# Asichurter/GPU-Computing-Course

Measured on AMD Instinct MI355X. Metric: triangle-pairs tested/sec (total collision time in ms_per_step), 1M-tri self-collision, higher is better.
Workload: dtype f64

## Files before the change

gpu-computing-course_amd/csrc/cd_build.h:

```cpp
#pragma once
#include "cd_bvh.h"

namespace cd {

struct B32 { float lx, ly, lz, hx, hy, hz; };

__device__ __forceinline__ float hw_min(float a, float b) { float r; asm("v_min_f32 %0, %1, %2" : "=v"(r) : "v"(a), "v"(b)); return r; }
__device__ __forceinline__ float hw_max(float a, float b) { float r; asm("v_max_f32 %0, %1, %2" : "=v"(r) : "v"(a), "v"(b)); return r; }
__device__ __forceinline__ B32 b32_identity()
{
    const float inf = __uint_as_float(0x7f800000u);
    return B32{inf, inf, inf, -inf, -inf, -inf};
}
__device__ __forceinline__ B32 b32_merge(const B32 &a, const B32 &b)
{
    return B32{hw_min(a.lx, b.lx), hw_min(a.ly, b.ly), hw_min(a.lz, b.lz), hw_max(a.hx, b.hx), hw_max(a.hy, b.hy), hw_max(a.hz, b.hz)};
}
__device__ __forceinline__ B32 b32_of(const AmbTable &amb, const Box &b)
{
    const Enc32 e = enc_box32(amb, b);
    return B32{e.lx, e.ly, e.lz, e.hx, e.hy, e.hz};
}
__device__ __forceinline__ B32 b32_load(const float *p)
{
    const float2 a = reinterpret_cast<const float2 *>(p)[0], b = reinterpret_cast<const float2 *>(p)[1], c = reinterpret_cast<const float2 *>(p)[2];
    return B32{a.x, a.y, b.x, b.y, c.x, c.y};
}
__device__ __forceinline__ void b32_store(float *p, const B32 &v)
{
    reinterpret_cast<float2 *>(p)[0] = make_float2(v.lx, v.ly); reinterpret_cast<float2 *>(p)[1] = make_float2(v.lz, v.hx);
    reinterpret_cast<float2 *>(p)[2] = make_float2(v.hy, v.hz);
}
__device__ __forceinline__ B32 b32_of_leaf(const LeafBox32 *__restrict__ qbox32, int j)
{
    const float4 a = reinterpret_cast<const float4 *>(qbox32 + j)[0];
    const float2 b = reinterpret_cast<const float2 *>(qbox32 + j)[2];
    return B32{a.x, a.y, a.z, a.w, b.x, b.y};
}

__device__ __forceinline__ B32 seg_query32(const float (*t)[6], int l, int r)
{
    B32 acc = b32_identity();
    l += REFIT_BLK; r += REFIT_BLK + 1;
    for (int lev = 0; lev <= REFIT_LOG; ++lev) {
        const bool on = l < r;
        if (!__builtin_amdgcn_ballot_w64(on)) break;
        const int il = (on & ((l & 1) != 0)) ? l : 0, ir = (on & ((r & 1) != 0)) ? r - 1 : 0;
        acc = b32_merge(acc, b32_load(t[il]));
        acc = b32_merge(acc, b32_load(t[ir]));
        l = (l + 1) >> 1; r >>= 1;
    }
    return acc;
}

constexpr int DK_SHIFT = 9;
typedef uint16_t DKey;
constexpr DKey DK_PAD = 0xffffu;
static_assert(DL_LEVELS - 1 <= DK_SHIFT && ((64 + 32 + 1) << DK_SHIFT) < 0xffff, "key layout");
__device__ __forceinline__ int nsv_dir(const DKey (*T)[DL_STRIDE], bool right, int s, int thr)
{
    const int tk = thr << DK_SHIFT;
    int p = s;
#pragma unroll
    for (int k = DL_LEVELS - 1; k >= 0; --k) {
        const int q = right ? p + (1 << k) : p - (1 << k);
        const int idx = right ? p : q + 1;
        const bool inside = right ? (q <= DL_N) : (q >= -1);
        const DKey v = T[k][(idx >= 0 && idx < DL_N) ? idx : 0];
        p = (inside & (v >= (DKey)tk)) ? q : p;
    }
    return p;
}

__device__ __forceinline__ unsigned long long f64_ordered(double d)
{
    const unsigned long long u = (unsigned long long)__double_as_longlong(d);
    return (u >> 63) ? ~u : (u | 0x8000000000000000ull);
}
__device__ __forceinline__ double f64_from_ordered(unsigned long long k)
{
    return __longlong_as_double((long long)((k >> 63) ? (k & 0x7fffffffffffffffull) : ~k));
}

struct ZeroPlan { uint32_t *w0; uint32_t nw0; uint4 *q; uint32_t nq; uint32_t *w1; uint32_t nw1;
                  uint32_t *flag; };

__global__ __launch_bounds__(REFIT_BLK) void k_build_block(const double *__restrict__ verts, const LeafTri *__restrict__ leaf, int n,
                                                           const uint64_t *__restrict__ keys, int32_t *__restrict__ split_of,
                                                           double *__restrict__ boxes, NodeRec32 *__restrict__ recs32, LeafBox32 *__restrict__ qbox32,
                                                           int32_t *__restrict__ root_name, double *__restrict__ seg, float *__restrict__ seg32, int nbp2,
                                                           int32_t *__restrict__ cross_list, uint32_t *__restrict__ cross_count, uint32_t cross_cap, ZeroPlan zp,
                                                           int seg_min ,
                                                           AmbTable amb, const uint8_t *__restrict__ vamb,
                                                           const uint32_t *__restrict__ hint_perm, const uint8_t *__restrict__ hint_tri, uint32_t *__restrict__ hint_cost ,
                                                           unsigned long long *__restrict__ leaf_side ,
                                                           int store_qbox )
{
    {
        const uint32_t G = gridDim.x * REFIT_BLK;
        for (uint32_t x = blockIdx.x * REFIT_BLK + threadIdx.x; x < zp.nq; x += G) zp.q[x] = make_uint4(0u, 0u, 0u, 0u);
        if (blockIdx.x == gridDim.x - 1) {
            for (uint32_t x = threadIdx.x; x < zp.nw0; x += REFIT_BLK) zp.w0[x] = 0u;
            for (uint32_t x = threadIdx.x; x < zp.nw1; x += REFIT_BLK) zp.w1[x] = 0u;
            if (threadIdx.x == 0 && zp.flag) *zp.flag = 0u;
        }
    }
    __shared__ float t[2 * REFIT_BLK][6];
    constexpr size_t TABLE_BYTES = sizeof(DKey) * DL_LEVELS * DL_STRIDE, NB_BYTES = sizeof(float) * 6 * REFIT_BLK;
    __shared__ __align__(16) unsigned char scratch[TABLE_BYTES > NB_BYTES ? TABLE_BYTES : NB_BYTES];
    DKey (*dt)[DL_STRIDE] = reinterpret_cast<DKey (*)[DL_STRIDE]>(scratch);
    float (*nb)[6] = reinterpret_cast<float (*)[6]>(scratch);
    __shared__ int16_t lsplit[REFIT_BLK];
    __shared__ uint8_t lcov[REFIT_BLK];
    __shared__ unsigned long long lexact[REFIT_BLK / 64], lcertain[REFIT_BLK / 64];
    __shared__ unsigned long long acc[6];
    __shared__ int32_t lcross[64];
    __shared__ uint32_t lcount, lbase;
    const int b = blockIdx.x, b0 = b * REFIT_BLK, tid = threadIdx.x;
    const int j = b0 + tid;
    if (tid == 0) { lcount = 0; b32_store(t[0], b32_identity()); }
    lcov[tid] = 0;
    if (tid < 6) acc[tid] = (tid & 1) ? 0ull : ~0ull;
    for (int x = tid; x < DL_STRIDE; x += REFIT_BLK) {
        int v = 0;
        const int p = b0 - 1 + x;
        if (x < DL_N && p >= 0 && p < n - 1) v = delta_k(keys, n, p, keys[p], p + 1) + 1;
        dt[0][x] = x < DL_N ? (DKey)(v << DK_SHIFT) : DK_PAD;
    }
    Box mine = box_identity();
    B32 m32 = b32_identity();
    bool exact = false, certain = false;
    if (j < n) {
        const LeafTri lt = leaf[j];
        const d3 A = load_vertex(verts, lt.v0), B = load_vertex(verts, lt.v1), C = load_vertex(verts, lt.v2);
        mine = box_set(A, B, C);
        const Enc32 e = enc_leaf32(amb, mine, A, B, C, vamb, lt.v0, lt.v1, lt.v2);
        m32 = B32{e.lx, e.ly, e.lz, e.hx, e.hy, e.hz};
        certain = e.certain;
        exact = certain && box_is_fp32(mine);
        if (!exact || n == 1) store_box(boxes, (n - 1) + j, mine);
        if (store_qbox) {
            float4 *qp = reinterpret_cast<float4 *>(qbox32 + j);
            qp[0] = make_float4(m32.lx, m32.ly, m32.lz, m32.hx);
            qp[1] = make_float4(m32.hy, m32.hz, __uint_as_float((exact ? LB_EXACT : 0u) | (certain ? LB_CERTAIN : 0u) | (box_overlap(mine, mine) ? LB_SELF : 0u)), 0.f);
        }
    }
    b32_store(t[REFIT_BLK + tid], m32);
    {
        const unsigned long long em = __builtin_amdgcn_ballot_w64(exact), cm = __builtin_amdgcn_ballot_w64(certain);
        if ((tid & 63) == 0) { lexact[tid >> 6] = em; lcertain[tid >> 6] = cm; }
    }
    for (int dd = REFIT_LOG - 1; dd >= 0; --dd) {
        __syncthreads();
        {
            const int k = REFIT_LOG - dd;
            for (int x = tid; x < DL_STRIDE; x += REFIT_BLK) {
                const int y = x + (1 << (k - 1));
                const DKey u = dt[k - 1][x], w = y < DL_STRIDE ? dt[k - 1][y] : DK_PAD;
                dt[k][x] = (w >> DK_SHIFT) < (u >> DK_SHIFT) ? (DKey)(w + (1 << (k - 1))) : u;
            }
        }
        const int cnt = 1 << dd;
        if (tid < cnt) {
            const int k = cnt + tid;
            const B32 m = b32_merge(b32_load(t[2 * k]), b32_load(t[2 * k + 1]));
            b32_store(t[k], m);
            if (REFIT_LOG - dd >= seg_min) b32_store(seg32 + 6 * ((((size_t)nbp2 + b) << dd) + tid), m);
        }
    }
    __syncthreads();
    if (j < n) {
        const B32 tot = b32_load(t[1]);
        if (m32.lx == tot.lx) atomicMin(&acc[0], f64_ordered(mine.x1));
        if (m32.hx == tot.hx) atomicMax(&acc[1], f64_ordered(mine.x2));
        if (m32.ly == tot.ly) atomicMin(&acc[2], f64_ordered(mine.y1));
        if (m32.hy == tot.hy) atomicMax(&acc[3], f64_ordered(mine.y2));
        if (m32.lz == tot.lz) atomicMin(&acc[4], f64_ordered(mine.z1));
        if (m32.hz == tot.hz) atomicMax(&acc[5], f64_ordered(mine.z2));
    }
    if (hint_cost) {
        uint32_t c = j < n ? (uint32_t)hint_tri[hint_perm[j]] : 0u;
#pragma unroll
        for (int o = 32; o; o >>= 1) { const uint32_t u = (uint32_t)__shfl_xor((int)c, o); c = u > c ? u : c; }
        if ((tid & 63) == 0 && j < n) hint_cost[j >> 6] = c;
    }
    const bool is_left = j < n && (dt[0][tid + 1] >> DK_SHIFT) > (dt[0][tid] >> DK_SHIFT);
    {
        const unsigned long long sm = __builtin_amdgcn_ballot_w64(is_left);
        if ((tid & 63) == 0 && j < n) leaf_side[j >> 6] = sm;
    }
    const int i = j;
    int first = 0, last = 0, split = 0; bool have = false, cross = false;
    if (i < n - 1) {
        const int x = tid;
        const int dL = (int)(dt[0][x] >> DK_SHIFT), dR = (int)(dt[0][x + 1] >> DK_SHIFT);
        const bool right = dR >= dL;
        const int thr = right ? dL : dR;
        int p = nsv_dir(dt, right, right ? x + 2 : x - 1, thr);
        if (right && thr == 0) p = (n - 1 <= b0 + REFIT_BLK - 1) ? (n - 1) - (b0 - 1) : DL_N;
        if (right) { first = i; last = b0 - 1 + p; have = p <= REFIT_BLK; }
        else { first = b0 + p; last = i; have = p >= 0; }
        cross = !have;
        if (have) {
            const int a = first - (b0 - 1), e = last - 1 - (b0 - 1);
            const int k = 31 - __clz(e - a + 1);
            const int a1 = e - (1 << k) + 1;
            const DKey m0 = dt[k][a], m1 = dt[k][a1];
            const int omask = (1 << DK_SHIFT) - 1;
            split = b0 - 1 + (((m1 >> DK_SHIFT) < (m0 >> DK_SHIFT)) ? a1 + ((int)m1 & omask) : a + ((int)m0 & omask));
            split_of[i] = split;
            if (split == first) lcov[split - b0] = 1;
            if (split + 1 == last) lcov[split + 1 - b0] = 1;
        }
        lsplit[tid] = have ? (int16_t)(split - b0) : (int16_t)-1;
        if (cross) {
            const uint32_t k = atomicAdd(&lcount, 1u);
            if (k < 64u) lcross[k] = i;
            else { const uint32_t g = atomicAdd(cross_count, 1u); if (g < cross_cap) cross_list[g] = i; }
        }
    }
    __syncthreads();
    b32_store(nb[tid], seg_query32(t, have ? first - b0 : 1, have ? last - b0 : 0));
    __syncthreads();
    if (j < n && n > 1 && !lcov[tid]) {
        float4 *h = const_cast<float4 *>(is_left ? rec_left(recs32, n, (uint32_t)j) : rec_right(recs32, n, (uint32_t)(j - 1)));
        h[0] = make_float4(m32.lx, m32.ly, m32.lz, m32.hx);
        h[1] = make_float4(m32.hy, m32.hz, __int_as_float(~j), __uint_as_float((exact ? 1u : 0u) | (certain ? 2u : 0u)));
    }
    if (have) {
        const bool leafL = split == first, leafR = split + 1 == last;
        const int sl = split - b0, sr = split + 1 - b0;
        const B32 bl = b32_load(leafL ? t[REFIT_BLK + sl] : nb[sl]);
        const B32 br = b32_load(leafR ? t[REFIT_BLK + sr] : nb[sr]);
        const int32_t la = leafL ? ~split : b0 + (int)lsplit[sl], lb = leafR ? ~(split + 1) : b0 + (int)lsplit[sr];
        const uint32_t fl = ((leafL && ((lcertain[sl >> 6] >> (sl & 63)) & 1ull)) ? REC_L_CERTAIN : 0u) |
                            ((leafR && ((lcertain[sr >> 6] >> (sr & 63)) & 1ull)) ? REC_R_CERTAIN : 0u);
        const uint32_t fx = ((leafL && ((lexact[sl >> 6] >> (sl & 63)) & 1ull)) ? REC_L_EXACT : 0u) |
                            ((leafR && ((lexact[sr >> 6] >> (sr & 63)) & 1ull)) ? REC_R_EXACT : 0u);
        float4 *pl = const_cast<float4 *>(rec_left(recs32, n, (uint32_t)split)), *pr = const_cast<float4 *>(rec_right(recs32, n, (uint32_t)split));
        pl[0] = make_float4(bl.lx, bl.ly, bl.lz, bl.hx); pl[1] = make_float4(bl.hy, bl.hz, __int_as_float(la), __uint_as_float((uint32_t)first | fx));
        pr[0] = make_float4(br.lx, br.ly, br.lz, br.hx); pr[1] = make_float4(br.hy, br.hz, __int_as_float(lb), __uint_as_float((uint32_t)last | fl));
        if (i == 0) *root_name = split;
    }
    if (tid == 0) {
        const Box tot{f64_from_ordered(acc[0]), f64_from_ordered(acc[1]), f64_from_ordered(acc[2]), f64_from_ordered(acc[3]),
                      f64_from_ordered(acc[4]), f64_from_ordered(acc[5])};
        store_box(seg, nbp2 + b, tot);
        if (nbp2 == 1) store_box(boxes, 0, tot);
    }
    const uint32_t cnt = min(lcount, 64u);
    if (cnt == 0) return;
    if (tid == 0) lbase = atomicAdd(cross_count, cnt);
    __syncthreads();
    if ((uint32_t)tid < cnt && lbase + tid < cross_cap) cross_list[lbase + tid] = lcross[tid];
}

__global__ __launch_bounds__(256) void k_fill_qbox(const double *__restrict__ verts, const LeafTri *__restrict__ leaf, int n, LeafBox32 *__restrict__ qbox32,
                                                   AmbTable amb, const uint8_t *__restrict__ vamb)
{
    const int j = blockIdx.x * 256 + threadIdx.x;
    if (j >= n) return;
    const LeafTri lt = leaf[j];
    const d3 A = load_vertex(verts, lt.v0), B = load_vertex(verts, lt.v1), C = load_vertex(verts, lt.v2);
    const Box mine = box_set(A, B, C);
    const Enc32 e = enc_leaf32(amb, mine, A, B, C, vamb, lt.v0, lt.v1, lt.v2);
    const bool exact = e.certain && box_is_fp32(mine);
    float4 *qp = reinterpret_cast<float4 *>(qbox32 + j);
    qp[0] = make_float4(e.lx, e.ly, e.lz, e.hx);
    qp[1] = make_float4(e.hy, e.hz, __uint_as_float((exact ? LB_EXACT : 0u) | (e.certain ? LB_CERTAIN : 0u) | (box_overlap(mine, mine) ? LB_SELF : 0u)), 0.f);
}

__device__ __forceinline__ B32 seg_piece32(const AmbTable &amb, const double *__restrict__ seg, const float *__restrict__ seg32, const LeafBox32 *__restrict__ qbox32,
                                           int n, long long P, long long k, int p, int seg_min = SEG_MIN_LEVEL)
{
    if (p > REFIT_LOG) return b32_of(amb, load_box(seg, (int)k));
    if (p >= seg_min) return b32_load(seg32 + 6 * (size_t)k);
    const long long j0 = (k << p) - P;
    B32 x = b32_identity();
    for (int u = 0; u < (1 << p); ++u) { const long long jj = j0 + u; if (jj < n) x = b32_merge(x, b32_of_leaf(qbox32, (int)jj)); }
    return x;
}

template <int CTRL>
__device__ __forceinline__ float dpp_row_shl32(float v, float fill)
{
    return __int_as_float(__builtin_amdgcn_update_dpp(__float_as_int(fill), __float_as_int(v), CTRL, 0xf, 0xf, false));
}
template <int CTRL>
__device__ __forceinline__ B32 dpp_step32(const B32 &x)
{
    const float inf = __uint_as_float(0x7f800000u);
    const B32 y{dpp_row_shl32<CTRL>(x.lx, inf), dpp_row_shl32<CTRL>(x.ly, inf), dpp_row_shl32<CTRL>(x.lz, inf),
                dpp_row_shl32<CTRL>(x.hx, -inf), dpp_row_shl32<CTRL>(x.hy, -inf), dpp_row_shl32<CTRL>(x.hz, -inf)};
    return b32_merge(x, y);
}
__device__ __forceinline__ B32 b32_shfl_down(const B32 &x, int s)
{
    return B32{__shfl_down(x.lx, s), __shfl_down(x.ly, s), __shfl_down(x.lz, s), __shfl_down(x.hx, s), __shfl_down(x.hy, s), __shfl_down(x.hz, s)};
}

__global__ __launch_bounds__(256) void k_cross_records(int n, const NodeMeta *__restrict__ meta, const double *__restrict__ seg, const float *__restrict__ seg32,
                                                       int nbp2, const LeafBox32 *__restrict__ qbox32, double *__restrict__ boxes, NodeRec32 *__restrict__ recs32,
                                                       const int32_t *__restrict__ split_of, int32_t *__restrict__ root_name,
                                                       const int32_t *__restrict__ dense, const uint32_t *__restrict__ dense_total, uint32_t dense_cap, AmbTable amb)
{
    const int tid = threadIdx.x, lane = tid & 63;
    const uint32_t total = min(*dense_total, dense_cap);
    const long long P = (long long)nbp2 * REFIT_BLK;
    for (uint32_t kk = blockIdx.x * 4 + (tid >> 6); kk < total; kk += gridDim.x * 4) {
        const int i = __builtin_amdgcn_readfirstlane(dense[kk]);
        const NodeMeta m = meta[i];
        const int first = min(i, m.z), last = max(i, m.z);
        const int split = (m.x >= n - 1) ? m.x - (n - 1) : m.x;
        const bool second = lane >= 32;
        B32 x = b32_identity();
        if (last - first < 65535) {
            const int hl = lane & 31;
            const bool is_left = hl < 16;
            const int l0 = second ? split + 1 : first, r0 = second ? last : split;
            const int p = is_left ? hl : 31 - hl;
            const long long lp = ((long long)l0 + P + ((1ll << p) - 1)) >> p;
            const long long rp = ((long long)r0 + P + 1) >> p;
            if (lp < rp) {
                const long long k = is_left ? lp : rp - 1;
                const bool take = is_left ? (lp & 1) : (rp & 1);
                if (take) x = seg_piece32(amb, seg, seg32, qbox32, n, P, k, p);
            }
            x = dpp_step32<0x101>(x); x = dpp_step32<0x102>(x); x = dpp_step32<0x104>(x); x = dpp_step32<0x108>(x);
            x = b32_merge(x, b32_shfl_down(x, 16));
        } else {
            B32 res[2];
            for (int h = 0; h < 2; ++h) {
                const int l0 = h ? split + 1 : first, r0 = h ? last : split;
                const bool is_left = lane < 32;
                const int p = is_left ? lane : 63 - lane;
                const long long lp = ((long long)l0 + P + ((1ll << p) - 1)) >> p;
                const long long rp = ((long long)r0 + P + 1) >> p;
                B32 y = b32_identity();
                if (lp < rp) {
                    const long long k = is_left ? lp : rp - 1;
                    const bool take = is_left ? (lp & 1) : (rp & 1);
                    if (take) y = seg_piece32(amb, seg, seg32, qbox32, n, P, k, p);
                }
                for (int s = 1; s < 64; s <<= 1) y = b32_merge(y, b32_shfl_down(y, s));
                res[h] = B32{__shfl(y.lx, 0), __shfl(y.ly, 0), __shfl(y.lz, 0), __shfl(y.hx, 0), __shfl(y.hy, 0), __shfl(y.hz, 0)};
            }
            x = second ? res[1] : res[0];
        }
        const bool leafL = split == first, leafR = split + 1 == last;
        uint32_t fl = 0, fx = 0;
        if (leafL) { const uint32_t f = qbox32[first].flags; if (f & LB_CERTAIN) fl |= REC_L_CERTAIN; if (f & LB_EXACT) fx |= REC_L_EXACT; }
        if (leafR) { const uint32_t f = qbox32[last].flags; if (f & LB_CERTAIN) fl |= REC_R_CERTAIN; if (f & LB_EXACT) fx |= REC_R_EXACT; }
        if (lane == 0) {
            const int32_t la = child_link(meta, split_of, m.x, n - 1);
            float4 *pl = const_cast<float4 *>(rec_left(recs32, n, (uint32_t)split));
            pl[0] = make_float4(x.lx, x.ly, x.lz, x.hx); pl[1] = make_float4(x.hy, x.hz, __int_as_float(la), __uint_as_float((uint32_t)first | fx));
            if (i == 0) { *root_name = split; store_box(boxes, 0, load_box(seg, 1)); }
        }
        if (lane == 32) {
            const int32_t lb = child_link(meta, split_of, m.y, n - 1);
            float4 *pr = const_cast<float4 *>(rec_right(recs32, n, (uint32_t)split));
            pr[0] = make_float4(x.lx, x.ly, x.lz, x.hx); pr[1] = make_float4(x.hy, x.hz, __int_as_float(lb), __uint_as_float((uint32_t)last | fl));
        }
    }
}

__device__ __forceinline__ B32 block_box32(const float *__restrict__ seg32, int nbp2, int nblocks, int b)
{
    const B32 v = b32_load(seg32 + 6 * ((size_t)nbp2 + (b < nblocks ? b : 0)));
    return b < nblocks ? v : b32_identity();
}
struct U3 { unsigned long long a, b, c; };
__device__ __forceinline__ U3 b32_words(const B32 &v)
{
    auto w = [](float lo, float hi) { return (unsigned long long)__float_as_uint(lo) | ((unsigned long long)__float_as_uint(hi) << 32); };
    return U3{w(v.lx, v.ly), w(v.lz, v.hx), w(v.hy, v.hz)};
}
template <class Low>
__device__ __forceinline__ void top32_to_lds(float *top, const float *__restrict__ blk, int nbp2, int nblocks, Low low)
{
    const int tid = threadIdx.x, lane = tid & 63;
    const int M = nbp2 >> 3;
    if (M >= 1) {
        const int T = M;
        B32 x = b32_identity();
        if (tid < T) {
            const int b = 8 * tid;
            const float4 *q = reinterpret_cast<const float4 *>(blk + 6 * (size_t)b);
            float4 v[12];
#pragma unroll
            for (int u = 0; u < 12; ++u) v[u] = q[u];
            const B32 id = b32_identity();
            B32 pr[4];
#pragma unroll
            for (int u = 0; u < 4; ++u) {
                const float4 q0 = v[3 * u], q1 = v[3 * u + 1], q2 = v[3 * u + 2];
                const B32 b0 = b + 2 * u < nblocks ? B32{q0.x, q0.y, q0.z, q0.w, q1.x, q1.y} : id, b1 = b + 2 * u + 1 < nblocks ? B32{q1.z, q1.w, q2.x, q2.y, q2.z, q2.w} : id;
                pr[u] = b32_merge(b0, b1);
                low((nbp2 >> 1) + 4 * tid + u, pr[u]);
            }
            const B32 q0 = b32_merge(pr[0], pr[1]), q1 = b32_merge(pr[2], pr[3]);
            low((nbp2 >> 2) + 2 * tid, q0); low((nbp2 >> 2) + 2 * tid + 1, q1);
            x = b32_merge(q0, q1);
            b32_store(top + 6 * (M + tid), x);
        }
        const int kt = M + tid;
        for (int s = 1; s < 64 && s < T; s <<= 1) {
            x = b32_merge(x, b32_shfl_down(x, s));
            if (tid < T && (lane & (2 * s - 1)) == 0) b32_store(top + 6 * (kt / (2 * s)), x);
        }
        __syncthreads();
        if (T > 64 && tid == 0) {
            const int kw = T / 64;
            if (T == 128) b32_store(top + 6, b32_merge(b32_load(top + 6 * 2), b32_load(top + 6 * 3)));
            else {
                const B32 l = b32_merge(b32_load(top + 6 * kw), b32_load(top + 6 * (kw + 1))), r = b32_merge(b32_load(top + 6 * (kw + 2)), b32_load(top + 6 * (kw + 3)));
                b32_store(top + 6 * 2, l); b32_store(top + 6 * 3, r); b32_store(top + 6, b32_merge(l, r));
            }
        }
    }
    __syncthreads();
}
template <class Low>
__device__ __forceinline__ void top32_tiny(const float *__restrict__ blk, int nbp2, int nblocks, Low low)
{
    if (threadIdx.x != 0) return;
    auto blkbox = [&](int b) { const B32 v = b32_load(blk + 6 * (size_t)(b < nblocks ? b : 0)); return b < nblocks ? v : b32_identity(); };
    const B32 l = b32_merge(blkbox(0), blkbox(1));
    if (nbp2 == 2) { low(1, l); return; }
    const B32 r = b32_merge(blkbox(2), blkbox(3));
    low(2, l); low(3, r); low(1, b32_merge(l, r));
}

__device__ __forceinline__ void root_box_fold(const double *__restrict__ seg, int nbp2, int nblocks, double *__restrict__ out)
{
    __shared__ double wbox[4][6];
    const int tid = threadIdx.x, lane = tid & 63, w = tid >> 6;
    const int T = nbp2 < 256 ? nbp2 : 256, per = nbp2 / T;
    Box x = box_identity();
    if (tid < T)
        for (int u = 0; u < per; ++u) { const int b = tid * per + u; if (b < nblocks) x = box_merge(x, load_box(seg, nbp2 + b)); }
    for (int s = 1; s < 64 && s < T; s <<= 1) x = box_merge(x, box_shfl_down(x, s));
    if (lane == 0) { double *d = wbox[w]; d[0] = x.x1; d[1] = x.x2; d[2] = x.y1; d[3] = x.y2; d[4] = x.z1; d[5] = x.z2; }
    __syncthreads();
    if (tid == 0) {
        auto wb = [&](int k) { return Box{wbox[k][0], wbox[k][1], wbox[k][2], wbox[k][3], wbox[k][4], wbox[k][5]}; };
        Box r = wb(0);
        for (int k = 1; k < (T + 63) / 64; ++k) r = box_merge(r, wb(k));
        store_box(out, 0, r);
    }
}

__global__ __launch_bounds__(256) void k_top_publish(const float *__restrict__ seg32, int nbp2, int nblocks, unsigned long long *__restrict__ top_pub)
{
    __shared__ float top[6 * (TOP_IN_BLOCK / 4)];
    const int span = blockIdx.x, nspans = nbp2 / TOP_IN_BLOCK, tid = threadIdx.x;
    const int live = nblocks - span * TOP_IN_BLOCK;
    auto heap = [&](int k) { const int d = 31 - __clz(k); return ((size_t)(nspans + span) << d) + (size_t)(k - (1 << d)); };
    top32_to_lds(top, seg32 + 6 * ((size_t)nbp2 + (size_t)span * TOP_IN_BLOCK), TOP_IN_BLOCK, live < 0 ? 0 : (live > TOP_IN_BLOCK ? TOP_IN_BLOCK : live),
                 [&](int k, const B32 &v) { const U3 w = b32_words(v); unsigned long long *d = top_pub + 3 * heap(k); d[0] = w.a; d[1] = w.b; d[2] = w.c; });
    for (int k = 1 + tid; k < TOP_IN_BLOCK / 4; k += 256) {
        const size_t g = heap(k);
        const unsigned long long *src = reinterpret_cast<const unsigned long long *>(top + 6 * k);
#pragma unroll
        for (int u = 0; u < 3; ++u) top_pub[3 * g + u] = src[u];
    }
}
constexpr int TOP_MAX_SPANS = 1024;
__global__ __launch_bounds__(256) void k_top_publish_upper(unsigned long long *__restrict__ top_pub, int nspans, uint32_t *__restrict__ top_flag, uint32_t top_seq)
{
    __shared__ float h[2 * TOP_MAX_SPANS][6];
    const int tid = threadIdx.x;
    for (int k = nspans + tid; k < 2 * nspans; k += 256) {
        unsigned long long *dst = reinterpret_cast<unsigned long long *>(h[k]);
#pragma unroll
        for (int u = 0; u < 3; ++u) dst[u] = top_pub[3 * (size_t)k + u];
    }
    for (int w = nspans >> 1; w >= 1; w >>= 1) {
        __syncthreads();
        for (int k = w + tid; k < 2 * w; k += 256) {
            const B32 m = b32_merge(b32_load(h[2 * k]), b32_load(h[2 * k + 1]));
            b32_store(h[k], m);
            const unsigned long long *src = reinterpret_cast<const unsigned long long *>(h[k]);
#pragma unroll
            for (int u = 0; u < 3; ++u) top_pub[3 * (size_t)k + u] = src[u];
        }
    }
    if (tid == 0) *top_flag = top_seq;
}

__global__ __launch_bounds__(256, 2) void k_cross_fused(const uint64_t *__restrict__ keys, int n, const double *__restrict__ seg, const float *__restrict__ seg32,
                                                     int nbp2, int nblocks, const unsigned long long *__restrict__ leaf_side , double *__restrict__ boxes,
                                                     NodeRec32 *__restrict__ recs32, const int32_t *__restrict__ split_of, int32_t *__restrict__ root_name,
                                                     const int32_t *__restrict__ dense, const uint32_t *__restrict__ dense_total, uint32_t dense_cap,
                                                     unsigned long long *top_pub , uint32_t *top_flag, uint32_t top_seq,
                                                     uint32_t nord ,
                                                     uint32_t order_groups, const uint32_t *__restrict__ hint_cost, uint32_t *__restrict__ hint_order)
{
    extern __shared__ float top[];
    if (blockIdx.x < nord) { build_half_order<256>(blockIdx.x & 7u, blockIdx.x >> 3, order_groups, hint_cost, hint_order, *reinterpret_cast<OrderLds<256> *>(top)); return; }
    const uint32_t bid = blockIdx.x - nord, nbid = gridDim.x - nord;
    const int tid = threadIdx.x, lane = tid & 63, g = lane / XG, gl = lane % XG;
    if (bid == nbid - 1) { root_box_fold(seg, nbp2, nblocks, boxes); return; }
    if (bid == 0) {
        if (nbp2 > TOP_IN_BLOCK) return;
        auto low = [&](int k, const B32 &v) {
            const U3 w = b32_words(v); unsigned long long *d = top_pub + 3 * (size_t)k;
            __hip_atomic_store(d, w.a, __ATOMIC_RELAXED, __HIP_MEMORY_SCOPE_AGENT); __hip_atomic_store(d + 1, w.b, __ATOMIC_RELAXED, __HIP_MEMORY_SCOPE_AGENT);
            __hip_atomic_store(d + 2, w.c, __ATOMIC_RELAXED, __HIP_MEMORY_SCOPE_AGENT);
        };
        if (nbp2 < 8) top32_tiny(seg32 + 6 * (size_t)nbp2, nbp2, nblocks, low);
        else top32_to_lds(top, seg32 + 6 * (size_t)nbp2, nbp2, nblocks, low);
        const int nn = nbp2 < 8 ? 1 : nbp2 >> 2;
        for (int k = 1 + tid; k < nn; k += 256) {
            const unsigned long long *src = reinterpret_cast<const unsigned long long *>(top + 6 * k);
#pragma unroll
            for (int u = 0; u < 3; ++u) __hip_atomic_store(top_pub + 3 * (size_t)k + u, src[u], __ATOMIC_RELAXED, __HIP_MEMORY_SCOPE_AGENT);
        }
        __builtin_amdgcn_s_waitcnt(0);
        __syncthreads();
        if (tid == 0) __hip_atomic_store(top_flag, top_seq, __ATOMIC_RELAXED, __HIP_MEMORY_SCOPE_AGENT);
        return;
    }
    constexpr int PER_WAVE = 64 / XG, PER_BLOCK = 256 / XG;
    const uint32_t total = min(*dense_total, dense_cap);
    const long long P = (long long)nbp2 * REFIT_BLK;
    for (uint32_t wbase = (bid - 1) * PER_BLOCK + (tid >> 6) * PER_WAVE; wbase < total; wbase += (nbid - 2) * PER_BLOCK) {
        const uint32_t kq = wbase + g;
        const bool live = kq < total;
        int first = 0, last = 0, split = 0;
        {
            auto delta_v = [](uint64_t ka, int ia, uint64_t kb, int ib) { const uint64_t x = ka ^ kb; return x ? __clzll((long long)x) : 64 + __clz((int)((uint32_t)ia ^ (uint32_t)ib)); };
            const int i = live ? dense[kq] : 0;
            const uint64_t ki = keys[i], kprev = keys[i > 0 ? i - 1 : 0], knext = keys[i + 1 < n ? i + 1 : n - 1];
            const int dnext = i + 1 < n ? delta_v(ki, i, knext, i + 1) : -1, dprev = i > 0 ? delta_v(ki, i, kprev, i - 1) : -1;
            const int d = (dnext - dprev) >= 0 ? 1 : -1;
            const int delta_min = d > 0 ? dprev : dnext;
            int mlen = 0;
            for (int r = 0; r < 2; ++r) {
                const bool todo = live && mlen == 0;
                if (!__builtin_amdgcn_ballot_w64(todo)) break;
                const int e = r * XG + gl;
                const long long o = (long long)i + (long long)d * (2ll << (e < 31 ? e : 31));
                const bool yes = todo && e < 31 && o >= 0 && o < n && delta_k(keys, n, i, ki, (int)o) > delta_min;
                const uint32_t no = ~group_ballot(yes, g) & ((1u << XG) - 1u);
                if (todo && no) mlen = 2 << (r * XG + __ffs((int)no) - 1);
            }
            const int l = group_last_true(live, mlen >> 1, mlen, g, gl, [&](int x) { return delta_k(keys, n, i, ki, i + x * d) > delta_min; });
            const int j = i + l * d;
            first = min(i, j); last = max(i, j);
            const uint64_t kj = keys[j];
            const uint64_t kbefore = first > 0 ? keys[first - 1] : 0ull, kafter = last < n - 1 ? keys[last + 1] : 0ull;
            const uint64_t kf = first == i ? ki : kj, kl = last == i ? ki : kj;
            const int common = delta_v(kf, first, kl, last);
            split = group_last_true(live, first, last, g, gl, [&](int x) { return delta_k(keys, n, first, kf, x) > common; });
            if (live && gl == 0) {
                if (first == 0 && last == n - 1) *root_name = split;
                else {
                    const int dl = first > 0 ? delta_v(kf, first, kbefore, first - 1) : -1, dr = last < n - 1 ? delta_v(kl, last, kafter, last + 1) : -1;
                    uint32_t *half = reinterpret_cast<uint32_t *>(const_cast<float4 *>(dr > dl ? rec_left(recs32, n, (uint32_t)last) : rec_right(recs32, n, (uint32_t)(first - 1))));
                    half[6] = (uint32_t)split;
                }
            }
        }
        const bool leafL = split == first, leafR = split + 1 == last;
        const bool crossL = !leafL && first / REFIT_BLK != split / REFIT_BLK, crossR = !leafR && (split + 1) / REFIT_BLK != last / REFIT_BLK;
        const bool own = live && gl == 0;
        const uint32_t pwL = reinterpret_cast<const uint32_t *>(rec_left(recs32, n, (uint32_t)(own && leafL ? split : 0)))[7];
        const uint32_t pwR = reinterpret_cast<const uint32_t *>(rec_right(recs32, n, (uint32_t)(own && leafR ? split : 0)))[7];
        const uint32_t flagL = ((pwL & 1u) ? LB_EXACT : 0u) | ((pwL & 2u) ? LB_CERTAIN : 0u), flagR = ((pwR & 1u) ? LB_EXACT : 0u) | ((pwR & 2u) ? LB_CERTAIN : 0u);
        const int32_t soL = split_of[own && !leafL && !crossL ? split : 0], soR = split_of[own && !leafR && !crossR ? split + 1 : 0];
        const int sweeps = __builtin_amdgcn_ballot_w64(live && last - first >= 65535) ? 2 : 1;
        B32 accL = b32_identity(), accR = b32_identity();
        auto piece = [&](int h, int p, int side, long long &k) {
            const int l0 = h ? split + 1 : first, r0 = h ? last : split;
            const long long lp = ((long long)l0 + P + ((1ll << p) - 1)) >> p;
            const long long rp = ((long long)r0 + P + 1) >> p;
            k = side ? rp - 1 : lp;
            return live && lp < rp && ((side ? rp : lp) & 1);
        };
        for (int sw = 0; sw < sweeps; ++sw) {
            const int p = gl + 16 * sw;
            long long kk[4]; bool tk[4]; bool any_top = false;
#pragma unroll
            for (int u = 0; u < 4; ++u) { tk[u] = p > REFIT_LOG && piece(u >> 1, p, u & 1, kk[u]); any_top |= tk[u]; }
            if (!__builtin_amdgcn_ballot_w64(any_top)) continue;
            bool ready = !any_top;
            const bool must = any_top && p > REFIT_LOG + 2;
#ifdef CROSS_FORCE_FALLBACK
            for (uint32_t spin = 0; spin < 0u; ++spin) {
#else
            for (uint32_t spin = 0; spin < (1u << 20); ++spin) {
#endif
                if (!ready) ready = __hip_atomic_load(top_flag, __ATOMIC_RELAXED, __HIP_MEMORY_SCOPE_AGENT) == top_seq;
                if (!__builtin_amdgcn_ballot_w64(must && !ready)) break;
                __builtin_amdgcn_s_sleep(2);
            }
#pragma unroll
            for (int u = 0; u < 4; ++u) if (tk[u]) {
                B32 v;
                if (ready) {
                    unsigned long long w[3];
#pragma unroll
                    for (int e = 0; e < 3; ++e) w[e] = __hip_atomic_load(top_pub + 3 * (size_t)kk[u] + e, __ATOMIC_RELAXED, __HIP_MEMORY_SCOPE_AGENT);
                    v = B32{__uint_as_float((uint32_t)w[0]), __uint_as_float((uint32_t)(w[0] >> 32)), __uint_as_float((uint32_t)w[1]),
                            __uint_as_float((uint32_t)(w[1] >> 32)), __uint_as_float((uint32_t)w[2]), __uint_as_float((uint32_t)(w[2] >> 32))};
                } else {
                    v = b32_identity();
                    const long long b_first = (kk[u] << (p - REFIT_LOG)) - nbp2;
                    for (long long bb = 0; bb < (1ll << (p - REFIT_LOG)); ++bb) v = b32_merge(v, block_box32(seg32, nbp2, nblocks, (int)(b_first + bb)));
                }
                if (u < 2) accL = b32_merge(accL, v); else accR = b32_merge(accR, v);
            }
        }
        {
            constexpr int SMIN = SEG32_MIN_LEVEL, LEAF_ITEMS = 2 * ((1 << SMIN) - 1), N_ITEMS = LEAF_ITEMS + 2 * (REFIT_LOG + 1 - SMIN);
            static_assert(XG == 16 && N_ITEMS <= 2 * XG, "a lane fetches items gl and gl + 16 of either child");
            static_assert(REFIT_BLK == (1 << REFIT_LOG) && SMIN >= 1 && SMIN <= REFIT_LOG, "item t >= LEAF_ITEMS is side (t - LEAF_ITEMS) & 1 of level SMIN + (t - LEAF_ITEMS) / 2 <= REFIT_LOG of a 2^REFIT_LOG-leaf block");
            B32 it[4]; bool tk[4];
            static_assert(LEAF_ITEMS <= XG, "the leaf items are a lane's FIRST item of either child (r = 0, 2)");
#pragma unroll
            for (int r = 0; r < 4; ++r) {
                const int h = r >> 1, t = gl + 16 * (r & 1);
                int p, side, e;
                if (t < LEAF_ITEMS) { const int lg = 31 - __clz(t + 2); p = lg - 1; const int idx = t + 2 - (1 << lg); side = idx >> p; e = idx & ((1 << p) - 1); }
                else { const int u = t - LEAF_ITEMS; p = SMIN + (u >> 1); side = u & 1; e = 0; if (p > REFIT_LOG) p = REFIT_LOG; }
                long long k;
                bool take = t < N_ITEMS && piece(h, p, side, k);
                const bool leafitem = (r & 1) == 0 && p < SMIN;
                uint32_t jl = 0u;
                if (leafitem) {
                    const long long jj = take ? ((k << p) - P + e) : 0;
                    take = take && jj < n;
                    jl = take ? (uint32_t)jj : 0u;
                }
                const float *p1 = leafitem ? reinterpret_cast<const float *>(rec_left(recs32, n, jl + 1u < (uint32_t)n ? jl : 0u)) : seg32 + 6 * (size_t)(take ? k : (P >> p));
                const B32 v1 = b32_load(p1);
                if ((r & 1) == 0) {
                    const B32 vr = b32_load(leafitem ? reinterpret_cast<const float *>(rec_right(recs32, n, jl > 0u ? jl - 1u : 0u)) : p1);
                    const unsigned long long sw = leaf_side[jl >> 6];
                    const bool rt = leafitem && ((sw >> (jl & 63u)) & 1ull) == 0ull;
                    it[r] = B32{rt ? vr.lx : v1.lx, rt ? vr.ly : v1.ly, rt ? vr.lz : v1.lz, rt ? vr.hx : v1.hx, rt ? vr.hy : v1.hy, rt ? vr.hz : v1.hz};
                } else it[r] = v1;
                tk[r] = take;
            }
#pragma unroll
            for (int r = 0; r < 4; ++r) if (tk[r]) { if (r < 2) accL = b32_merge(accL, it[r]); else accR = b32_merge(accR, it[r]); }
        }
        accL = dpp_step32<0x101>(accL); accL = dpp_step32<0x102>(accL); accL = dpp_step32<0x104>(accL); accL = dpp_step32<0x108>(accL);
        accR = dpp_step32<0x101>(accR); accR = dpp_step32<0x102>(accR); accR = dpp_step32<0x104>(accR); accR = dpp_step32<0x108>(accR);
        if (own) {
            const uint32_t fl = ((leafL && (flagL & LB_CERTAIN)) ? REC_L_CERTAIN : 0u) | ((leafR && (flagR & LB_CERTAIN)) ? REC_R_CERTAIN : 0u);
            const uint32_t fx = ((leafL && (flagL & LB_EXACT)) ? REC_L_EXACT : 0u) | ((leafR && (flagR & LB_EXACT)) ? REC_R_EXACT : 0u);
            const int32_t linkL = leafL ? ~split : soL, linkR = leafR ? ~(split + 1) : soR;
            float4 *pl = const_cast<float4 *>(rec_left(recs32, n, (uint32_t)split)), *pr = const_cast<float4 *>(rec_right(recs32, n, (uint32_t)split));
            pl[0] = make_float4(accL.lx, accL.ly, accL.lz, accL.hx);
            pr[0] = make_float4(accR.lx, accR.ly, accR.lz, accR.hx);
            if (crossL) { reinterpret_cast<float2 *>(pl + 1)[0] = make_float2(accL.hy, accL.hz); reinterpret_cast<uint32_t *>(pl + 1)[3] = (uint32_t)first | fx; }
            else pl[1] = make_float4(accL.hy, accL.hz, __int_as_float(linkL), __uint_as_float((uint32_t)first | fx));
            if (crossR) { reinterpret_cast<float2 *>(pr + 1)[0] = make_float2(accR.hy, accR.hz); reinterpret_cast<uint32_t *>(pr + 1)[3] = (uint32_t)last | fl; }
            else pr[1] = make_float4(accR.hy, accR.hz, __int_as_float(linkR), __uint_as_float((uint32_t)last | fl));
        }
    }
}

}
```

gpu-computing-course_amd/csrc/mi355cd.hip:

```cpp
#include "../../include/mi355cd.h"
#include "cd_math.h"
#include "cd_sort.h"
#include "cd_bvh.h"
#include "cd_build.h"
#include "cd_traverse.h"
#include "cd_post.h"
#include "cd_proximity.h"
#include "cd_ccd.h"
#include "cd_between.h"
#include "cd_rays.h"
#include "cd_points.h"

#include <hip/hip_runtime.h>
#include <hip/hip_ext.h>
#include <atomic>
#include <cfloat>
#include <chrono>
#include <cmath>
#include <cstdio>
#include <cstring>
#include <mutex>
#include <new>
#include <utility>
#include <vector>

using namespace cd;

namespace {

#define HIPCHK(expr)                                                   \
    do {                                                               \
        hipError_t e_ = (expr);                                        \
        if (e_ != hipSuccess) return -(int)e_;                         \
    } while (0)

enum Stage { ST_CREATED = 0, ST_SORTED = 1, ST_BUILT = 2, ST_REFIT = 3 };

enum Ev { EV_MORTON0, EV_MORTON1, EV_SORT1, EV_HIER0, EV_HIER1, EV_REFIT0, EV_REFIT1, EV_TRAV0, EV_TRAV1, EV_DESC1, EV_DEEP0, EV_DEEP1, EV_CHK0, EV_CHK1, EV_BLK0, EV_BLK1, EV_COUNT };

}

struct TravBuf {
    TravState *d_state = nullptr; bool state_owned = false;
    uint32_t *d_pairs = nullptr; uint64_t pairs_cap = 0;
    char *h_report = nullptr;
    uint32_t synced_reports = 0;
    uint64_t direct_id = 0; uint32_t synced_direct = 0;
    uint2 *d_defer = nullptr; uint32_t defer_cap = 0;
    Candidates *d_cand = nullptr; uint64_t cand_cap = 0;
    int32_t *d_deep = nullptr; uint64_t deep_items = 0;
    uint32_t *post_dst = nullptr; uint64_t post_n = 0;
    bool prepared = false; unsigned long long prep_seq = 0; uint32_t *prep_area = nullptr; bool posted = false;
};

struct cd_multi;
struct cd_ctx {
    uint32_t nv = 0, nt = 0;
    cd_multi *attached_multi = nullptr;
    int stage = ST_CREATED;
    int frame_mode = CD_FRAME_REFERENCE;
    uint32_t vbase = 0;
    int trav_variant = 3;
    uint32_t queries_per_wave = 64; 
    uint32_t dbg_no_shared_path = 0;
    uint32_t dbg_diag = 0;
    uint32_t dbg_lds_pad = 0;
    double frame_host[FRAME_WORDS] = {0.004501, -0.476622, -0.381965, 3.08, 0.76, 2.36, 0.0, 0.0};
    hipStream_t stream = nullptr;
    hipEvent_t ev[EV_COUNT] = {};
    double *d_verts = nullptr; uint32_t *d_vidx = nullptr; uint32_t *d_ids = nullptr;
    uint64_t *d_keys[2] = {nullptr, nullptr}; uint32_t *d_perm[2] = {nullptr, nullptr};
    uint32_t *d_counts = nullptr; uint32_t ntiles = 0;
    uint32_t *d_chunk_tot = nullptr;
    void *d_os = nullptr; size_t os_bytes = 0 , zero_bytes = 0 , sort_hi_bytes = 0 ;
    unsigned long long *d_os_look_lo = nullptr;
    uint32_t *d_os_hist = nullptr; uint32_t *d_os_ticket = nullptr; unsigned long long *d_os_look = nullptr;
    double *d_frame = nullptr, *d_partial = nullptr;
    unsigned long long *d_top_pub = nullptr; uint32_t top_seq = 0;
    LeafTri *d_leaf = nullptr; NodeMeta *d_meta = nullptr; int32_t *d_parent = nullptr; double *d_seg = nullptr; float *d_seg32 = nullptr; uint32_t nbp2 = 1; int32_t *d_cross = nullptr; uint32_t cross_cap = 0;
    double *d_boxes = nullptr; uint32_t *d_bounded = nullptr; NodeRec32 *d_recs32 = nullptr; LeafBox32 *d_qbox = nullptr;
    unsigned long long *d_leaf_side = nullptr;
    uint32_t dbg_big_offsets = 0;
    uint32_t dbg_store_qbox = 0;
    AmbTable amb = {nullptr, 0u, 0u};
    unsigned long long *d_amb_keys = nullptr, *d_amb_vals = nullptr; uint64_t amb_cap = 0; uint32_t *d_amb_flag = nullptr;
    bool cell_table_opt = true;
    uint8_t *d_vamb = nullptr, *vamb = nullptr;
    int32_t *d_root = nullptr;
    int32_t *d_split_of = nullptr;
    uint32_t stamp_mask = 15;
    uint32_t dbg_sort_windows = 0;
    bool left_frame = false; uint32_t steps_in_mode1 = 0;
    bool local_small_ok = true, local_small_active = false;
    uint32_t dbg_split_cross = 0;
    uint32_t dbg_no_fused_build = 0;
    uint32_t *d_small = nullptr;
    TravBuf tb[2];
    int exact_blocks = 1024;
    uint64_t *pp_keys[2] = {nullptr, nullptr}; uint32_t *pp_vals[2] = {nullptr, nullptr}; uint32_t *pp_flags = nullptr;
    void *pp_os = nullptr; size_t pp_os_bytes = 0; uint32_t pp_cap = 0;
    uint64_t last_pairs_on_device = 0;
    struct StepLeft {
        bool leaves_filled = false;
        bool leaf_records_filled = false;
        bool hierarchy_valid = false;
        bool internal_boxes_valid = false;
        bool last_tree_fused = false;
        bool events_ride = false;
        bool scratch_clean = false;
        bool qbox_valid = false;
    } left;
    cd_stats stats = {};
    uint32_t sort_flags[9] = {};
    bool stage_events = true;
    uint32_t dbg_report_copies = 0;
    bool order_hint_large = false;
    bool order_hint = true;
    bool order_ready = false;
    uint32_t *d_cost = nullptr, *d_order = nullptr;
    bool order_pending = false;
    uint8_t *d_tri_cost = nullptr;
    bool prezeroed = false;
    hipEvent_t tree_done_event = nullptr;
    bool quiet_pass = false;
    int sort_mode = 0;
    bool graph_opt = false;
    bool poll_opt = true;
    unsigned long long report_seq = 0;
    uint32_t polled_steps = 0, poll_fallbacks = 0;
    uint32_t poll_fb_busy = 0, poll_fb_late_word = 0, poll_fb_lost = 0, poll_max_wait_us = 0;
    bool dbg_poll_check = false;
    uint32_t poll_stale = 0;
    hipGraph_t graph = nullptr; hipGraphExec_t graph_exec = nullptr;
    struct GraphKey { uint64_t cap, spec_n; int sort_mode, variant, frame_mode; uint32_t nt, exact_blocks, dbg; const void *p_pairs, *p_cand, *p_defer, *p_report; uint64_t cand_cap; uint32_t defer_cap, pad; } graph_key = {};
    struct GraphPost { StepLeft left; uint32_t sort_passes; } graph_post = {};
    uint64_t graph_replays = 0, graph_captures = 0;
    bool all_verts_referenced = false;
    int wall_clock_khz = 0;
    double root_box_host[6] = {};
    bool root_box_valid = false;
    ProxState *d_px_state = nullptr; ProxState *h_px_state = nullptr;
    uint2 *d_px_cand = nullptr; uint64_t px_shard_cap = 0;
    uint32_t *d_px_pairs = nullptr; double *d_px_dists = nullptr; uint64_t px_pairs_cap = 0;
    CcdState *d_cc_state = nullptr; CcdState *h_cc_state = nullptr;
    uint2 *d_cc_cand = nullptr; uint64_t cc_shard_cap = 0;
    uint32_t *d_cc_pairs = nullptr; double *d_cc_toi = nullptr, *d_cc_dists = nullptr; uint64_t cc_pairs_cap = 0;
    double *d_cc_x1 = nullptr; NodeRec32 *d_cc_recs = nullptr; int32_t *d_cc_up = nullptr; uint32_t *d_cc_arrive = nullptr;
    CcdState *d_bw_state = nullptr; CcdState *h_bw_state = nullptr;
    uint2 *d_bw_cand = nullptr; uint64_t bw_shard_cap = 0;
    uint32_t *d_bw_pairs = nullptr; double *d_bw_toi = nullptr, *d_bw_dists = nullptr; uint64_t bw_pairs_cap = 0;
    double *d_bw_x1a = nullptr; double *d_bw_x1b = nullptr; uint64_t bw_x1b_cap = 0;
    NodeRec32 *d_bw_recs = nullptr; int32_t *d_bw_up = nullptr; uint32_t *d_bw_arrive = nullptr; uint64_t bw_rec_cap = 0;
    int device = 0;
    struct SweptSeen { bool ran = false; uint32_t n = 0, m_bits = 0; double dist = 0.0; };
    SweptSeen cc_seen;
    SweptSeen bw_seen;
    RayState *d_ry_state = nullptr; RayState *h_ry_state = nullptr;
    char *d_ry_block = nullptr; uint64_t ry_cap = 0;
    PointState *d_pt_state = nullptr; PointState *h_pt_state = nullptr;
    char *d_pt_block = nullptr; uint64_t pt_cap = 0;
};

namespace {

size_t top_pub_nodes(const cd_ctx *c) { return std::max<size_t>(TOP_IN_BLOCK, c->nbp2); }
size_t top_pub_bytes(const cd_ctx *c) { return sizeof(unsigned long long) * 3 * top_pub_nodes(c) + 64; }
uint32_t *top_flag_of(cd_ctx *c) { return reinterpret_cast<uint32_t *>(c->d_top_pub + 3 * top_pub_nodes(c)); }

void free_all(cd_ctx *c)
{
    hipFree(c->d_verts); hipFree(c->d_vidx); hipFree(c->d_ids);
    for (int i = 0; i < 2; ++i) { hipFree(c->d_keys[i]); hipFree(c->d_perm[i]); }
    hipFree(c->d_counts); hipFree(c->d_chunk_tot); hipFree(c->d_os); hipFree(c->d_frame); hipFree(c->d_partial);
    hipFree(c->d_top_pub); hipFree(c->d_leaf); hipFree(c->d_meta); hipFree(c->d_parent); hipFree(c->d_seg); hipFree(c->d_seg32); hipFree(c->d_cross); hipFree(c->d_boxes);
    hipFree(c->d_bounded); hipFree(c->d_recs32); hipFree(c->d_qbox); hipFree(c->d_leaf_side); hipFree(c->d_split_of); hipFree(c->d_cost); hipFree(c->d_order); hipFree(c->d_tri_cost);
    hipFree(c->d_amb_keys); hipFree(c->d_amb_flag); hipFree(c->d_vamb);
    for (TravBuf &tb : c->tb) {
        if (tb.d_pairs) hipFree(reinterpret_cast<char *>(tb.d_pairs) - sizeof(Report));
        if (tb.h_report) hipHostFree(tb.h_report);
        hipFree(tb.d_defer); hipFree(tb.d_deep); hipFree(tb.d_cand);
        if (tb.state_owned) hipFree(tb.d_state);
    }
    for (int i = 0; i < 2; ++i) { hipFree(c->pp_keys[i]); hipFree(c->pp_vals[i]); }
    hipFree(c->pp_flags); hipFree(c->pp_os);
    hipFree(c->d_px_state); hipFree(c->d_px_cand); hipFree(c->d_px_pairs); hipFree(c->d_px_dists);
    if (c->h_px_state) hipHostFree(c->h_px_state);
    hipFree(c->d_cc_state); hipFree(c->d_cc_cand); hipFree(c->d_cc_pairs); hipFree(c->d_cc_toi); hipFree(c->d_cc_dists);
    hipFree(c->d_cc_x1); hipFree(c->d_cc_recs); hipFree(c->d_cc_up); hipFree(c->d_cc_arrive);
    if (c->h_cc_state) hipHostFree(c->h_cc_state);
    hipFree(c->d_bw_state); hipFree(c->d_bw_cand); hipFree(c->d_bw_pairs); hipFree(c->d_bw_toi); hipFree(c->d_bw_dists);
    hipFree(c->d_bw_x1a); hipFree(c->d_bw_x1b); hipFree(c->d_bw_recs); hipFree(c->d_bw_up); hipFree(c->d_bw_arrive);
    if (c->h_bw_state) hipHostFree(c->h_bw_state);
    hipFree(c->d_ry_state); hipFree(c->d_ry_block);
    if (c->h_ry_state) hipHostFree(c->h_ry_state);
    hipFree(c->d_pt_state); hipFree(c->d_pt_block);
    if (c->h_pt_state) hipHostFree(c->h_pt_state);
    if (c->graph_exec) hipGraphExecDestroy(c->graph_exec);
    if (c->graph) hipGraphDestroy(c->graph);
    for (int i = 0; i < EV_COUNT; ++i) if (c->ev[i]) hipEventDestroy(c->ev[i]);
    if (c->stream) hipStreamDestroy(c->stream);
}

inline uint32_t cdiv(uint64_t a, uint32_t b) { return (uint32_t)((a + b - 1) / b); }

struct PinnedPairs { std::mutex mu; struct Buf { const uint32_t *p; uint64_t cap, id; }; std::vector<Buf> v; uint64_t next_id = 1; };
PinnedPairs &pinned_pairs() { static PinnedPairs p; return p; }
uint64_t pinned_pairs_id(const uint32_t *pairs, uint64_t cap)
{
    if (!pairs) return 0;
    PinnedPairs &pp = pinned_pairs();
    std::lock_guard<std::mutex> lock(pp.mu);
    for (const auto &e : pp.v) if (e.p == pairs && cap <= e.cap) return e.id;
    return 0;
}
constexpr uint64_t SPEC_PAIRS = 1u << 15;

__global__ void k_morton_points(const double *__restrict__ xyz, uint64_t n, const double *__restrict__ frame , uint64_t *__restrict__ keys)
{
    const unsigned long long layout = (unsigned long long)__double_as_longlong(frame[6]);
    const KeyLayout kl = key_layout(layout, frame, frame + 3);
    for (uint64_t i = blockIdx.x * (uint64_t)blockDim.x + threadIdx.x; i < n; i += (uint64_t)gridDim.x * blockDim.x)
        keys[i] = layout ? morton3d_layout(xyz[3 * i], xyz[3 * i + 1], xyz[3 * i + 2], kl) : morton3d(xyz[3 * i], xyz[3 * i + 1], xyz[3 * i + 2], frame, frame + 3);
}
__global__ void k_expand_values(const uint64_t *__restrict__ v, uint64_t n, uint64_t *__restrict__ out)
{
    for (uint64_t i = blockIdx.x * (uint64_t)blockDim.x + threadIdx.x; i < n; i += (uint64_t)gridDim.x * blockDim.x) out[i] = expand64(v[i]);
}

__global__ void k_box_pairs(const double *__restrict__ a, const double *__restrict__ b, uint64_t n, uint8_t *__restrict__ overlap,
                            double *__restrict__ merged)
{
    for (uint64_t i = blockIdx.x * (uint64_t)blockDim.x + threadIdx.x; i < n; i += (uint64_t)gridDim.x * blockDim.x) {
        const double *pa = a + 6 * i, *pb = b + 6 * i;
        const Box x{pa[0], pa[1], pa[2], pa[3], pa[4], pa[5]}, y{pb[0], pb[1], pb[2], pb[3], pb[4], pb[5]};
        if (overlap) overlap[i] = box_overlap(x, y) ? 1 : 0;
        if (merged) {
            const Box m = box_merge(x, y);
            double *o = merged + 6 * i;
            o[0] = m.x1; o[1] = m.x2; o[2] = m.y1; o[3] = m.y2; o[4] = m.z1; o[5] = m.z2;
        }
    }
}
__global__ void k_tri_contact_points(const double *__restrict__ t, uint64_t n, uint8_t *__restrict__ out)
{
    for (uint64_t i = blockIdx.x * (uint64_t)blockDim.x + threadIdx.x; i < n; i += (uint64_t)gridDim.x * blockDim.x) {
        const double *p = t + 18 * i;
        out[i] = tri_contact_fast(d3{p[0], p[1], p[2]}, d3{p[3], p[4], p[5]}, d3{p[6], p[7], p[8]},
                                  d3{p[9], p[10], p[11]}, d3{p[12], p[13], p[14]}, d3{p[15], p[16], p[17]}) ? 1 : 0;
    }
}

__global__ void k_amb_scan(const double *__restrict__ v, uint64_t n3, uint32_t *__restrict__ flag)
{
    bool any = false;
    for (uint64_t i = blockIdx.x * (uint64_t)blockDim.x + threadIdx.x; i < n3; i += (uint64_t)gridDim.x * blockDim.x) { const double x = v[i]; any |= (double)(float)x != x; }
    if (__builtin_amdgcn_ballot_w64(any) != 0ull && (threadIdx.x & 63) == 0) atomicOr(flag, 1u);
}
__global__ void k_amb_insert(const double *__restrict__ v, uint64_t n3, unsigned long long *keys, unsigned long long *vals, uint32_t shift, uint32_t mask)
{
    for (uint64_t i = blockIdx.x * (uint64_t)blockDim.x + threadIdx.x; i < n3; i += (uint64_t)gridDim.x * blockDim.x) {
        double x = v[i];
        if (x == 0.0) x = 0.0;
        const unsigned long long key = amb_key((int)(i % 3), amb_cell(x));
        uint32_t h = amb_hash(key, shift);
        for (uint32_t probe = 0; probe <= mask; ++probe) {
            unsigned long long old = __hip_atomic_load(&keys[h], __ATOMIC_RELAXED, __HIP_MEMORY_SCOPE_AGENT) & ~AMB_BIT;
            if (old == 0ull) old = atomicCAS(&keys[h], 0ull, key) & ~AMB_BIT;
            if (old == 0ull || old == key) break;
            h = (h + 1u) & mask;
        }
        const unsigned long long o = f64_ordered(x);
        unsigned long long w = __hip_atomic_load(&vals[h], __ATOMIC_RELAXED, __HIP_MEMORY_SCOPE_AGENT);
        if (w == 0ull) w = atomicCAS(&vals[h], 0ull, o);
        if (w != 0ull && w != o && !(__hip_atomic_load(&keys[h], __ATOMIC_RELAXED, __HIP_MEMORY_SCOPE_AGENT) & AMB_BIT)) atomicOr(&keys[h], AMB_BIT);
    }
}
__global__ void k_amb_vertex(const double *__restrict__ verts, uint32_t nv, AmbTable t, uint8_t *__restrict__ vamb)
{
    for (uint32_t v = blockIdx.x * blockDim.x + threadIdx.x; v < nv; v += gridDim.x * blockDim.x) {
        const double x = verts[3 * (size_t)v], y = verts[3 * (size_t)v + 1], z = verts[3 * (size_t)v + 2];
        vamb[v] = (uint8_t)((amb_lookup(t, 0, x) ? 1u : 0u) | (amb_lookup(t, 1, y) ? 2u : 0u) | (amb_lookup(t, 2, z) ? 4u : 0u));
    }
}

constexpr int BOUNDS_BLOCKS = 1024;
constexpr uint32_t SORT_RETRY_STEPS = 64;
void graph_drop(cd_ctx *c);

int ensure_pairs(cd_ctx *c, TravBuf &tb, uint64_t cap)
{
    if (cap <= tb.pairs_cap) return 0;
    if (tb.d_pairs) hipFree(reinterpret_cast<char *>(tb.d_pairs) - sizeof(Report));
    tb.d_pairs = nullptr; tb.pairs_cap = 0;
    if (&tb == &c->tb[0]) c->last_pairs_on_device = 0;
    char *block = nullptr;
    HIPCHK(hipMalloc(&block, sizeof(Report) + sizeof(uint32_t) * 2 * cap + 16));
    tb.d_pairs = reinterpret_cast<uint32_t *>(block + sizeof(Report));
    tb.pairs_cap = cap;
    return 0;
}

float elapsed(cd_ctx *c, int a, int b)
{
    float ms = 0.f;
    if (hipEventElapsedTime(&ms, c->ev[a], c->ev[b]) != hipSuccess) { (void)hipGetLastError(); return 0.f; }
    return ms;
}

inline hipError_t evrec(cd_ctx *c, int idx)
{
    if (!c->stage_events && !(idx == EV_MORTON0 || idx == EV_TRAV0 || idx == EV_DESC1 || idx == EV_TRAV1 || idx == EV_DEEP0 || idx == EV_DEEP1)) return hipSuccess;
    if (!c->stage_events && idx == EV_MORTON0 && !(c->stamp_mask & 8u)) return hipSuccess;
    return hipEventRecord(c->ev[idx], c->stream);
}

struct Prezeroed {
    cd_ctx *c;
    explicit Prezeroed(cd_ctx *c_) : c(c_) { c->prezeroed = true; }
    ~Prezeroed() { c->prezeroed = false; }
};

static bool fused_build_next(const cd_ctx *c);
int enqueue_morton_sort(cd_ctx *c, bool links_too = true, bool frame_ready = false)
{
    const uint32_t n = c->nt;
    hipStream_t s = c->stream;
    c->order_ready = false;
    HIPCHK(evrec(c, EV_MORTON0));
    const bool auto_frame = c->frame_mode == CD_FRAME_AUTO;
    if (auto_frame && !frame_ready) k_centroid_bounds<false><<<BOUNDS_BLOCKS, 256, 0, s>>>(c->d_verts, c->d_vidx, n, c->d_partial);
    const bool self_cleaning = c->prezeroed && c->sort_mode <= 1 && fused_build_next(c);
    const bool skip_memset = self_cleaning && c->left.scratch_clean;
    c->left.scratch_clean = false;
    if (!skip_memset) HIPCHK(hipMemsetAsync(c->d_os, 0, c->sort_mode <= 1 ? (c->prezeroed ? c->zero_bytes : c->sort_hi_bytes) : c->os_bytes, s));
    const int mode = c->sort_mode;
    const bool hybrid = mode <= 1;
    const int down = mode == 0 ? 4 : 0;
    const int first_digit = hybrid ? 6 : (mode == 2 ? 4 : 0);
    int cur = mode == 3 ? 0 : 1;
    const uint32_t mblocks = c->ntiles < 2048u ? c->ntiles : 2048u;
    unsigned long long host_layout = 0ull; std::memcpy(&host_layout, &c->frame_host[6], sizeof host_layout);
    const double *mframe = auto_frame ? nullptr : c->d_frame;
    const double *mpart = auto_frame ? c->d_partial : nullptr;
    if (auto_frame || host_layout != 0ull)
        k_morton<true><<<mblocks, MORTON_THREADS, 0, s>>>(c->d_verts, c->d_vidx, n, mframe, c->d_keys[cur], c->d_os_hist, first_digit, down, c->d_os_ticket + 16,
                                                          mpart, (uint32_t)BOUNDS_BLOCKS, c->d_frame, nullptr, c->d_counts);
    else
        k_morton<false><<<mblocks, MORTON_THREADS, 0, s>>>(c->d_verts, c->d_vidx, n, mframe, c->d_keys[cur], c->d_os_hist, first_digit, down, c->d_os_ticket + 16,
                                                           mpart, (uint32_t)BOUNDS_BLOCKS, c->d_frame, nullptr, c->d_counts);
    HIPCHK(evrec(c, EV_MORTON1));
    const bool chunked = c->ntiles > (uint32_t)OS_CHUNK_MIN_TILES;
    if (chunked) k_tile_chunks<<<cdiv(c->ntiles, (uint32_t)OS_CHUNK), RADIX, 0, s>>>(c->d_counts, c->ntiles, c->d_chunk_tot);
    for (int pass = first_digit; pass < 8; ++pass) {
        k_os_pass<<<c->ntiles, OS_THREADS, 0, s>>>(c->d_keys[cur], c->d_perm[cur], c->d_keys[cur ^ 1], c->d_perm[cur ^ 1], n, pass * RADIX_BITS - down,
                                                    c->d_os_hist + pass * RADIX,
                                                    (pass >= 6 ? c->d_os_look + (size_t)(pass - 6) * c->ntiles * RADIX : c->d_os_look_lo + (size_t)pass * c->ntiles * RADIX),
                                                    c->d_os_ticket + pass, pass == first_digit, HIST_COPIES, pass == first_digit ? c->d_counts : nullptr,
                                                    pass == first_digit && chunked ? c->d_chunk_tot : nullptr);
        cur ^= 1;
    }
    c->left.leaves_filled = false; c->left.leaf_records_filled = false;
    if (hybrid) {
        const LeafFill fill{c->d_vidx, c->d_ids, n, c->d_leaf, links_too ? c->d_parent : nullptr, links_too ? c->d_bounded : nullptr};
        const bool small = c->dbg_sort_windows == 2 || (c->dbg_sort_windows == 0 && c->local_small_ok);
        c->local_small_active = small;
        if (small) {
            const uint32_t per_half_cu = cdiv(n, 512u), win = per_half_cu >= (uint32_t)LocalSmall::W ? (uint32_t)LocalSmall::W : (per_half_cu < 512u ? 512u : per_half_cu);
            k_local_sort<LeafFill, LocalSmall><<<cdiv(n, win), LocalSmall::THREADS, 0, s>>>(c->d_keys[1], c->d_perm[1], c->d_keys[0], c->d_perm[0], n, 48 - down, c->d_os_ticket + 16, fill,
                                                                                            self_cleaning ? c->d_small : nullptr, self_cleaning ? 128u : 0u, win);
        } else {
            const uint32_t per_cu = cdiv(n, 256u), win = per_cu >= (uint32_t)LOCAL_W ? (uint32_t)LOCAL_W : (per_cu < 1024u ? 1024u : per_cu);
            k_local_sort<LeafFill, LocalLarge><<<cdiv(n, win), LocalLarge::THREADS, 0, s>>>(c->d_keys[1], c->d_perm[1], c->d_keys[0], c->d_perm[0], n, 48 - down, c->d_os_ticket + 16, fill,
                                                                                            self_cleaning ? c->d_small : nullptr, self_cleaning ? 128u : 0u, win);
        }
        c->left.leaves_filled = links_too;
        c->left.leaf_records_filled = true;
    } else if (mode != 3) {
        k_sort_fixup_fill<<<cdiv(n, 256), 256, 0, s>>>(c->d_keys[1], c->d_perm[1], c->d_keys[0], c->d_perm[0], n, c->d_os_ticket + 16,
                                                       c->d_vidx, c->d_ids, c->d_leaf, links_too ? c->d_parent : nullptr, links_too ? c->d_bounded : nullptr);
        c->left.leaves_filled = links_too;
        c->left.leaf_records_filled = true;
    }
    c->stats.sort_passes = hybrid ? 2 : (mode == 2 ? 4 : 8);
    HIPCHK(evrec(c, EV_SORT1));
    HIPCHK(hipGetLastError());
    return 0;
}

int enqueue_hierarchy(cd_ctx *c, bool poison_boxes)
{
    const uint32_t n = c->nt;
    hipStream_t s = c->stream;
    HIPCHK(evrec(c, EV_HIER0));
    if (!c->prezeroed) HIPCHK(hipMemsetAsync(c->d_small, 0, 16 * sizeof(uint32_t), s));
    if (!c->left.leaves_filled || poison_boxes)
        k_fill_leaves<<<cdiv(n, 256), 256, 0, s>>>(c->d_perm[0], c->d_vidx, c->d_ids, n, c->d_leaf, c->d_parent, c->d_bounded, poison_boxes ? c->d_boxes : nullptr);
    c->left.leaves_filled = false;
    if (n > 1)
        k_hierarchy<<<cdiv(n - 1, 256), 256, 0, s>>>(c->d_keys[0], (int)n, c->d_meta, c->d_parent, c->d_small);
    c->left.hierarchy_valid = true;
    HIPCHK(evrec(c, EV_HIER1));
    HIPCHK(hipGetLastError());
    return 0;
}

static bool qbox_wanted(const cd_ctx *c)
{
    return c->trav_variant != 3 || c->dbg_split_cross || c->dbg_store_qbox || c->amb.keys != nullptr || c->amb.mask != 0u || c->attached_multi != nullptr;
}
int ensure_qbox(cd_ctx *c)
{
    if (c->left.qbox_valid) return 0;
    k_fill_qbox<<<cdiv(c->nt, 256), 256, 0, c->stream>>>(c->d_verts, c->d_leaf, (int)c->nt, c->d_qbox, c->amb, (const uint8_t *)c->vamb);
    HIPCHK(hipGetLastError());
    c->left.qbox_valid = true;
    return 0;
}
int enqueue_refit(cd_ctx *c, bool write_internal, bool fused = false)
{
    const uint32_t n = c->nt;
    hipStream_t s = c->stream;
    HIPCHK(evrec(c, EV_REFIT0));
    const int nblocks = (int)cdiv(n, REFIT_BLK);
    int32_t *cross_list = c->d_cross;
    uint32_t *cross_count = c->d_small + 16;
    if (!c->prezeroed) HIPCHK(hipMemsetAsync(cross_count, 0, 64 * sizeof(uint32_t), s));
    if (fused) {
        if (!c->left.leaf_records_filled)
            k_fill_leaves<<<cdiv(n, 256), 256, 0, s>>>(c->d_perm[0], c->d_vidx, c->d_ids, n, c->d_leaf, c->d_parent, c->d_bounded, nullptr);
        c->left.leaves_filled = false; c->left.leaf_records_filled = true;
        c->left.hierarchy_valid = false;
        const bool stamp = (c->stamp_mask & 1u) != 0;
        const bool self_cleaning = c->prezeroed && c->sort_mode <= 1;
        ZeroPlan zp{nullptr, 0u, nullptr, 0u, nullptr, 0u, top_flag_of(c)};
        if (self_cleaning) {
            const size_t gran = sizeof(unsigned long long) * (size_t)c->ntiles * RADIX;
            zp = ZeroPlan{c->d_os_hist, (uint32_t)HIST_COPIES * 8u * RADIX + 8u ,
                          reinterpret_cast<uint4 *>(c->d_os_look), (uint32_t)(2 * gran / sizeof(uint4)),
                          reinterpret_cast<uint32_t *>(c->tb[0].d_state), (uint32_t)(sizeof(TravState) / sizeof(uint32_t)), top_flag_of(c)};
        }
        const int seg_min = (c->nbp2 > 1 && !c->dbg_split_cross) ? SEG32_MIN_LEVEL : SEG_MIN_LEVEL;
        const bool hint = c->order_hint && c->trav_variant >= 3 && n > 64u && c->nbp2 > 1 && !c->dbg_split_cross && (c->nbp2 <= (uint32_t)TOP_IN_BLOCK || c->order_hint_large);
        const uint32_t *hp = hint ? c->d_perm[0] : nullptr; const uint8_t *ht = hint ? c->d_tri_cost : nullptr; uint32_t *hc = hint ? c->d_cost : nullptr;
        const int store_q = qbox_wanted(c) ? 1 : 0;
        c->left.qbox_valid = store_q != 0;
        if (stamp)
            hipExtLaunchKernelGGL(k_build_block, dim3(nblocks), dim3(REFIT_BLK), 0u, s, c->ev[EV_BLK0], c->ev[EV_BLK1], 0u,
                                  (const double *)c->d_verts, (const LeafTri *)c->d_leaf, (int)n, (const uint64_t *)c->d_keys[0], c->d_split_of,
                                  c->d_boxes, c->d_recs32, c->d_qbox, c->d_root, c->d_seg, c->d_seg32, (int)c->nbp2,
                                  cross_list, cross_count, c->cross_cap, zp, seg_min, c->amb, (const uint8_t *)c->vamb, hp, ht, hc, c->d_leaf_side, store_q);
        else
            k_build_block<<<nblocks, REFIT_BLK, 0, s>>>(c->d_verts, c->d_leaf, (int)n, c->d_keys[0], c->d_split_of, c->d_boxes, c->d_recs32, c->d_qbox, c->d_root,
                                                        c->d_seg, c->d_seg32, (int)c->nbp2, cross_list, cross_count, c->cross_cap, zp, seg_min, c->amb, (const uint8_t *)c->vamb,
                                                        hp, ht, hc, c->d_leaf_side, store_q);
        c->order_pending = hint;
        c->left.scratch_clean = self_cleaning;
    } else {
        c->left.qbox_valid = true;
        k_refit_seg_local<<<nblocks, REFIT_BLK, 0, s>>>(c->d_verts, c->d_leaf, (int)n, c->d_meta, c->d_boxes, c->d_bounded,
                                                       c->d_recs32, c->d_qbox, c->d_root, write_internal ? 1 : 0, c->d_seg, (int)c->nbp2,
                                                       cross_list, cross_count, c->cross_cap, c->amb, (const uint8_t *)c->vamb);
    }
    if (fused && n > 1 && c->nbp2 > 1 && !c->dbg_split_cross) {
        const uint32_t xb = (uint32_t)nblocks < 8u ? 8u : ((uint32_t)nblocks > 1790u ? 1790u : (uint32_t)nblocks);
        hipEvent_t done = c->tree_done_event; c->tree_done_event = nullptr;
        const uint32_t ogroups = (n + 63u) / 64u;
        const uint32_t nord = c->order_pending ? 8u * (((ogroups + 7u) / 8u + (uint32_t)ORDER_MAX_ITEMS - 1u) / (uint32_t)ORDER_MAX_ITEMS) : 0u;
        c->order_pending = false;
        const bool large = c->nbp2 > (uint32_t)TOP_IN_BLOCK;
        const uint32_t xlds = std::max((uint32_t)(large ? 64u : sizeof(float) * 6 * (c->nbp2 >= 4 ? c->nbp2 / 4 : 1)) ,
                                       nord ? (uint32_t)sizeof(OrderLds<256>) : 0u );
        uint32_t *top_flag = top_flag_of(c);
        if (++c->top_seq == 0u) ++c->top_seq;
        if (large) {
            const int nspans = (int)(c->nbp2 / (uint32_t)TOP_IN_BLOCK);
            k_top_publish<<<nspans, 256, 0, s>>>(c->d_seg32, (int)c->nbp2, nblocks, c->d_top_pub);
            k_top_publish_upper<<<1, 256, 0, s>>>(c->d_top_pub, nspans, top_flag, c->top_seq);
        }
        if (done)
            hipExtLaunchKernelGGL(k_cross_fused, dim3(nord + xb + 2u ), dim3(256), xlds, s, nullptr, done, 0u,
                                  (const uint64_t *)c->d_keys[0], (int)n, (const double *)c->d_seg, (const float *)c->d_seg32, (int)c->nbp2, nblocks, (const unsigned long long *)c->d_leaf_side, c->d_boxes,
                                  c->d_recs32, (const int32_t *)c->d_split_of, c->d_root, (const int32_t *)c->d_cross, (const uint32_t *)cross_count, c->cross_cap,
                                  c->d_top_pub, top_flag, c->top_seq, nord, ogroups, (const uint32_t *)c->d_cost, c->d_order);
        else
            k_cross_fused<<<nord + xb + 2u, 256, xlds, s>>>(c->d_keys[0], (int)n, c->d_seg, c->d_seg32, (int)c->nbp2, nblocks, c->d_leaf_side, c->d_boxes,
                                                            c->d_recs32, c->d_split_of, c->d_root, c->d_cross, cross_count, c->cross_cap, c->d_top_pub, top_flag, c->top_seq,
                                                            nord, ogroups, c->d_cost, c->d_order);
        if (nord) c->order_ready = true;
        c->left.internal_boxes_valid = write_internal;
        HIPCHK(evrec(c, EV_REFIT1));
        HIPCHK(hipGetLastError());
        return 0;
    }
    const bool top_in_meta = fused && n > 1 && c->nbp2 <= (uint32_t)TOP_IN_BLOCK;
    if (!top_in_meta) {
        if (fused && n > 1) {
            int nb = (int)c->nbp2, live = nblocks;
            while (nb > 1) {
                const int span = nb < TOP_IN_BLOCK ? nb : TOP_IN_BLOCK;
                k_top_levels<<<nb / span, 256, 0, s>>>(c->d_seg, nb, live);
                nb /= span; live = (live + span - 1) / span;
            }
        } else k_refit_seg_top<<<1, 1024, 0, s>>>(c->d_seg, (int)c->nbp2, nblocks);
    }
    const uint32_t xblocks = 2u * nblocks < 256u ? 256u : (2u * nblocks > 16384u ? 16384u : 2u * (uint32_t)nblocks);
    if (fused && n > 1) {
        k_cross_meta<<<xblocks, 256, 0, s>>>(c->d_keys[0], (int)n, c->d_meta, c->d_split_of, c->d_cross, cross_count, c->cross_cap,
                                             top_in_meta ? c->d_seg : nullptr, (int)c->nbp2, nblocks);
        k_cross_records<<<xblocks, 256, 0, s>>>((int)n, c->d_meta, c->d_seg, c->d_seg32, (int)c->nbp2, c->d_qbox, c->d_boxes, c->d_recs32,
                                                c->d_split_of, c->d_root, c->d_cross, cross_count, c->cross_cap, c->amb);
    } else if (n > 1)
        k_refit_seg_cross<<<xblocks, 256, 0, s>>>((int)n, c->d_meta, c->d_seg, (int)c->nbp2, c->d_boxes, c->d_bounded, c->d_recs32,
                                                  c->d_root, write_internal ? 1 : 0, c->d_cross, cross_count, c->cross_cap, c->amb);
    c->left.internal_boxes_valid = write_internal;
    HIPCHK(evrec(c, EV_REFIT1));
    HIPCHK(hipGetLastError());
    return 0;
}

static bool fused_build_next(const cd_ctx *c) { return !(c->trav_variant == 0 || c->dbg_no_fused_build); }
int enqueue_tree(cd_ctx *c)
{
    c->left.last_tree_fused = false;
    if (!fused_build_next(c)) {
        int rc = enqueue_hierarchy(c, false);
        if (!rc) rc = enqueue_refit(c, c->trav_variant == 0, false);
        return rc;
    }
    c->left.last_tree_fused = true;
    return enqueue_refit(c, false, true);
}

template <bool EXTERNAL, bool DEEP>
void launch_pass(cd_ctx *c, TravBuf &tb, const QuerySrc &src, uint32_t items, uint64_t cap_pairs)
{
    const int n = (int)c->nt;
    hipStream_t s = c->stream;
    const uint32_t vb = EXTERNAL ? c->vbase : 0u;
    if (c->trav_variant == 0) {
        k_traverse<EXTERNAL, DEEP><<<cdiv(items, TRAV_THREADS), TRAV_THREADS, 0, s>>>(src, items, n, c->d_meta, c->d_boxes, c->d_leaf, c->d_verts, tb.d_pairs, cap_pairs, tb.d_state,
                                                                                       DEEP ? nullptr : tb.d_defer, DEEP ? 0u : tb.defer_cap, DEEP ? tb.d_deep : nullptr, vb);
    } else {
        const bool half_mode = c->trav_variant >= 3 && !EXTERNAL && (DEEP || items == (uint32_t)n);
        const uint32_t qpw = (DEEP || c->trav_variant >= 3) ? 64u : c->queries_per_wave;
        const uint64_t shard_cap = tb.cand_cap / NSHARD;
        const dim3 grid(cdiv(items, qpw * DESC_WAVES));
        const size_t pad = DEEP ? 0 : c->dbg_lds_pad;
        const bool ride = !DEEP && !c->stage_events && !c->quiet_pass;
        hipEvent_t e0 = (ride && (c->stamp_mask & 2u)) ? c->ev[EV_TRAV0] : nullptr, e1 = (ride && (c->stamp_mask & 2u)) ? c->ev[EV_DESC1] : nullptr;
        hipEvent_t e2 = (ride && (c->stamp_mask & 4u)) ? c->ev[EV_TRAV1] : nullptr;
        const uint32_t qarg = qpw | (c->dbg_no_shared_path ? 0x40000000u : 0u);
        uint2 *dl = DEEP ? nullptr : tb.d_defer; const uint32_t dcap = DEEP ? 0u : tb.defer_cap; int32_t *deep = DEEP ? tb.d_deep : nullptr;
        const uint32_t half = half_mode ? 1u : 0u;
        const bool plain = !e0 && !e1 && !e2;
        if (half_mode && !DEEP) {
            const dim3 hgrid(cdiv(items, 64u)), hblock(HALF_THREADS);
            const uint32_t *h_order = (c->order_hint && c->order_ready) ? c->d_order : nullptr;
            const bool h_rec = c->order_hint && (c->nbp2 <= (uint32_t)TOP_IN_BLOCK || c->order_hint_large);
            const uint32_t *h_perm = h_rec ? c->d_perm[0] : nullptr; uint8_t *h_tri = h_rec ? c->d_tri_cost : nullptr;
#define LAUNCH_HALF_(DIAG, TIES, BIG)                                                                                                           \
            do { if (plain) k_descend_half<DIAG, TIES, BIG><<<hgrid, hblock, pad, s>>>(src, n, c->d_recs32, tb.d_state, tb.d_cand, (unsigned long long)shard_cap, dl, dcap, h_order, h_perm, h_tri); \
                 else hipExtLaunchKernelGGL((k_descend_half<DIAG, TIES, BIG>), hgrid, hblock, (uint32_t)pad, s, e0, e1, 0u, src, n, (const NodeRec32 *)c->d_recs32, \
                                            tb.d_state, tb.d_cand, (unsigned long long)shard_cap, dl, dcap, h_order, h_perm, h_tri); } while (0)
            const bool ties = c->amb.keys != nullptr || c->amb.mask != 0u;
            const bool big = n > HALF_SMALL_N || c->dbg_big_offsets;
#define LAUNCH_HALF(DIAG, TIES) do { if (big) LAUNCH_HALF_(DIAG, TIES, true); else LAUNCH_HALF_(DIAG, TIES, false); } while (0)
            if (c->dbg_diag) { if (ties) LAUNCH_HALF(true, true); else LAUNCH_HALF(true, false); }
            else { if (ties) LAUNCH_HALF(false, true); else LAUNCH_HALF(false, false); }
#undef LAUNCH_HALF
#undef LAUNCH_HALF_
        }
        else if (qpw == 64)
            hipExtLaunchKernelGGL((k_descend<EXTERNAL, DEEP, false>), grid, dim3(DESC_THREADS), (uint32_t)pad, s, e0, e1, 0u,
                                  src, items, n, qarg, (const NodeRec32 *)c->d_recs32, (const double *)c->d_boxes, tb.d_state, tb.d_cand, (unsigned long long)shard_cap, dl, dcap, deep, vb, half);
        else
            hipExtLaunchKernelGGL((k_descend<EXTERNAL, DEEP, true>), grid, dim3(DESC_THREADS), (uint32_t)pad, s, e0, e1, 0u,
                                  src, items, n, qarg, (const NodeRec32 *)c->d_recs32, (const double *)c->d_boxes, tb.d_state, tb.d_cand, (unsigned long long)shard_cap, dl, dcap, deep, vb, half);
        if (!DEEP && !ride && !c->quiet_pass) evrec(c, EV_DESC1);
        uint32_t *post = DEEP ? nullptr : tb.post_dst; const unsigned long long post_n = DEEP ? 0ull : (unsigned long long)tb.post_n;
        if (!DEEP) { tb.posted = post != nullptr; tb.post_dst = nullptr; tb.post_n = 0; }
        if (plain)
            k_exact<EXTERNAL><<<c->exact_blocks, EXACT_THREADS, 0, s>>>(src, n, c->d_leaf, c->d_boxes, c->d_verts, vb, tb.d_cand, (unsigned long long)shard_cap, tb.d_pairs,
                                                                        (unsigned long long)cap_pairs, tb.d_state, half, post, post_n);
        else
            hipExtLaunchKernelGGL((k_exact<EXTERNAL>), dim3(c->exact_blocks), dim3(EXACT_THREADS), 0u, s, nullptr, e2, 0u,
                                  src, n, (const LeafTri *)c->d_leaf, (const double *)c->d_boxes, (const double *)c->d_verts, vb, (const Candidates *)tb.d_cand,
                                  (unsigned long long)shard_cap, tb.d_pairs, (unsigned long long)cap_pairs, tb.d_state, half, post, post_n);
        c->left.events_ride = ride;
    }
}

struct HostCounters { uint64_t n_pairs, pairs_tested, node_visits, max_shard_candidates; uint32_t n_deferred; uint64_t wave_steps, candidates, clk_start_inv, clk_end; };

int ensure_report(TravBuf &tb)
{
    if (!tb.h_report) {
        HIPCHK(hipHostMalloc(&tb.h_report, sizeof(Report) + sizeof(uint32_t) * 2 * SPEC_PAIRS, hipHostMallocCoherent));
        std::memset(tb.h_report, 0, sizeof(Report));
    }
    return 0;
}
int enqueue_report(cd_ctx *c, TravBuf &tb, bool want_pairs, uint64_t &spec_n, uint32_t *direct = nullptr, unsigned long long seq = 0)
{
    { const int rc = ensure_report(tb); if (rc) return rc; }
    if (!want_pairs) spec_n = 0; else if (spec_n > SPEC_PAIRS) spec_n = SPEC_PAIRS;
    constexpr int REPORT_BLOCKS = 32;
    const uint64_t copy_n = tb.posted ? 0 : spec_n;
    tb.posted = false;
    k_report<<<copy_n ? REPORT_BLOCKS : 1, REPORT_THREADS, 0, c->stream>>>(tb.d_state, c->d_os_ticket + 8, c->d_boxes, reinterpret_cast<Report *>(tb.h_report),
                                                              tb.d_pairs, direct ? direct : reinterpret_cast<uint32_t *>(tb.h_report + sizeof(Report)), (unsigned long long)copy_n, seq);
    return 0;
}
constexpr uint32_t POLL_WARM = 2;
bool poll_this_report(const cd_ctx *c, TravBuf &tb, uint64_t direct_id)
{
    if (direct_id && direct_id != tb.direct_id) { tb.direct_id = direct_id; tb.synced_direct = 0; }
    return c->poll_opt && !c->stage_events && c->stamp_mask == 0 && tb.synced_reports >= POLL_WARM && (!direct_id || tb.synced_direct >= POLL_WARM);
}
int wait_report(cd_ctx *c, TravBuf &tb, unsigned long long seq)
{
    if (seq != 0ull) {
        const volatile unsigned long long *p = &reinterpret_cast<const volatile Report *>(tb.h_report)->seq;
        const auto t0 = std::chrono::steady_clock::now();
        for (uint32_t it = 1; *p != seq; ++it) {
#if defined(__x86_64__) || defined(__i386__)
            __builtin_ia32_pause();
#endif
            if ((it & 1023u) == 0 && std::chrono::steady_clock::now() - t0 > std::chrono::milliseconds(20)) break;
        }
        if (*p == seq) {
            std::atomic_thread_fence(std::memory_order_acquire);
            if ((c->polled_steps & 15u) == 0) {
                const auto us = std::chrono::duration_cast<std::chrono::microseconds>(std::chrono::steady_clock::now() - t0).count();
                if ((uint64_t)us > c->poll_max_wait_us) c->poll_max_wait_us = (uint32_t)us;
            }
            if ((++c->polled_steps & 63u) == 0) HIPCHK(hipStreamSynchronize(c->stream));
            return 0;
        }
// ... 225 lines not shown
        if (cap != c->amb_cap) {
            hipFree(c->d_amb_keys); c->d_amb_keys = c->d_amb_vals = nullptr; c->amb_cap = 0;
            HIPCHK(hipMalloc(&c->d_amb_keys, sizeof(unsigned long long) * 2 * cap));
            c->d_amb_vals = c->d_amb_keys + cap;
            c->amb_cap = cap;
        }
        HIPCHK(hipMemsetAsync(c->d_amb_keys, 0, sizeof(unsigned long long) * 2 * cap, s));
        const uint32_t shift = 64u - lg, mask = (uint32_t)(cap - 1);
        k_amb_insert<<<blocks, 256, 0, s>>>(c->d_verts, n3, c->d_amb_keys, c->d_amb_vals, shift, mask);
        c->amb = AmbTable{c->d_amb_keys, shift, mask};
        if (!c->d_vamb) HIPCHK(hipMalloc(&c->d_vamb, c->nv));
        k_amb_vertex<<<(uint32_t)std::min<uint64_t>((c->nv + 255ull) / 256, 4096), 256, 0, s>>>(c->d_verts, c->nv, c->amb, c->d_vamb);
        c->vamb = c->d_vamb;
        HIPCHK(hipStreamSynchronize(s));
        HIPCHK(hipGetLastError());
    }
    if (before.keys != c->amb.keys || before.shift != c->amb.shift || before.mask != c->amb.mask) graph_drop(c);
    return CD_OK;
}
bool graph_eligible(const cd_ctx *c)
{
    return c->graph_opt && !c->stage_events && c->stamp_mask == 0 && c->sort_mode <= 1 && fused_build_next(c) && c->trav_variant == 3 &&
           c->left.scratch_clean && !c->dbg_diag && !c->dbg_lds_pad && c->nt > 1 && c->tree_done_event == nullptr;
}
int graph_step(cd_ctx *c, uint32_t *pairs, uint64_t cap_pairs, uint64_t *n_pairs, bool &handled)
{
    handled = false;
    TravBuf &tb = c->tb[0];
    hipStream_t s = c->stream;
    int rc = ensure_pairs(c, tb, cap_pairs > 0 ? cap_pairs : 1);
    if (!rc) rc = ensure_report(tb);
    if (rc) return rc;
    uint64_t spec_n = pairs ? (cap_pairs < SPEC_PAIRS ? cap_pairs : SPEC_PAIRS) : 0;
    const bool direct = pinned_pairs_id(pairs, cap_pairs) != 0;
    const cd_ctx::GraphKey key{cap_pairs, spec_n, c->sort_mode, c->trav_variant, c->frame_mode, c->nt, (uint32_t)c->exact_blocks, c->dbg_no_shared_path | (c->dbg_split_cross << 1) | (c->order_hint ? 4u : 0u) | (c->order_ready ? 8u : 0u) | (c->local_small_ok ? 16u : 0u) | (c->dbg_sort_windows << 5) | (qbox_wanted(c) ? 128u : 0u) ,
                               tb.d_pairs, tb.d_cand, tb.d_defer, direct ? (const void *)pairs : (const void *)tb.h_report, tb.cand_cap, tb.defer_cap, 0u};
    static_assert(sizeof(cd_ctx::GraphKey) == 2 * 8 + 6 * 4 + 4 * 8 + 8 + 2 * 4, "GraphKey has no padding");
    if (!c->graph_exec || std::memcmp(&key, &c->graph_key, sizeof key) != 0) {
        graph_drop(c);
        HIPCHK(hipStreamBeginCapture(s, hipStreamCaptureModeThreadLocal));
        c->prezeroed = true;
        rc = enqueue_morton_sort(c, false);
        if (!rc) rc = enqueue_tree(c);
        if (!rc) {
            QuerySrc src{c->d_leaf, c->d_boxes, c->d_qbox, c->d_root, nullptr, nullptr, c->d_os_ticket + 8};
            launch_pass<false, false>(c, tb, src, c->nt, cap_pairs);
            rc = enqueue_report(c, tb, pairs != nullptr, spec_n, direct ? pairs : nullptr);
        }
        c->prezeroed = false;
        hipGraph_t g = nullptr;
        const hipError_t ee = hipStreamEndCapture(s, &g);
        if (rc || ee != hipSuccess || !g) { if (g) hipGraphDestroy(g); (void)hipGetLastError(); c->left.scratch_clean = false; return CD_OK; }
        c->graph = g;
        if (hipGraphInstantiate(&c->graph_exec, g, nullptr, nullptr, 0) != hipSuccess) { graph_drop(c); (void)hipGetLastError(); c->left.scratch_clean = false; return CD_OK; }
        std::memset(&c->graph_key, 0, sizeof c->graph_key);
        c->graph_key = key;
        c->graph_post = {c->left, c->stats.sort_passes};
        ++c->graph_captures;
    }
    c->left = c->graph_post.left; c->stats.sort_passes = c->graph_post.sort_passes;
    HIPCHK(hipGraphLaunch(c->graph_exec, s));
    HIPCHK(hipStreamSynchronize(s));
    ++c->graph_replays;
    HostCounters h = {};
    parse_report(c, tb, h, direct ? nullptr : pairs, spec_n);
    c->stage = ST_REFIT; c->root_box_valid = true;
    { const int js = judge_sort_flags(c); if (js != CD_OK) return CD_OK; }
    if (shards_overflowed(tb, h) || h.n_deferred > 0) {
        handled = true;
        c->left.scratch_clean = false;
        return run_traversal(c, tb, nullptr, 0, pairs, cap_pairs, n_pairs);
    }
    handled = true;
    const uint64_t found = h.n_pairs, ncopy = found < cap_pairs ? found : cap_pairs;
    if (pairs && ncopy > spec_n) {
        HIPCHK(hipMemcpyAsync(pairs + 2 * spec_n, tb.d_pairs + 2 * spec_n, sizeof(uint32_t) * 2 * (ncopy - spec_n), hipMemcpyDeviceToHost, s));
        HIPCHK(hipStreamSynchronize(s));
    }
    c->stats.ms_morton = c->stats.ms_sort = c->stats.ms_hierarchy = c->stats.ms_refit = c->stats.ms_traverse = c->stats.ms_descend = c->stats.ms_exact = 0.f;
    c->stats.ms_pipeline = c->stats.ms_build_block = 0.f;
    c->stats.traverse_launches = 0; c->stats.stack_overflows = 0;
    c->stats.n_pairs = found; c->stats.pairs_tested = h.pairs_tested; c->stats.node_visits = h.node_visits;
    c->stats.wave_steps = h.wave_steps; c->stats.candidates = h.candidates;
    c->stats.ms_descend_clock = (h.clk_end && h.clk_start_inv && c->wall_clock_khz > 0) ? (float)((double)(h.clk_end - ~h.clk_start_inv) / (double)c->wall_clock_khz) : 0.f;
    c->last_pairs_on_device = ncopy;
    if (n_pairs) *n_pairs = found;
    return found > cap_pairs ? CD_OVERFLOW : CD_OK;
}

}

void multi_detach_from(cd_ctx *c);

extern "C" {

const char *cd_version(void) { return "mi355cd 0.1 gfx950"; }

int cd_create(cd_ctx **out, const double *verts_xyz, uint32_t nv, const uint32_t *vidx3, const uint32_t *ids, uint32_t nt)
{
    if (!out || !verts_xyz || !vidx3 || nv == 0 || nt == 0) return CD_ERR_ARG;
    *out = nullptr;
    int ndev = 0;
    if (hipGetDeviceCount(&ndev) != hipSuccess || ndev == 0) return CD_ERR_NO_DEVICE;
    for (uint64_t k = 0; k < 3ull * nt; ++k) if (vidx3[k] >= nv) return CD_ERR_INDEX;
    bool all_ref = true;
    { std::vector<uint8_t> used(nv, 0);
      for (uint64_t k = 0; k < 3ull * nt; ++k) used[vidx3[k]] = 1;
      for (uint32_t v = 0; v < nv && all_ref; ++v) all_ref = used[v] != 0; }
    cd_ctx *c = new (std::nothrow) cd_ctx();
    if (!c) return CD_ERR_ARG;
    c->nv = nv; c->nt = nt;
    c->all_verts_referenced = all_ref;
    c->ntiles = cdiv(nt, SORT_TILE);
    { int dev = 0, khz = 0; if (hipGetDevice(&dev) == hipSuccess) { c->device = dev; if (hipDeviceGetAttribute(&khz, hipDeviceAttributeWallClockRate, dev) == hipSuccess) c->wall_clock_khz = khz; } (void)hipGetLastError(); }
    const size_t n = nt;
#define ALLOC(p, bytes) do { hipError_t e_ = hipMalloc((void **)&(p), (bytes)); if (e_ != hipSuccess) { free_all(c); delete c; return -(int)e_; } } while (0)
    hipError_t e = hipStreamCreateWithFlags(&c->stream, hipStreamNonBlocking);
    if (e != hipSuccess) { delete c; return -(int)e; }
    for (int i = 0; i < EV_COUNT; ++i) { e = hipEventCreate(&c->ev[i]); if (e != hipSuccess) { free_all(c); delete c; return -(int)e; } }
    ALLOC(c->d_verts, sizeof(double) * 3 * (size_t)nv);
    ALLOC(c->d_vidx, sizeof(uint32_t) * 3 * n);
    if (ids) ALLOC(c->d_ids, sizeof(uint32_t) * n);
    for (int i = 0; i < 2; ++i) { ALLOC(c->d_keys[i], sizeof(uint64_t) * n); ALLOC(c->d_perm[i], sizeof(uint32_t) * n); }
    ALLOC(c->d_counts, sizeof(uint32_t) * RADIX * c->ntiles);
    ALLOC(c->d_chunk_tot, sizeof(uint32_t) * RADIX * cdiv(c->ntiles, (uint32_t)OS_CHUNK));
    const size_t gran = sizeof(unsigned long long) * (size_t)c->ntiles * RADIX;
    const size_t look_off = sizeof(uint32_t) * HIST_COPIES * 8 * RADIX + 128;
    c->sort_hi_bytes = look_off + 2 * gran;
    const size_t small_off = (c->sort_hi_bytes + 127) & ~(size_t)127, state_off = small_off + 512;
    c->zero_bytes = state_off + sizeof(TravState);
    const size_t lo_off = (c->zero_bytes + 127) & ~(size_t)127;
    c->os_bytes = lo_off + 6 * gran;
    ALLOC(c->d_os, c->os_bytes);
    c->d_small = reinterpret_cast<uint32_t *>(reinterpret_cast<char *>(c->d_os) + small_off);
    c->tb[0].d_state = reinterpret_cast<TravState *>(reinterpret_cast<char *>(c->d_os) + state_off);
    c->d_root = reinterpret_cast<int32_t *>(c->d_small + 96);
    c->d_os_hist = reinterpret_cast<uint32_t *>(c->d_os);
    c->d_os_ticket = c->d_os_hist + HIST_COPIES * 8 * RADIX;
    c->d_os_look = reinterpret_cast<unsigned long long *>(reinterpret_cast<char *>(c->d_os) + look_off);
    c->d_os_look_lo = reinterpret_cast<unsigned long long *>(reinterpret_cast<char *>(c->d_os) + lo_off);
    ALLOC(c->d_frame, sizeof(double) * FRAME_WORDS);
    ALLOC(c->d_partial, sizeof(double) * BOUNDS_STRIDE * BOUNDS_BLOCKS);
    ALLOC(c->d_leaf, sizeof(LeafTri) * n);
    { hipError_t e_ = hipMemset(c->d_leaf, 0, sizeof(LeafTri) * n); if (e_ != hipSuccess) { free_all(c); delete c; return -(int)e_; } }
    ALLOC(c->d_meta, sizeof(NodeMeta) * n);
    ALLOC(c->d_parent, sizeof(int32_t) * 2 * n);
    { uint32_t nb = cdiv(nt, REFIT_BLK); c->nbp2 = 1; while (c->nbp2 < nb) c->nbp2 <<= 1; }
    if (c->nbp2 / (uint32_t)TOP_IN_BLOCK > (uint32_t)TOP_MAX_SPANS) { free_all(c); delete c; return CD_ERR_ARG; }
    ALLOC(c->d_seg, sizeof(double) * 6 * (size_t)c->nbp2 * REFIT_BLK);
    ALLOC(c->d_top_pub, top_pub_bytes(c));
    if (hipMemset(c->d_top_pub, 0, top_pub_bytes(c)) != hipSuccess) { free_all(c); delete c; return -(int)hipGetLastError(); }
    ALLOC(c->d_seg32, sizeof(float) * 6 * ((size_t)c->nbp2 << (REFIT_LOG - SEG32_MIN_LEVEL + 1)));
    c->cross_cap = nt;
    ALLOC(c->d_cross, sizeof(int32_t) * (size_t)c->cross_cap);
    ALLOC(c->d_boxes, sizeof(double) * 6 * 2 * n);
    ALLOC(c->d_bounded, sizeof(uint32_t) * n);
    ALLOC(c->d_recs32, sizeof(NodeRec32) * n);
    ALLOC(c->d_qbox, sizeof(LeafBox32) * n);
    ALLOC(c->d_leaf_side, sizeof(unsigned long long) * ((n + 63) / 64 + 1));
    ALLOC(c->d_split_of, sizeof(int32_t) * n);
    { const size_t groups = ((size_t)n + 63) / 64;
      ALLOC(c->d_cost, sizeof(uint32_t) * groups); ALLOC(c->d_order, sizeof(uint32_t) * groups); ALLOC(c->d_tri_cost, n);
      if (hipMemset(c->d_cost, 0, sizeof(uint32_t) * groups) != hipSuccess || hipMemset(c->d_tri_cost, 0, n) != hipSuccess) { free_all(c); delete c; return CD_ERR_ARG; } }
    c->tb[0].cand_cap = ((4 * n > (1u << 20) ? 4 * n : (1u << 20)) + 4 * NSHARD - 1) / (4 * NSHARD) * (4 * NSHARD);
    ALLOC(c->tb[0].d_cand, sizeof(Candidates) * c->tb[0].cand_cap);
    c->tb[0].defer_cap = 1u << 16;
    ALLOC(c->tb[0].d_defer, sizeof(uint2) * c->tb[0].defer_cap);
#undef ALLOC
    bool ok = hipMemcpy(c->d_verts, verts_xyz, sizeof(double) * 3 * (size_t)nv, hipMemcpyHostToDevice) == hipSuccess &&
              hipMemcpy(c->d_vidx, vidx3, sizeof(uint32_t) * 3 * n, hipMemcpyHostToDevice) == hipSuccess &&
              (!ids || hipMemcpy(c->d_ids, ids, sizeof(uint32_t) * n, hipMemcpyHostToDevice) == hipSuccess) &&
              hipMemcpy(c->d_frame, c->frame_host, sizeof(double) * FRAME_WORDS, hipMemcpyHostToDevice) == hipSuccess;
    if (!ok) { free_all(c); delete c; return -(int)hipGetLastError(); }
    { const int rc = amb_refresh(c); if (rc) { free_all(c); delete c; return rc; } }
    *out = c;
    return CD_OK;
}

void cd_destroy(cd_ctx *c)
{
    if (!c) return;
    multi_detach_from(c);
    hipStreamSynchronize(c->stream);
    free_all(c);
    delete c;
}

int cd_update_vertices(cd_ctx *c, const double *verts_xyz)
{
    if (!c || !verts_xyz) return CD_ERR_ARG;
    HIPCHK(hipStreamSynchronize(c->stream));
    HIPCHK(hipMemcpy(c->d_verts, verts_xyz, sizeof(double) * 3 * (size_t)c->nv, hipMemcpyHostToDevice));
    c->stage = ST_CREATED;
    c->root_box_valid = false;
    return amb_refresh(c);
}

static int install_frame(cd_ctx *c, int mode, const double off[3], const double span[3], unsigned long long layout)
{
    if (off) for (int a = 0; a < 3; ++a) { c->frame_host[a] = off[a]; c->frame_host[3 + a] = span[a]; }
    std::memcpy(&c->frame_host[6], &layout, sizeof layout); c->frame_host[7] = 0.0;
    c->frame_mode = mode;
    HIPCHK(hipStreamSynchronize(c->stream));
    HIPCHK(hipMemcpy(c->d_frame, c->frame_host, sizeof(double) * FRAME_WORDS, hipMemcpyHostToDevice));
    c->stage = ST_CREATED;
    graph_drop(c);
    return CD_OK;
}
int cd_set_morton_frame(cd_ctx *c, int mode, const double offset[3], const double span[3])
{
    if (!c) return CD_ERR_ARG;
    if (mode == CD_FRAME_REFERENCE) {
        const double ref[6] = {0.004501, -0.476622, -0.381965, 3.08, 0.76, 2.36};
        return install_frame(c, mode, ref, ref + 3, 0ull);
    }
    if (mode == CD_FRAME_CUSTOM) {
        if (!offset || !span) return CD_ERR_ARG;
        return install_frame(c, mode, offset, span, 0ull);
    }
    if (mode != CD_FRAME_AUTO) return CD_ERR_ARG;
    return install_frame(c, mode, nullptr, nullptr, 0ull);
}
int cd_set_morton_frame_layout(cd_ctx *c, const double offset[3], const double span[3], uint64_t layout)
{
    if (!c || !offset || !span || !layout_ok(layout)) return CD_ERR_ARG;
    for (int a = 0; a < 3; ++a) if (!(span[a] > 0.0)) return CD_ERR_ARG;
    return install_frame(c, CD_FRAME_CUSTOM, offset, span, layout);
}
int cd_get_morton_frame(cd_ctx *c, double offset[3], double span[3], uint64_t *layout)
{
    if (!c) return CD_ERR_ARG;
    if (c->stage < ST_SORTED) return CD_ERR_ORDER;
    double f[FRAME_WORDS];
    HIPCHK(hipStreamSynchronize(c->stream));
    HIPCHK(hipMemcpy(f, c->d_frame, sizeof f, hipMemcpyDeviceToHost));
    for (int a = 0; a < 3; ++a) { if (offset) offset[a] = f[a]; if (span) span[a] = f[3 + a]; }
    if (layout) std::memcpy(layout, &f[6], sizeof *layout);
    return CD_OK;
}

constexpr int SORT_REDO = 77;
constexpr int SORT_REDO_MAX = 4;
namespace { int judge_sort_flags(cd_ctx *c)
{
    for (int i = 0; i < 9; ++i) if (c->sort_flags[i]) c->left.scratch_clean = false;
    for (int i = 0; i < 8; ++i) if (c->sort_flags[i]) return CD_ERR_SORT;
    const uint32_t f = c->sort_flags[8];
    if (!f) return CD_OK;
    if (c->sort_mode >= 3) return CD_ERR_SORT;
    if (f & SORTF_FIXUP) { c->sort_mode = 3; c->left_frame = false; return SORT_REDO; }
    if (f & SORTF_RUN) {
        if (!(f & SORTF_ABOVE) && c->local_small_active && c->local_small_ok && c->sort_mode <= 1) { c->local_small_ok = false; return SORT_REDO; }
        c->sort_mode = 2; c->left_frame = false; return SORT_REDO;
    }
    if (c->sort_mode == 0) { c->sort_mode = 1; c->left_frame = true; c->steps_in_mode1 = 0; return SORT_REDO; }
    c->sort_mode = 2; c->left_frame = false; return SORT_REDO;
} }
static void sort_retry_tick(cd_ctx *c)
{
    if (c->sort_mode == 1 && c->left_frame && ++c->steps_in_mode1 >= SORT_RETRY_STEPS) { c->sort_mode = 0; c->steps_in_mode1 = 0; c->local_small_ok = true; graph_drop(c); }
}
extern "C++" {
template <class Attempt> static int with_sort_redo(cd_ctx *c, Attempt attempt)
{
    for (int redo = 0;; ++redo) {
        const int rc = attempt();
        if (rc < 0) return rc;
        const int js = judge_sort_flags(c);
        if (js != SORT_REDO) return js ? js : rc;
        if (redo == SORT_REDO_MAX) return CD_ERR_SORT;
    }
}
static int sync_with_flags(cd_ctx *c)
{
    HIPCHK(hipMemcpyAsync(c->sort_flags, c->d_os_ticket + 8, sizeof c->sort_flags, hipMemcpyDeviceToHost, c->stream));
    HIPCHK(hipMemcpyAsync(c->root_box_host, c->d_boxes, sizeof(double) * 6, hipMemcpyDeviceToHost, c->stream));
    HIPCHK(hipStreamSynchronize(c->stream));
    return CD_OK;
}
template <class Tail> static int fused_step(cd_ctx *c, Tail tail)
{
    const int rc = with_sort_redo(c, [&]() -> int {
        Prezeroed fused(c);
        int re = enqueue_morton_sort(c, !fused_build_next(c));
        if (!re) re = enqueue_tree(c);
        return re ? re : tail();
    });
    if (rc >= 0) { c->root_box_valid = true; c->stage = ST_REFIT; }
    return rc;
}
}
static void read_build_times(cd_ctx *c)
{
    c->stats.ms_morton = elapsed(c, EV_MORTON0, EV_MORTON1);
    c->stats.ms_sort = elapsed(c, EV_MORTON1, EV_SORT1);
    c->stats.ms_hierarchy = c->left.last_tree_fused ? 0.f : elapsed(c, EV_HIER0, EV_HIER1);
    c->stats.ms_refit = elapsed(c, EV_REFIT0, EV_REFIT1);
}

int cd_morton_sort(cd_ctx *c)
{
    if (!c) return CD_ERR_ARG;
    sort_retry_tick(c);
    const int rc = with_sort_redo(c, [c]() -> int {
        const int re = enqueue_morton_sort(c);
        if (re) return re;
        HIPCHK(hipMemcpyAsync(c->sort_flags, c->d_os_ticket + 8, sizeof c->sort_flags, hipMemcpyDeviceToHost, c->stream));
// ... 104 lines not shown
    c->stats.ms_build_block = (c->left.last_tree_fused && (c->stamp_mask & 1u)) ? elapsed(c, EV_BLK0, EV_BLK1) : 0.f;
    return rc;
}

int cd_brute_force(cd_ctx *c, int box_filter, uint32_t *pairs, uint64_t cap_pairs, uint64_t *n_pairs)
{
    if (!c || (cap_pairs && !pairs)) return CD_ERR_ARG;
    int rc = ensure_pairs(c, c->tb[0], cap_pairs > 0 ? cap_pairs : 1);
    if (rc) return rc;
    hipStream_t s = c->stream;
    HIPCHK(hipMemsetAsync(c->tb[0].d_state, 0, sizeof(TravState), s));
    k_brute_force<<<cdiv(c->nt, 256), 256, 0, s>>>(c->d_verts, c->d_vidx, c->d_ids, c->nt, box_filter, c->tb[0].d_pairs, cap_pairs, c->tb[0].d_state);
    HostCounters h;
    { int r = read_state(c, c->tb[0], h); if (r) return r; }
    HIPCHK(hipGetLastError());
    const uint64_t ncopy = h.n_pairs < cap_pairs ? h.n_pairs : cap_pairs;
    if (pairs && ncopy) HIPCHK(hipMemcpy(pairs, c->tb[0].d_pairs, sizeof(uint32_t) * 2 * ncopy, hipMemcpyDeviceToHost));
    c->stats.n_pairs = h.n_pairs; c->stats.pairs_tested = h.pairs_tested;
    c->last_pairs_on_device = ncopy;
    if (n_pairs) *n_pairs = h.n_pairs;
    return h.n_pairs > cap_pairs ? CD_OVERFLOW : CD_OK;
}

int cd_test_pairs(cd_ctx *c, const uint32_t *pairs, uint64_t np, uint8_t *out)
{
    if (!c || !pairs || !out) return CD_ERR_ARG;
    if (np == 0) return CD_OK;
    for (uint64_t k = 0; k < 2 * np; ++k) if (pairs[k] >= c->nt) return CD_ERR_INDEX;
    uint32_t *d_p = nullptr; uint8_t *d_o = nullptr;
    HIPCHK(hipMalloc(&d_p, sizeof(uint32_t) * 2 * np));
    if (hipMalloc(&d_o, np) != hipSuccess) { hipFree(d_p); return -(int)hipErrorOutOfMemory; }
    int rc = CD_OK;
    if (hipMemcpy(d_p, pairs, sizeof(uint32_t) * 2 * np, hipMemcpyHostToDevice) != hipSuccess) rc = -(int)hipErrorInvalidValue;
    if (!rc) {
        k_test_pairs<<<cdiv(np, 256), 256, 0, c->stream>>>(c->d_verts, c->d_vidx, c->d_ids, d_p, np, d_o);
        if (hipStreamSynchronize(c->stream) != hipSuccess || hipMemcpy(out, d_o, np, hipMemcpyDeviceToHost) != hipSuccess) rc = -(int)hipGetLastError();
    }
    hipFree(d_p); hipFree(d_o);
    return rc;
}

int cd_sorted_pairs(cd_ctx *c, uint32_t *pairs, uint64_t cap_pairs, uint64_t *n_pairs)
{
    if (!c || !n_pairs || (cap_pairs && !pairs)) return CD_ERR_ARG;
    if (c->stage < ST_REFIT) return CD_ERR_ORDER;
    if (c->stats.n_pairs > c->last_pairs_on_device) return CD_OVERFLOW;
    const uint32_t m = (uint32_t)c->last_pairs_on_device;
    *n_pairs = m;
    if (m == 0) return CD_OK;
    int rc = pp_reserve(c, m);
    if (rc) return rc;
    hipStream_t s = c->stream;
    k_pairs_to_keys<<<cdiv(m, 256), 256, 0, s>>>(c->tb[0].d_pairs, m, c->pp_keys[0]);
    if ((rc = pp_sort(c, m))) return rc;
    k_keys_to_pairs<<<cdiv(m, 256), 256, 0, s>>>(c->pp_keys[0], m, reinterpret_cast<uint32_t *>(c->pp_keys[1]));
    const uint64_t ncopy = m < cap_pairs ? m : cap_pairs;
    if (ncopy) HIPCHK(hipMemcpyAsync(pairs, c->pp_keys[1], sizeof(uint32_t) * 2 * ncopy, hipMemcpyDeviceToHost, s));
    uint32_t f[8];
    HIPCHK(hipMemcpyAsync(f, reinterpret_cast<uint32_t *>(c->pp_os) + 8 * RADIX + 8, sizeof f, hipMemcpyDeviceToHost, s));
    HIPCHK(hipStreamSynchronize(s));
    HIPCHK(hipGetLastError());
    for (int i = 0; i < 8; ++i) if (f[i]) return CD_ERR_SORT;
    return m > cap_pairs ? CD_OVERFLOW : CD_OK;
}

int cd_collision_triangles(cd_ctx *c, uint32_t *ids, uint64_t cap, uint64_t *n)
{
    if (!c || !n || (cap && !ids)) return CD_ERR_ARG;
    if (c->stage < ST_REFIT) return CD_ERR_ORDER;
    if (c->stats.n_pairs > c->last_pairs_on_device) return CD_OVERFLOW;
    const uint64_t m2_64 = 2 * c->last_pairs_on_device;
    *n = 0;
    if (m2_64 == 0) return CD_OK;
    if (m2_64 > 0xfffffff0ull) return CD_ERR_ARG;
    const uint32_t m2 = (uint32_t)m2_64;
    int rc = pp_reserve(c, m2);
    if (rc) return rc;
    hipStream_t s = c->stream;
    k_ids_to_keys<<<cdiv(m2, 256), 256, 0, s>>>(c->tb[0].d_pairs, m2, c->pp_keys[0]);
    if ((rc = pp_sort(c, m2))) return rc;
    k_unique_flags<<<cdiv(m2, 256), 256, 0, s>>>(c->pp_keys[0], m2, c->pp_flags);
    k_scan_exclusive<<<1, 1024, 0, s>>>(c->pp_flags, m2);
    uint32_t *out = c->pp_vals[0], *d_count = reinterpret_cast<uint32_t *>(c->pp_os) + 8 * RADIX;
    k_unique_scatter<<<cdiv(m2, 256), 256, 0, s>>>(c->pp_keys[0], c->pp_flags, m2, out, c->pp_cap, d_count);
    uint32_t cnt = 0, f[8];
    HIPCHK(hipMemcpyAsync(&cnt, d_count, sizeof cnt, hipMemcpyDeviceToHost, s));
    HIPCHK(hipMemcpyAsync(f, reinterpret_cast<uint32_t *>(c->pp_os) + 8 * RADIX + 8, sizeof f, hipMemcpyDeviceToHost, s));
    HIPCHK(hipStreamSynchronize(s));
    HIPCHK(hipGetLastError());
    for (int i = 0; i < 8; ++i) if (f[i]) return CD_ERR_SORT;
    *n = cnt;
    const uint64_t ncopy = cnt < cap ? cnt : cap;
    if (ncopy) HIPCHK(hipMemcpy(ids, out, sizeof(uint32_t) * ncopy, hipMemcpyDeviceToHost));
    return cnt > cap ? CD_OVERFLOW : CD_OK;
}

int cd_export_keys(cd_ctx *c, uint64_t *keys, uint32_t *perm)
{
    if (!c) return CD_ERR_ARG;
    if (c->stage < ST_SORTED) return CD_ERR_ORDER;
    if (keys) HIPCHK(hipMemcpy(keys, c->d_keys[0], sizeof(uint64_t) * c->nt, hipMemcpyDeviceToHost));
    if (perm) HIPCHK(hipMemcpy(perm, c->d_perm[0], sizeof(uint32_t) * c->nt, hipMemcpyDeviceToHost));
    return CD_OK;
}

int cd_export_tree(cd_ctx *c, int32_t *parent, int32_t *left, int32_t *right, double *boxes, uint32_t *bounded)
{
    if (!c) return CD_ERR_ARG;
    if (c->stage < ST_BUILT) return CD_ERR_ORDER;
    const size_t n = c->nt;
    { const int rm = materialise_internal_boxes(c); if (rm) return rm; }
    if (parent) HIPCHK(hipMemcpy(parent, c->d_parent, sizeof(int32_t) * (2 * n - 1), hipMemcpyDeviceToHost));
    if ((left || right) && n > 1) {
        std::vector<int4> m(n - 1);
        HIPCHK(hipMemcpy(m.data(), c->d_meta, sizeof(int4) * (n - 1), hipMemcpyDeviceToHost));
        for (size_t i = 0; i < n - 1; ++i) { if (left) left[i] = m[i].x; if (right) right[i] = m[i].y; }
    }
    if (boxes || bounded) { if (c->stage < ST_REFIT) return CD_ERR_ORDER; }

    if (boxes) HIPCHK(hipMemcpy(boxes, c->d_boxes, sizeof(double) * 6 * (2 * n - 1), hipMemcpyDeviceToHost));
    if (bounded && n > 1) HIPCHK(hipMemcpy(bounded, c->d_bounded, sizeof(uint32_t) * (n - 1), hipMemcpyDeviceToHost));
    return CD_OK;
}

int cd_debug_counters(cd_ctx *c, unsigned long long out[12])
{
    if (!c || !out) return CD_ERR_ARG;
    std::vector<TravState> h(1);
    HIPCHK(hipMemcpy(h.data(), c->tb[0].d_state, sizeof(TravState), hipMemcpyDeviceToHost));
    for (int k = 0; k < 12; ++k) { out[k] = 0; for (int i = 0; i < NSHARD; ++i) out[k] += h[0].shard[i].pad[k]; }
    return CD_OK;
}

int cd_debug_hint(cd_ctx *c, uint32_t *cost, uint32_t *order, uint8_t *tri)
{
    if (!c) return CD_ERR_ARG;
    HIPCHK(hipStreamSynchronize(c->stream));
    const size_t groups = ((size_t)c->nt + 63) / 64;
    if (tri) HIPCHK(hipMemcpy(tri, c->d_tri_cost, c->nt, hipMemcpyDeviceToHost));
    if (cost) HIPCHK(hipMemcpy(cost, c->d_cost, sizeof(uint32_t) * groups, hipMemcpyDeviceToHost));
    if (order) { if (!c->order_ready) return CD_ERR_ORDER; HIPCHK(hipMemcpy(order, c->d_order, sizeof(uint32_t) * groups, hipMemcpyDeviceToHost)); }
    return CD_OK;
}

int cd_debug_hint_set(cd_ctx *c, const uint32_t *order)
{
    if (!c || !order) return CD_ERR_ARG;
    HIPCHK(hipStreamSynchronize(c->stream));
    const uint32_t groups = (c->nt + 63u) / 64u;
    std::vector<uint8_t> seen(groups, 0);
    for (uint32_t b = 0; b < groups; ++b) { if (order[b] >= groups || seen[order[b]]) return CD_ERR_ARG; seen[order[b]] = 1; }
    HIPCHK(hipMemcpy(c->d_order, order, sizeof(uint32_t) * groups, hipMemcpyHostToDevice));
    c->order_ready = true;
    return CD_OK;
}

int cd_debug_records(cd_ctx *c, void *recs, void *qboxes, int32_t *root)
{
    if (!c) return CD_ERR_ARG;
    if (c->stage < ST_REFIT) return CD_ERR_ORDER;
    HIPCHK(hipStreamSynchronize(c->stream));
    if (recs) HIPCHK(hipMemcpy(recs, c->d_recs32, sizeof(NodeRec32) * (size_t)c->nt, hipMemcpyDeviceToHost));
    if (qboxes) { const int rq = ensure_qbox(c); if (rq) return rq; HIPCHK(hipStreamSynchronize(c->stream)); HIPCHK(hipMemcpy(qboxes, c->d_qbox, sizeof(LeafBox32) * (size_t)c->nt, hipMemcpyDeviceToHost)); }
    if (root) HIPCHK(hipMemcpy(root, c->d_root, sizeof(int32_t), hipMemcpyDeviceToHost));
    return CD_OK;
}

int cd_debug_swept(cd_ctx *c, int between, void *recs, int32_t *up, uint32_t *m_bits, float *pad, uint32_t *n_leaves)
{
    if (!c || (between != 0 && between != 1)) return CD_ERR_ARG;
    const cd_ctx::SweptSeen &seen = between ? c->bw_seen : c->cc_seen;
    if (!seen.ran) return CD_ERR_ORDER;
    HIPCHK(hipStreamSynchronize(c->stream));
    const size_t n = seen.n;
    if (n >= 2) {
        if (recs) HIPCHK(hipMemcpy(recs, between ? c->d_bw_recs : c->d_cc_recs, sizeof(NodeRec32) * n, hipMemcpyDeviceToHost));
        if (up) HIPCHK(hipMemcpy(up, between ? c->d_bw_up : c->d_cc_up, sizeof(int32_t) * (2 * n - 1), hipMemcpyDeviceToHost));
    }
    if (m_bits) *m_bits = seen.m_bits;
    if (pad) {
        float m; std::memcpy(&m, &seen.m_bits, sizeof m);
        const double v = 2.0 * seen.dist + 2.0 * seen.dist * PROX_SLACK + (double)m * PROX_SLACK;
        float f = INFINITY;
        if (v <= (double)FLT_MAX) { f = (float)v; if ((double)f < v) f = std::nextafterf(f, INFINITY); }
        *pad = f;
    }
    if (n_leaves) *n_leaves = seen.n;
    return CD_OK;
}

static int morton_batch(const void *in, size_t in_bytes, uint64_t n, const double frame[FRAME_WORDS], uint64_t *out)
{
    int ndev = 0;
    if (hipGetDeviceCount(&ndev) != hipSuccess || ndev == 0) return CD_ERR_NO_DEVICE;
    void *d_in = nullptr; uint64_t *d_out = nullptr; double *d_frame = nullptr;
    int rc = CD_OK;
    hipError_t e = hipMalloc(&d_in, in_bytes);
    if (e == hipSuccess) e = hipMalloc(&d_out, sizeof(uint64_t) * n);
    if (e == hipSuccess && frame) e = hipMalloc(&d_frame, sizeof(double) * FRAME_WORDS);
    if (e == hipSuccess) e = hipMemcpy(d_in, in, in_bytes, hipMemcpyHostToDevice);
    if (e == hipSuccess && frame) e = hipMemcpy(d_frame, frame, sizeof(double) * FRAME_WORDS, hipMemcpyHostToDevice);
    if (e == hipSuccess) {
        const uint32_t blocks = cdiv(n, 256) < 4096u ? cdiv(n, 256) : 4096u;
        if (frame) k_morton_points<<<blocks, 256>>>(static_cast<const double *>(d_in), n, d_frame, d_out);
        else k_expand_values<<<blocks, 256>>>(static_cast<const uint64_t *>(d_in), n, d_out);
        e = hipGetLastError();
        if (e == hipSuccess) e = hipMemcpy(out, d_out, sizeof(uint64_t) * n, hipMemcpyDeviceToHost);
    }
    if (e != hipSuccess) rc = -(int)e;
    hipFree(d_in); hipFree(d_out); hipFree(d_frame);
    return rc;
}
int cd_morton3d_points(const double *xyz, uint64_t n, const double offset[3], const double span[3], uint64_t *keys)
{
    if (!xyz || !keys || (!offset) != (!span)) return CD_ERR_ARG;
    if (n == 0) return CD_OK;
    double frame[FRAME_WORDS] = {0.004501, -0.476622, -0.381965, 3.08, 0.76, 2.36, 0.0, 0.0};
    if (offset) for (int a = 0; a < 3; ++a) { frame[a] = offset[a]; frame[3 + a] = span[a]; }
    return morton_batch(xyz, sizeof(double) * 3 * n, n, frame, keys);
}
int cd_morton3d_points_layout(const double *xyz, uint64_t n, const double offset[3], const double span[3], uint64_t layout, uint64_t *keys)
{
    if (!xyz || !keys || !offset || !span || !layout_ok(layout)) return CD_ERR_ARG;
    if (n == 0) return CD_OK;
    double frame[FRAME_WORDS] = {offset[0], offset[1], offset[2], span[0], span[1], span[2], 0.0, 0.0};
    std::memcpy(&frame[6], &layout, sizeof layout);
    return morton_batch(xyz, sizeof(double) * 3 * n, n, frame, keys);
}
int cd_expand64_values(const uint64_t *v, uint64_t n, uint64_t *out)
{
    if (!v || !out) return CD_ERR_ARG;
    if (n == 0) return CD_OK;
    return morton_batch(v, sizeof(uint64_t) * n, n, nullptr, out);
}

int cd_box_pairs(const double *a, const double *b, uint64_t n, uint8_t *overlap, double *merged)
{
    if (!a || !b || (!overlap && !merged)) return CD_ERR_ARG;
    if (n == 0) return CD_OK;
    int ndev = 0;
    if (hipGetDeviceCount(&ndev) != hipSuccess || ndev == 0) return CD_ERR_NO_DEVICE;
    double *d_a = nullptr, *d_b = nullptr, *d_m = nullptr; uint8_t *d_o = nullptr;
    const size_t bytes = sizeof(double) * 6 * n;
    hipError_t e = hipMalloc(&d_a, bytes);
    if (e == hipSuccess) e = hipMalloc(&d_b, bytes);
    if (e == hipSuccess && overlap) e = hipMalloc(&d_o, n);
    if (e == hipSuccess && merged) e = hipMalloc(&d_m, bytes);
    if (e == hipSuccess) e = hipMemcpy(d_a, a, bytes, hipMemcpyHostToDevice);
    if (e == hipSuccess) e = hipMemcpy(d_b, b, bytes, hipMemcpyHostToDevice);
    if (e == hipSuccess) {
        k_box_pairs<<<cdiv(n, 256) < 4096u ? cdiv(n, 256) : 4096u, 256>>>(d_a, d_b, n, d_o, d_m);
        e = hipGetLastError();
        if (e == hipSuccess && overlap) e = hipMemcpy(overlap, d_o, n, hipMemcpyDeviceToHost);
        if (e == hipSuccess && merged) e = hipMemcpy(merged, d_m, bytes, hipMemcpyDeviceToHost);
    }
    hipFree(d_a); hipFree(d_b); hipFree(d_o); hipFree(d_m);
    return e == hipSuccess ? CD_OK : -(int)e;
}
int cd_tri_contact_points(const double *tri, uint64_t n, uint8_t *out)
{
    if (!tri || !out) return CD_ERR_ARG;
    if (n == 0) return CD_OK;
    int ndev = 0;
    if (hipGetDeviceCount(&ndev) != hipSuccess || ndev == 0) return CD_ERR_NO_DEVICE;
    double *d_t = nullptr; uint8_t *d_o = nullptr;
    hipError_t e = hipMalloc(&d_t, sizeof(double) * 18 * n);
    if (e == hipSuccess) e = hipMalloc(&d_o, n);
    if (e == hipSuccess) e = hipMemcpy(d_t, tri, sizeof(double) * 18 * n, hipMemcpyHostToDevice);
    if (e == hipSuccess) {
        k_tri_contact_points<<<cdiv(n, 256) < 4096u ? cdiv(n, 256) : 4096u, 256>>>(d_t, n, d_o);
        e = hipGetLastError();
        if (e == hipSuccess) e = hipMemcpy(out, d_o, n, hipMemcpyDeviceToHost);
    }
    hipFree(d_t); hipFree(d_o);
    return e == hipSuccess ? CD_OK : -(int)e;
}

int cd_alloc_host_pairs(uint64_t cap_pairs, uint32_t **pairs)
{
    if (!pairs || cap_pairs == 0) return CD_ERR_ARG;
    *pairs = nullptr;
    int ndev = 0;
    if (hipGetDeviceCount(&ndev) != hipSuccess || ndev == 0) return CD_ERR_NO_DEVICE;
    void *p = nullptr;
    HIPCHK(hipHostMalloc(&p, sizeof(uint32_t) * 2 * cap_pairs + 16, hipHostMallocCoherent));
    PinnedPairs &pp = pinned_pairs();
    { std::lock_guard<std::mutex> lock(pp.mu); pp.v.push_back(PinnedPairs::Buf{static_cast<const uint32_t *>(p), cap_pairs, pp.next_id++}); }
    *pairs = static_cast<uint32_t *>(p);
    return CD_OK;
}
void cd_free_host_pairs(uint32_t *pairs)
{
    if (!pairs) return;
    PinnedPairs &pp = pinned_pairs();
    { std::lock_guard<std::mutex> lock(pp.mu);
      for (size_t i = 0; i < pp.v.size(); ++i) if (pp.v[i].p == pairs) { pp.v.erase(pp.v.begin() + (long)i); break; } }
    hipHostFree(pairs);
}


int cd_get_stats(cd_ctx *c, cd_stats *out) { if (!c || !out) return CD_ERR_ARG; *out = c->stats; return CD_OK; }
int cd_num_triangles(cd_ctx *c, uint32_t *nt) { if (!c || !nt) return CD_ERR_ARG; *nt = c->nt; return CD_OK; }

int cd_set_option(cd_ctx *c, int key, int64_t value)
{
    if (!c) return CD_ERR_ARG;
// ... 676 lines not shown
```

gpu-computing-course_amd/pyhost/mi355cd.py:

```python
from __future__ import annotations

import ctypes as C
import os

import numpy as np

_HERE = os.path.dirname(os.path.abspath(__file__))
LIB_PATH = os.path.join(os.path.dirname(_HERE), "libmi355cd.so")

CD_OK, CD_OVERFLOW = 0, 1
CD_ERR_ARG, CD_ERR_ORDER, CD_ERR_NO_DEVICE, CD_ERR_INDEX = -1001, -1002, -1003, -1004
CD_FRAME_REFERENCE, CD_FRAME_AUTO, CD_FRAME_CUSTOM = 0, 1, 2
CD_ERR_SORT, CD_ERR_IO, CD_ERR_FORMAT = -1005, -1006, -1007
CD_OPT_TRAVERSAL, CD_OPT_QUERIES_PER_WAVE, CD_OPT_SORT_FULL, CD_OPT_STAGE_TIMING, CD_OPT_KERNEL_STAMPS, CD_OPT_GRAPH, CD_OPT_POLL = 0, 1, 2, 3, 4, 5, 6
CD_OPT_CELL_TABLE = 7
CD_OPT_ORDER_HINT = 8
CD_DBG_LDS_PAD, CD_DBG_EXACT_BLOCKS, CD_DBG_NO_SHARED_PATH, CD_DBG_DIAG, CD_DBG_STAGEWISE_BUILD, CD_DBG_SPLIT_CROSS = 0, 1, 2, 3, 4, 5
CD_DBG_SORT_WINDOWS, CD_DBG_GET_SORT_FORM = 7, 8
CD_DBG_POLL_SCAN, CD_DBG_GET_POLL_STALE, CD_DBG_GET_POLL_FALLBACKS, CD_DBG_GET_POLLED_STEPS, CD_DBG_GET_TREE_WAS_FUSED = 10, 11, 12, 13, 14
CD_DBG_GET_ORDER_STATE = 15
CD_DBG_GET_POLL_FB_WHY, CD_DBG_GET_POLL_MAX_WAIT_US = 16, 17
CD_DBG_REPORT_COPIES = 6
CD_DBG_STORE_QBOX = 9
CD_DBG_BIG_OFFSETS = 18
CD_DBG_GET_GRAPH_CAPTURES, CD_DBG_GET_GRAPH_REPLAYS = 19, 20

QUERY_DTYPE = np.dtype([("v", "<f8", (9,)), ("id", "<u4"), ("vidx", "<u4", (3,))])
assert QUERY_DTYPE.itemsize == 88


class CdStats(C.Structure):
    _fields_ = [("ms_morton", C.c_float), ("ms_sort", C.c_float), ("ms_hierarchy", C.c_float),
                ("ms_refit", C.c_float), ("ms_traverse", C.c_float), ("ms_check", C.c_float),
                ("traverse_launches", C.c_uint32), ("stack_overflows", C.c_uint32),
                ("n_pairs", C.c_uint64), ("pairs_tested", C.c_uint64), ("node_visits", C.c_uint64),
                ("wave_steps", C.c_uint64), ("candidates", C.c_uint64),
                ("ms_descend", C.c_float), ("ms_exact", C.c_float), ("sort_passes", C.c_uint32), ("ms_pipeline", C.c_float),
                ("ms_build_block", C.c_float), ("ms_descend_clock", C.c_float)]


CD_MULTI_SELF_PEER, CD_MULTI_TIMING, CD_MULTI_SELF_SLICE, CD_MULTI_CROSS_SERIAL, CD_MULTI_INJECT_FAILURE, CD_MULTI_PRIORITY_STREAM = 1, 2, 4, 8, 16, 32
CD_MULTI_INJECT_ALLOC_FAILURE = 64
CD_ERR_RCCL, CD_ERR_PEER, CD_ERR_INJECTED = -1008, -1009, -1010


class CdCcdInfo(C.Structure):
    _fields_ = [("n_candidates", C.c_uint64), ("n_tested", C.c_uint64), ("n_evals", C.c_uint64), ("n_unresolved", C.c_uint64)]


class CdRayInfo(C.Structure):
    _fields_ = [("n_hits", C.c_uint64), ("node_visits", C.c_uint64), ("tri_tests", C.c_uint64)]


CD_RAY_ANY = 1
RAY_MISS = 0xFFFFFFFF


class CdPointInfo(C.Structure):
    _fields_ = [("n_found", C.c_uint64), ("node_visits", C.c_uint64), ("tri_tests", C.c_uint64)]


CD_POINT_ANY = 1
POINT_NONE = 0xFFFFFFFF


class CdMultiInfo(C.Structure):
    _fields_ = [("world", C.c_uint32), ("rank", C.c_uint32), ("n_peers", C.c_uint32), ("host_syncs", C.c_uint32), ("attempts", C.c_uint32),
                ("failed_rank_plus1", C.c_uint32), ("sent_queries", C.c_uint64), ("recv_queries", C.c_uint64), ("local_pairs", C.c_uint64),
                ("cross_pairs", C.c_uint64), ("pairs_tested", C.c_uint64), ("query_cap", C.c_uint64),
                ("ms_tree", C.c_float), ("ms_allgather", C.c_float), ("ms_pack", C.c_float), ("ms_counts", C.c_float),
                ("ms_exchange", C.c_float), ("ms_local", C.c_float), ("ms_cross", C.c_float), ("pad1", C.c_float)]


EXPORTS = [
    "cd_load_obj", "cd_free_obj", "cd_create", "cd_destroy", "cd_update_vertices", "cd_set_morton_frame", "cd_get_morton_frame", "cd_set_morton_frame_layout", "cd_morton_sort",
    "cd_build_hierarchy", "cd_refit_boxes", "cd_check_internal", "cd_check_leaves",
    "cd_check_triangle_idx", "cd_find_collisions", "cd_build_tree", "cd_self_collide", "cd_sorted_pairs", "cd_collision_triangles", "cd_brute_force",
    "cd_test_pairs", "cd_export_keys", "cd_export_tree", "cd_get_stats", "cd_debug_counters", "cd_debug_records", "cd_debug_swept", "cd_num_triangles",
    "cd_set_option", "cd_set_vertex_id_base", "cd_root_box", "cd_pack_queries", "cd_find_collisions_queries", "cd_version",
    "cd_debug_option", "cd_debug_hint", "cd_debug_hint_set", "cd_morton3d_points", "cd_morton3d_points_layout", "cd_expand64_values", "cd_box_pairs", "cd_tri_contact_points", "cd_alloc_host_pairs", "cd_free_host_pairs",
    "cd_multi_unique_id", "cd_multi_create", "cd_multi_create_from_comm", "cd_multi_destroy", "cd_multi_set_flags", "cd_multi_step",
    "cd_find_proximity", "cd_self_proximity", "cd_tri_distance_points",
    "cd_find_ccd", "cd_self_ccd", "cd_ccd_points",
    "cd_find_collisions_between", "cd_find_proximity_between", "cd_find_ccd_between",
    "cd_cast_rays", "cd_ray_tri_points",
    "cd_closest_points", "cd_pt_tri_points",
]

_lib = None


def load_library(path: str = LIB_PATH) -> C.CDLL:
    global _lib
    if _lib is None:
        try:
            import torch
        except Exception:
            pass
    if _lib is not None:
        return _lib
    path = os.environ.get("MI355CD_LIB", path)
    if not os.path.exists(path):
        raise RuntimeError(f"{path} not built: run __graft_entry__.build() (there is no CPU fallback)")
    lib = C.CDLL(path)
    vp, u32p, u64p, i32p, dp = C.c_void_p, C.POINTER(C.c_uint32), C.POINTER(C.c_uint64), C.POINTER(C.c_int32), C.POINTER(C.c_double)
    lib.cd_load_obj.argtypes = [C.c_char_p, C.POINTER(dp), u32p, C.POINTER(u32p), u32p, C.c_int]
    lib.cd_free_obj.argtypes = [dp, u32p]
    lib.cd_free_obj.restype = None
    lib.cd_create.argtypes = [C.POINTER(vp), vp, C.c_uint32, vp, vp, C.c_uint32]
    lib.cd_destroy.argtypes = [vp]
    lib.cd_destroy.restype = None
    lib.cd_update_vertices.argtypes = [vp, vp]
    lib.cd_set_morton_frame.argtypes = [vp, C.c_int, vp, vp]
    lib.cd_get_morton_frame.argtypes = [vp, vp, vp, u64p]
    lib.cd_set_morton_frame_layout.argtypes = [vp, vp, vp, C.c_uint64]
    lib.cd_morton_sort.argtypes = [vp]
    lib.cd_build_hierarchy.argtypes = [vp, u32p]
    lib.cd_refit_boxes.argtypes = [vp]
    lib.cd_check_internal.argtypes = [vp, vp]
    lib.cd_check_leaves.argtypes = [vp, vp]
    lib.cd_check_triangle_idx.argtypes = [vp, C.c_uint32, u32p]
    lib.cd_find_collisions.argtypes = [vp, vp, C.c_uint64, u64p]
    lib.cd_build_tree.argtypes = [vp]
    lib.cd_self_collide.argtypes = [vp, vp, C.c_uint64, u64p]
    lib.cd_sorted_pairs.argtypes = [vp, vp, C.c_uint64, u64p]
    lib.cd_collision_triangles.argtypes = [vp, vp, C.c_uint64, u64p]
    lib.cd_brute_force.argtypes = [vp, C.c_int, vp, C.c_uint64, u64p]
    lib.cd_test_pairs.argtypes = [vp, vp, C.c_uint64, vp]
    lib.cd_export_keys.argtypes = [vp, vp, vp]
    lib.cd_export_tree.argtypes = [vp, vp, vp, vp, vp, vp]
    lib.cd_get_stats.argtypes = [vp, C.POINTER(CdStats)]
    lib.cd_debug_counters.argtypes = [vp, vp]
    lib.cd_debug_records.argtypes = [vp, vp, vp, vp]
    lib.cd_debug_swept.argtypes = [vp, C.c_int, vp, vp, u32p, C.POINTER(C.c_float), u32p]
    lib.cd_debug_hint.argtypes = [vp, vp, vp, vp]
    lib.cd_debug_hint_set.argtypes = [vp, vp]
    lib.cd_num_triangles.argtypes = [vp, u32p]
    lib.cd_set_option.argtypes = [vp, C.c_int, C.c_int64]
    lib.cd_set_vertex_id_base.argtypes = [vp, C.c_uint32]
    lib.cd_root_box.argtypes = [vp, vp]
    lib.cd_pack_queries.argtypes = [vp, vp, vp, C.c_uint64, u64p]
    lib.cd_find_collisions_queries.argtypes = [vp, vp, C.c_uint64, vp, C.c_uint64, u64p]
    lib.cd_version.restype = C.c_char_p
    lib.cd_alloc_host_pairs.argtypes = [C.c_uint64, C.POINTER(u32p)]
    lib.cd_free_host_pairs.argtypes = [u32p]
    lib.cd_free_host_pairs.restype = None
    lib.cd_morton3d_points.argtypes = [vp, C.c_uint64, vp, vp, vp]
    lib.cd_morton3d_points_layout.argtypes = [vp, C.c_uint64, vp, vp, C.c_uint64, vp]
    lib.cd_expand64_values.argtypes = [vp, C.c_uint64, vp]
    lib.cd_debug_option.argtypes = [vp, C.c_int, C.c_int64, C.POINTER(C.c_int64)]
    lib.cd_box_pairs.argtypes = [vp, vp, C.c_uint64, vp, vp]
    lib.cd_tri_contact_points.argtypes = [vp, C.c_uint64, vp]
    lib.cd_find_proximity.argtypes = [vp, C.c_double, vp, vp, C.c_uint64, u64p, u64p]
    lib.cd_self_proximity.argtypes = [vp, C.c_double, vp, vp, C.c_uint64, u64p, u64p]
    lib.cd_tri_distance_points.argtypes = [vp, C.c_uint64, vp]
    lib.cd_find_ccd.argtypes = [vp, vp, C.c_double, vp, vp, vp, C.c_uint64, u64p, vp]
    lib.cd_self_ccd.argtypes = [vp, vp, C.c_double, vp, vp, vp, C.c_uint64, u64p, vp]
    lib.cd_ccd_points.argtypes = [vp, C.c_uint64, C.c_double, vp, vp, vp]
    lib.cd_find_collisions_between.argtypes = [vp, vp, vp, C.c_uint64, u64p, u64p]
    lib.cd_find_proximity_between.argtypes = [vp, vp, C.c_double, vp, vp, C.c_uint64, u64p, u64p]
    lib.cd_find_ccd_between.argtypes = [vp, vp, vp, vp, C.c_double, vp, vp, vp, C.c_uint64, u64p, vp]
    lib.cd_cast_rays.argtypes = [vp, vp, C.c_uint64, C.c_int, vp, vp, vp, vp, vp, vp]
    lib.cd_ray_tri_points.argtypes = [vp, vp, C.c_uint64, vp, vp, vp, vp]
    lib.cd_closest_points.argtypes = [vp, vp, C.c_uint64, C.c_int, vp, vp, vp, vp, vp, vp, vp, vp]
    lib.cd_pt_tri_points.argtypes = [vp, vp, C.c_uint64, vp, vp, vp, vp, vp]
    lib.cd_multi_unique_id.argtypes = [vp]
    lib.cd_multi_create.argtypes = [C.POINTER(vp), vp, vp, C.c_int, C.c_int, C.c_uint64, C.c_int]
    lib.cd_multi_create_from_comm.argtypes = [C.POINTER(vp), vp, vp, C.c_uint64, C.c_int]
    lib.cd_multi_destroy.argtypes = [vp]
    lib.cd_multi_destroy.restype = None
    lib.cd_multi_set_flags.argtypes = [vp, C.c_int]
    lib.cd_multi_step.argtypes = [vp, vp, C.c_uint64, u64p, C.POINTER(CdMultiInfo)]
    for name in EXPORTS:
        if name not in ("cd_destroy", "cd_version", "cd_free_obj", "cd_multi_destroy", "cd_free_host_pairs"):
            getattr(lib, name).restype = C.c_int
    _lib = lib
    return lib


class CdError(RuntimeError):
    def __init__(self, fn: str, rc: int):
        super().__init__(f"{fn} failed with status {rc}")
        self.rc = rc


def _ptr(a):
    return None if a is None else a.ctypes.data_as(C.c_void_p)


class CollisionDetector:

    def __init__(self, verts: np.ndarray, vidx: np.ndarray, ids: np.ndarray | None = None):
        self.lib = load_library()
        self.verts = np.ascontiguousarray(verts, dtype=np.float64).reshape(-1, 3)
        self.vidx = np.ascontiguousarray(vidx, dtype=np.uint32).reshape(-1, 3)
        self.ids = None if ids is None else np.ascontiguousarray(ids, dtype=np.uint32)
        self.nv, self.nt = self.verts.shape[0], self.vidx.shape[0]
        self._ctx = C.c_void_p()
        rc = self.lib.cd_create(C.byref(self._ctx), _ptr(self.verts), self.nv, _ptr(self.vidx), _ptr(self.ids), self.nt)
        if rc != CD_OK:
            self._ctx = C.c_void_p()
            raise CdError("cd_create", rc)

    def close(self):
        if getattr(self, "_ctx", None) and self._ctx.value:
            self.lib.cd_destroy(self._ctx)
            self._ctx = C.c_void_p()

    def __del__(self):
        try:
            self.close()
        except Exception:
            pass

    def __enter__(self):
        return self

    def __exit__(self, *a):
        self.close()

    def _chk(self, fn, rc, allow=(CD_OK,)):
        if rc not in allow:
            raise CdError(fn, rc)
        return rc

    def set_morton_frame(self, mode=CD_FRAME_REFERENCE, offset=None, span=None):
        off = None if offset is None else np.ascontiguousarray(offset, dtype=np.float64)
        sp = None if span is None else np.ascontiguousarray(span, dtype=np.float64)
        self._chk("cd_set_morton_frame", self.lib.cd_set_morton_frame(self._ctx, mode, _ptr(off), _ptr(sp)))

    def get_morton_frame(self):
        off = np.zeros(3, dtype=np.float64); sp = np.zeros(3, dtype=np.float64); lay = C.c_uint64(0)
        self._chk("cd_get_morton_frame", self.lib.cd_get_morton_frame(self._ctx, _ptr(off), _ptr(sp), C.byref(lay)))
        return off, sp, int(lay.value)

    def set_morton_frame_layout(self, offset, span, layout: int):
        off = np.ascontiguousarray(offset, dtype=np.float64); sp = np.ascontiguousarray(span, dtype=np.float64)
        self._chk("cd_set_morton_frame_layout", self.lib.cd_set_morton_frame_layout(self._ctx, _ptr(off), _ptr(sp), int(layout)))

    def keep_auto_frame(self):
        off, sp, lay = self.get_morton_frame()
        self.set_morton_frame_layout(off, sp, lay)
        return off, sp, lay

    def set_option(self, key: int, value: int):
        self._chk("cd_set_option", self.lib.cd_set_option(self._ctx, key, value))

    def debug_set(self, key: int, value: int):
        self._chk("cd_debug_option", self.lib.cd_debug_option(self._ctx, key, value, None))

    def debug_get(self, key: int) -> int:
        out = C.c_int64(0)
        self._chk("cd_debug_option", self.lib.cd_debug_option(self._ctx, key, 0, C.byref(out)))
        return out.value

    def update_vertices(self, verts):
        v = np.ascontiguousarray(verts, dtype=np.float64).reshape(-1, 3)
        assert v.shape[0] == self.nv
        self.verts = v
        self._chk("cd_update_vertices", self.lib.cd_update_vertices(self._ctx, _ptr(v)))

    def morton_sort(self):
        self._chk("cd_morton_sort", self.lib.cd_morton_sort(self._ctx))

    def build_hierarchy(self) -> int:
        w = C.c_uint32(0)
        self._chk("cd_build_hierarchy", self.lib.cd_build_hierarchy(self._ctx, C.byref(w)))
        return w.value

    def build_tree(self):
        self._chk("cd_build_tree", self.lib.cd_build_tree(self._ctx))

    def refit_boxes(self):
        self._chk("cd_refit_boxes", self.lib.cd_refit_boxes(self._ctx))

    def check_internal(self):
        out = np.zeros(5, dtype=np.uint32)
        self._chk("cd_check_internal", self.lib.cd_check_internal(self._ctx, _ptr(out)))
        return out

    def check_leaves(self):
        out = np.zeros(4, dtype=np.uint32)
        self._chk("cd_check_leaves", self.lib.cd_check_leaves(self._ctx, _ptr(out)))
        return out

    def check_triangle_idx(self, maxv: int) -> int:
# ... 62 lines not shown
        return pairs[:got].copy(), n.value, rc

    def find_proximity_between(self, other, dist: float, cap: int = 1 << 20):
        pairs = np.empty((max(cap, 1), 2), dtype=np.uint32)
        dists = np.empty(max(cap, 1), dtype=np.float64)
        n, tested = C.c_uint64(0), C.c_uint64(0)
        rc = self.lib.cd_find_proximity_between(self._ctx, other._ctx, float(dist), _ptr(pairs) if cap else None, _ptr(dists), cap,
                                                C.byref(n), C.byref(tested))
        self._chk("cd_find_proximity_between", rc, allow=(CD_OK, CD_OVERFLOW))
        self.between_tested = tested.value
        got = min(n.value, cap)
        return pairs[:got].copy(), dists[:got].copy(), n.value, rc

    def find_ccd_between(self, other, dist: float, verts_end=None, other_verts_end=None, cap: int = 1 << 20):
        def end(v, nv, what):
            if v is None:
                return None
            v = np.ascontiguousarray(v, dtype=np.float64)
            if v.shape != (nv, 3):
                raise ValueError(f"{what} must be [{nv}, 3], got {v.shape}")
            return v
        va = end(verts_end, self.nv, "verts_end")
        vb = end(other_verts_end, other.nv, "other_verts_end")
        pairs = np.empty((max(cap, 1), 2), dtype=np.uint32)
        toi = np.empty(max(cap, 1), dtype=np.float64)
        dists = np.empty(max(cap, 1), dtype=np.float64)
        n, info = C.c_uint64(0), CdCcdInfo()
        rc = self.lib.cd_find_ccd_between(self._ctx, _ptr(va), other._ctx, _ptr(vb), float(dist), _ptr(pairs) if cap else None,
                                          _ptr(toi), _ptr(dists), cap, C.byref(n), C.byref(info))
        self._chk("cd_find_ccd_between", rc, allow=(CD_OK, CD_OVERFLOW))
        self.ccd_info = info
        got = min(n.value, cap)
        return pairs[:got].copy(), toi[:got].copy(), dists[:got].copy(), n.value, rc

    def cast_rays(self, origins, dirs, tmax=np.inf, any_hit: bool = False):
        rays = pack_rays(origins, dirs, tmax)
        n = rays.shape[0]
        face = np.empty(n, dtype=np.uint32)
        info = CdRayInfo()
        if any_hit:
            rc = self.lib.cd_cast_rays(self._ctx, _ptr(rays), n, CD_RAY_ANY, _ptr(face), None, None, None, None, C.byref(info))
            self._chk("cd_cast_rays", rc)
            return face, info
        ids = np.empty(n, dtype=np.uint32)
        t = np.empty(n, dtype=np.float64)
        uv = np.empty((n, 2), dtype=np.float64)
        side = np.empty(n, dtype=np.uint8)
        rc = self.lib.cd_cast_rays(self._ctx, _ptr(rays), n, 0, _ptr(face), _ptr(ids), _ptr(t), _ptr(uv), _ptr(side), C.byref(info))
        self._chk("cd_cast_rays", rc)
        return face, ids, t, uv, side, info

    def closest_points(self, points, rmax=np.inf, any_within: bool = False):
        pts = pack_points(points, rmax)
        n = pts.shape[0]
        face = np.empty(n, dtype=np.uint32)
        info = CdPointInfo()
        if any_within:
            rc = self.lib.cd_closest_points(self._ctx, _ptr(pts), n, CD_POINT_ANY, _ptr(face), None, None, None, None, None, None, C.byref(info))
            self._chk("cd_closest_points", rc)
            return face, info
        ids = np.empty(n, dtype=np.uint32)
        dist = np.empty(n, dtype=np.float64)
        closest = np.empty((n, 3), dtype=np.float64)
        uv = np.empty((n, 2), dtype=np.float64)
        feature = np.empty(n, dtype=np.uint8)
        side = np.empty(n, dtype=np.uint8)
        rc = self.lib.cd_closest_points(self._ctx, _ptr(pts), n, 0, _ptr(face), _ptr(ids), _ptr(dist), _ptr(closest), _ptr(uv), _ptr(feature), _ptr(side),
                                        C.byref(info))
        self._chk("cd_closest_points", rc)
        return face, ids, dist, closest, uv, feature, side, info

    def find_collisions(self, cap: int = 1 << 20):
        return self._pairs_call(self.lib.cd_find_collisions, "cd_find_collisions", cap)

    def self_collide(self, cap: int = 1 << 20, copy: bool = True):
        return self._pairs_call(self.lib.cd_self_collide, "cd_self_collide", cap, copy=copy)

    def self_collide_into(self, buf: np.ndarray):
        fc = getattr(self, "_fast", None)
        if fc is None or fc[0] is not buf:
            n = C.c_uint64(0)
            self.fast_stats = CdStats()
            fc = self._fast = (buf, _ptr(buf), C.c_uint64(buf.shape[0]), n, C.byref(n), C.byref(self.fast_stats),
                               self.lib.cd_self_collide, self.lib.cd_get_stats)
        rc = fc[6](self._ctx, fc[1], fc[2], fc[4])
        if rc != CD_OK and rc != CD_OVERFLOW:
            raise CdError("cd_self_collide", rc)
        fc[7](self._ctx, fc[5])
        return fc[3].value, rc

    def sorted_pairs(self, cap: int = 1 << 20):
        return self._pairs_call(self.lib.cd_sorted_pairs, "cd_sorted_pairs", cap)

    def collision_triangles(self, cap: int = 1 << 21):
        n = C.c_uint64(0)
        buf = np.empty(cap, dtype=np.uint32)
        rc = self.lib.cd_collision_triangles(self._ctx, _ptr(buf), cap, C.byref(n))
        self._chk("cd_collision_triangles", rc, allow=(CD_OK, CD_OVERFLOW))
        return buf[:min(n.value, cap)].copy(), n.value, rc

    def brute_force(self, box_filter: bool = True, cap: int = 1 << 20):
        return self._pairs_call(self.lib.cd_brute_force, "cd_brute_force", cap, 1 if box_filter else 0)

    def test_pairs(self, pairs: np.ndarray) -> np.ndarray:
        p = np.ascontiguousarray(pairs, dtype=np.uint32).reshape(-1, 2)
        out = np.zeros(p.shape[0], dtype=np.uint8)
        self._chk("cd_test_pairs", self.lib.cd_test_pairs(self._ctx, _ptr(p), p.shape[0], _ptr(out)))
        return out

    def export_keys(self):
        keys = np.zeros(self.nt, dtype=np.uint64)
        perm = np.zeros(self.nt, dtype=np.uint32)
        self._chk("cd_export_keys", self.lib.cd_export_keys(self._ctx, _ptr(keys), _ptr(perm)))
        return keys, perm

    def export_tree(self, with_boxes: bool = True):
        n = self.nt
        parent = np.zeros(2 * n - 1, dtype=np.int32)
        left = np.zeros(max(n - 1, 0), dtype=np.int32)
        right = np.zeros(max(n - 1, 0), dtype=np.int32)
        boxes = np.zeros((2 * n - 1, 6), dtype=np.float64) if with_boxes else None
        bounded = np.zeros(max(n - 1, 0), dtype=np.uint32) if with_boxes else None
        self._chk("cd_export_tree", self.lib.cd_export_tree(self._ctx, _ptr(parent), _ptr(left), _ptr(right), _ptr(boxes), _ptr(bounded)))
        return parent, left, right, boxes, bounded

    def stats(self) -> CdStats:
        s = CdStats()
        self._chk("cd_get_stats", self.lib.cd_get_stats(self._ctx, C.byref(s)))
        return s

    def debug_counters(self) -> np.ndarray:
        out = np.zeros(12, dtype=np.uint64)
        self._chk("cd_debug_counters", self.lib.cd_debug_counters(self._ctx, out.ctypes.data))
        return out

    def debug_hint(self, with_order: bool = True, with_tri: bool = False):
        g = (self.nt + 63) // 64
        cost = np.zeros(g, dtype=np.uint32); order = np.zeros(g, dtype=np.uint32); tri = np.zeros(self.nt, dtype=np.uint8)
        self._chk("cd_debug_hint", self.lib.cd_debug_hint(self._ctx, _ptr(cost), _ptr(order) if with_order else None, _ptr(tri) if with_tri else None))
        return (cost, (order if with_order else None), tri) if with_tri else (cost, (order if with_order else None))

    def debug_hint_set(self, order: np.ndarray):
        o = np.ascontiguousarray(order, dtype=np.uint32)
        self._chk("cd_debug_hint_set", self.lib.cd_debug_hint_set(self._ctx, _ptr(o)))

    def debug_records(self):
        n = self.nt
        recs = np.zeros((2 * n, 8), dtype=np.uint32)
        qb = np.zeros((n, 8), dtype=np.uint32)
        root = C.c_int32(0)
        self._chk("cd_debug_records", self.lib.cd_debug_records(self._ctx, recs.ctypes.data, qb.ctypes.data, C.byref(root)))
        return recs[:n], recs[n:], qb, int(root.value)

    def debug_swept(self, other=None):
        which = 0 if other is None else 1
        m, pad, got = C.c_uint32(0), C.c_float(0.0), C.c_uint32(0)
        self._chk("cd_debug_swept", self.lib.cd_debug_swept(self._ctx, which, None, None, None, None, C.byref(got)))
        n = got.value
        if n != (self.nt if other is None else other.nt):
            raise ValueError(f"the swept tree there has {n} leaves: not this mesh's")
        if n < 2:
            self._chk("cd_debug_swept", self.lib.cd_debug_swept(self._ctx, which, None, None, C.byref(m), C.byref(pad), None))
            none = np.zeros((0, 8), dtype=np.uint32)
            return none, none, np.zeros(0, dtype=np.int32), int(m.value), np.float32(pad.value)
        recs = np.zeros((2 * n, 8), dtype=np.uint32)
        up = np.zeros(2 * n - 1, dtype=np.int32)
        self._chk("cd_debug_swept", self.lib.cd_debug_swept(self._ctx, which, recs.ctypes.data, up.ctypes.data, C.byref(m), C.byref(pad), None))
        return recs[:n], recs[n:], up, int(m.value), np.float32(pad.value)

    def set_vertex_id_base(self, base: int):
        self._chk("cd_set_vertex_id_base", self.lib.cd_set_vertex_id_base(self._ctx, base))

    def root_box(self) -> np.ndarray:
        b = np.zeros(6, dtype=np.float64)
        self._chk("cd_root_box", self.lib.cd_root_box(self._ctx, _ptr(b)))
        return b

    def pack_queries_into(self, box, d_out_ptr: int, cap: int):
        b = np.ascontiguousarray(box, dtype=np.float64)
        n = C.c_uint64(0)
        rc = self.lib.cd_pack_queries(self._ctx, _ptr(b), C.c_void_p(d_out_ptr), cap, C.byref(n))
        self._chk("cd_pack_queries", rc, allow=(CD_OK, CD_OVERFLOW))
        return n.value, rc

    def find_collisions_queries(self, d_queries_ptr: int, nq: int, cap: int = 1 << 20):
        return self._pairs_call(self.lib.cd_find_collisions_queries, "cd_find_collisions_queries", cap,
                                C.c_void_p(d_queries_ptr), C.c_uint64(nq))


def load_obj(path: str, threads: int = 0):
    lib = load_library()
    pv, pf = C.POINTER(C.c_double)(), C.POINTER(C.c_uint32)()
    nv, nt = C.c_uint32(0), C.c_uint32(0)
    rc = lib.cd_load_obj(path.encode(), C.byref(pv), C.byref(nv), C.byref(pf), C.byref(nt), threads)
    if rc != CD_OK:
        raise CdError("cd_load_obj", rc)
    try:
        verts = np.ctypeslib.as_array(pv, shape=(nv.value, 3)).copy()
        vidx = np.ctypeslib.as_array(pf, shape=(nt.value, 3)).copy()
    finally:
        lib.cd_free_obj(pv, pf)
    return verts, vidx


class HostPairs:

    def __init__(self, cap: int):
        self.lib = load_library()
        self._p = C.POINTER(C.c_uint32)()
        rc = self.lib.cd_alloc_host_pairs(cap, C.byref(self._p))
        if rc != CD_OK:
            raise CdError("cd_alloc_host_pairs", rc)
        self.array = np.ctypeslib.as_array(self._p, shape=(cap, 2))

    def close(self):
        if self._p:
            self.array = None
            self.lib.cd_free_host_pairs(self._p)
            self._p = C.POINTER(C.c_uint32)()

    def __enter__(self):
        return self

    def __exit__(self, *a):
        self.close()


def morton3d_points(xyz, offset=None, span=None) -> np.ndarray:
    p = np.ascontiguousarray(xyz, dtype=np.float64).reshape(-1, 3)
    off = None if offset is None else np.ascontiguousarray(offset, dtype=np.float64)
    sp = None if span is None else np.ascontiguousarray(span, dtype=np.float64)
    keys = np.zeros(p.shape[0], dtype=np.uint64)
    rc = load_library().cd_morton3d_points(_ptr(p), p.shape[0], _ptr(off), _ptr(sp), _ptr(keys))
    if rc != CD_OK:
        raise CdError("cd_morton3d_points", rc)
    return keys


def morton3d_points_layout(xyz, offset, span, layout: int) -> np.ndarray:
    p = np.ascontiguousarray(xyz, dtype=np.float64).reshape(-1, 3)
    off = np.ascontiguousarray(offset, dtype=np.float64); sp = np.ascontiguousarray(span, dtype=np.float64)
    keys = np.zeros(p.shape[0], dtype=np.uint64)
    rc = load_library().cd_morton3d_points_layout(_ptr(p), p.shape[0], _ptr(off), _ptr(sp), int(layout), _ptr(keys))
    if rc != CD_OK:
        raise CdError("cd_morton3d_points_layout", rc)
    return keys


def expand64_values(v) -> np.ndarray:
    a = np.ascontiguousarray(v, dtype=np.uint64).ravel()
    out = np.zeros(a.shape[0], dtype=np.uint64)
    rc = load_library().cd_expand64_values(_ptr(a), a.shape[0], _ptr(out))
    if rc != CD_OK:
        raise CdError("cd_expand64_values", rc)
    return out


def box_pairs(a, b, want_merged=True):
    a = np.ascontiguousarray(a, dtype=np.float64).reshape(-1, 6); b = np.ascontiguousarray(b, dtype=np.float64).reshape(-1, 6)
    ov = np.zeros(a.shape[0], dtype=np.uint8)
    mg = np.zeros_like(a) if want_merged else None
    rc = load_library().cd_box_pairs(_ptr(a), _ptr(b), a.shape[0], _ptr(ov), _ptr(mg))
    if rc != CD_OK:
        raise CdError("cd_box_pairs", rc)
    return ov, mg


def tri_contact_points(tri) -> np.ndarray:
    t = np.ascontiguousarray(tri, dtype=np.float64).reshape(-1, 18)
    out = np.zeros(t.shape[0], dtype=np.uint8)
    rc = load_library().cd_tri_contact_points(_ptr(t), t.shape[0], _ptr(out))
    if rc != CD_OK:
        raise CdError("cd_tri_contact_points", rc)
    return out


def tri_distance_points(tri) -> np.ndarray:
    t = np.ascontiguousarray(tri, dtype=np.float64).reshape(-1, 18)
    out = np.zeros(t.shape[0], dtype=np.float64)
    rc = load_library().cd_tri_distance_points(_ptr(t), t.shape[0], _ptr(out))
    if rc != CD_OK:
        raise CdError("cd_tri_distance_points", rc)
    return out


def pack_rays(origins, dirs, tmax=np.inf) -> np.ndarray:
    o = np.asarray(origins, dtype=np.float64).reshape(-1, 3)
    d = np.asarray(dirs, dtype=np.float64).reshape(-1, 3)
    if o.shape != d.shape:
        raise ValueError(f"origins {o.shape} and dirs {d.shape} differ")
    rays = np.empty((o.shape[0], 7), dtype=np.float64)
    rays[:, 0:3] = o
    rays[:, 3:6] = d
    rays[:, 6] = tmax
    return rays


def ray_tri_points(rays, tris):
    r = np.ascontiguousarray(np.asarray(rays, dtype=np.float64).reshape(-1, 7))
    p = np.ascontiguousarray(np.asarray(tris, dtype=np.float64).reshape(-1, 9))
    if r.shape[0] != p.shape[0]:
        raise ValueError(f"{r.shape[0]} rays against {p.shape[0]} triangles")
    n = r.shape[0]
    hit = np.zeros(n, dtype=np.uint8)
    t = np.zeros(n, dtype=np.float64)
    uv = np.zeros((n, 2), dtype=np.float64)
# ... 99 lines not shown
```

include/mi355cd.h:

```cpp
#ifndef MI355CD_H
#define MI355CD_H

#include <stdint.h>

#ifdef __cplusplus
extern "C" {
#endif

typedef struct cd_ctx cd_ctx;

enum {
    CD_OK            = 0,
    CD_OVERFLOW      = 1,
    CD_ERR_ARG       = -1001,
    CD_ERR_ORDER     = -1002,
    CD_ERR_NO_DEVICE = -1003,
    CD_ERR_INDEX     = -1004,
    CD_ERR_SORT      = -1005,
    CD_ERR_IO        = -1006,
    CD_ERR_FORMAT    = -1007,
    CD_ERR_RCCL      = -1008,
    CD_ERR_PEER      = -1009,
    CD_ERR_INJECTED  = -1010
};

enum {
    CD_FRAME_REFERENCE = 0,
    CD_FRAME_AUTO      = 1,
    CD_FRAME_CUSTOM    = 2
};

typedef struct cd_stats {
    float ms_morton;
    float ms_sort;
    float ms_hierarchy;
    float ms_refit;
    float ms_traverse;
    float ms_check;
    uint32_t traverse_launches;
    uint32_t stack_overflows;
    uint64_t n_pairs;
    uint64_t pairs_tested;
    uint64_t node_visits;
    uint64_t wave_steps;
    uint64_t candidates;
    float ms_descend;
    float ms_exact;
    uint32_t sort_passes;
    float ms_pipeline;
    float ms_build_block;
    float ms_descend_clock;
} cd_stats;

int cd_load_obj(const char *path, double **verts_xyz, uint32_t *nv, uint32_t **vidx3, uint32_t *nt, int threads);
void cd_free_obj(double *verts_xyz, uint32_t *vidx3);

int cd_create(cd_ctx **out, const double *verts_xyz, uint32_t nv,
              const uint32_t *vidx3, const uint32_t *ids, uint32_t nt);
void cd_destroy(cd_ctx *ctx);

int cd_update_vertices(cd_ctx *ctx, const double *verts_xyz);

int cd_set_morton_frame(cd_ctx *ctx, int mode, const double offset[3], const double span[3]);
int cd_get_morton_frame(cd_ctx *ctx, double offset[3], double span[3], uint64_t *layout);
int cd_set_morton_frame_layout(cd_ctx *ctx, const double offset[3], const double span[3], uint64_t layout);

int cd_morton3d_points(const double *xyz, uint64_t n, const double offset[3], const double span[3], uint64_t *keys);
int cd_morton3d_points_layout(const double *xyz, uint64_t n, const double offset[3], const double span[3], uint64_t layout, uint64_t *keys);
int cd_expand64_values(const uint64_t *v, uint64_t n, uint64_t *out);

int cd_box_pairs(const double *a, const double *b, uint64_t n, uint8_t *overlap, double *merged);
int cd_tri_contact_points(const double *tri, uint64_t n, uint8_t *out);

int cd_morton_sort(cd_ctx *ctx);

int cd_build_hierarchy(cd_ctx *ctx, uint32_t *parent_wrong_num);

int cd_refit_boxes(cd_ctx *ctx);

int cd_check_internal(cd_ctx *ctx, uint32_t out[5]);
int cd_check_leaves(cd_ctx *ctx, uint32_t out[4]);
int cd_check_triangle_idx(cd_ctx *ctx, uint32_t maxv, uint32_t *out);

int cd_find_collisions(cd_ctx *ctx, uint32_t *pairs, uint64_t cap_pairs, uint64_t *n_pairs);

int cd_alloc_host_pairs(uint64_t cap_pairs, uint32_t **pairs);
void cd_free_host_pairs(uint32_t *pairs);

int cd_build_tree(cd_ctx *ctx);

int cd_self_collide(cd_ctx *ctx, uint32_t *pairs, uint64_t cap_pairs, uint64_t *n_pairs);

int cd_sorted_pairs(cd_ctx *ctx, uint32_t *pairs, uint64_t cap_pairs, uint64_t *n_pairs);
int cd_collision_triangles(cd_ctx *ctx, uint32_t *ids, uint64_t cap, uint64_t *n);

int cd_brute_force(cd_ctx *ctx, int box_filter, uint32_t *pairs, uint64_t cap_pairs, uint64_t *n_pairs);

int cd_test_pairs(cd_ctx *ctx, const uint32_t *pairs, uint64_t n_pairs, uint8_t *out);

int cd_export_keys(cd_ctx *ctx, uint64_t *keys, uint32_t *perm);
int cd_export_tree(cd_ctx *ctx, int32_t *parent, int32_t *left, int32_t *right, double *boxes,
                   uint32_t *bounded);

enum {
    CD_OPT_TRAVERSAL        = 0,
    CD_OPT_SORT_FULL        = 2,
    CD_OPT_KERNEL_STAMPS    = 4,
    CD_OPT_STAGE_TIMING     = 3,
    CD_OPT_GRAPH            = 5,
    CD_OPT_POLL             = 6,
    CD_OPT_CELL_TABLE       = 7,
    CD_OPT_ORDER_HINT       = 8,
    CD_OPT_QUERIES_PER_WAVE = 1
};
int cd_set_option(cd_ctx *ctx, int key, int64_t value);

enum {
    CD_DBG_LDS_PAD            = 0,
    CD_DBG_EXACT_BLOCKS       = 1,
    CD_DBG_NO_SHARED_PATH     = 2,
    CD_DBG_DIAG               = 3,
    CD_DBG_STAGEWISE_BUILD    = 4,
    CD_DBG_SPLIT_CROSS        = 5,
    CD_DBG_REPORT_COPIES      = 6,
    CD_DBG_SORT_WINDOWS       = 7,
    CD_DBG_GET_SORT_FORM      = 8,
    CD_DBG_STORE_QBOX         = 9,
    CD_DBG_POLL_SCAN          = 10,
    CD_DBG_GET_POLL_STALE     = 11,
    CD_DBG_GET_POLL_FALLBACKS = 12,
    CD_DBG_GET_POLLED_STEPS   = 13,
    CD_DBG_GET_POLL_FB_WHY    = 16,
    CD_DBG_GET_POLL_MAX_WAIT_US = 17,
    CD_DBG_BIG_OFFSETS        = 18,
    CD_DBG_GET_GRAPH_CAPTURES = 19,
    CD_DBG_GET_GRAPH_REPLAYS  = 20,
    CD_DBG_GET_TREE_WAS_FUSED = 14,
    CD_DBG_GET_ORDER_STATE    = 15
};
int cd_debug_option(cd_ctx *ctx, int key, int64_t value, int64_t *out);

int cd_get_stats(cd_ctx *ctx, cd_stats *out);
int cd_debug_counters(cd_ctx *ctx, unsigned long long out[12]);
int cd_debug_hint(cd_ctx *ctx, uint32_t *cost, uint32_t *order, uint8_t *tri);
int cd_debug_hint_set(cd_ctx *ctx, const uint32_t *order);
int cd_debug_records(cd_ctx *ctx, void *recs, void *qboxes, int32_t *root);
int cd_debug_swept(cd_ctx *ctx, int between, void *recs, int32_t *up, uint32_t *m_bits, float *pad, uint32_t *n_leaves);
int cd_num_triangles(cd_ctx *ctx, uint32_t *nt);

typedef struct cd_query {
    double   v[9];
    uint32_t id;
    uint32_t vidx[3];
} cd_query;

int cd_set_vertex_id_base(cd_ctx *ctx, uint32_t base);
int cd_root_box(cd_ctx *ctx, double box[6]);
int cd_pack_queries(cd_ctx *ctx, const double box[6], void *d_out, uint64_t cap, uint64_t *n);
int cd_find_collisions_queries(cd_ctx *ctx, const void *d_queries, uint64_t nq,
                               uint32_t *pairs, uint64_t cap_pairs, uint64_t *n_pairs);

typedef struct cd_multi cd_multi;
enum {
    CD_MULTI_SELF_PEER = 1,
    CD_MULTI_TIMING    = 2,
    CD_MULTI_CROSS_SERIAL = 8,
    CD_MULTI_SELF_SLICE = 4,
    CD_MULTI_PRIORITY_STREAM = 32,
    CD_MULTI_INJECT_FAILURE = 16,
    CD_MULTI_INJECT_ALLOC_FAILURE = 64
};
typedef struct cd_multi_info {
    uint32_t world, rank;
    uint32_t n_peers;
    uint32_t host_syncs;
    uint32_t attempts;
    uint32_t failed_rank_plus1;
    uint64_t sent_queries, recv_queries, local_pairs, cross_pairs, pairs_tested, query_cap;
    float ms_tree, ms_allgather, ms_pack, ms_counts, ms_exchange, ms_local, ms_cross;
    float pad1;
} cd_multi_info;
int cd_multi_unique_id(void *id128);
int cd_multi_create(cd_multi **out, cd_ctx *ctx, const void *id128, int rank, int world, uint64_t query_cap_per_peer, int flags);
int cd_multi_create_from_comm(cd_multi **out, cd_ctx *ctx, void *nccl_comm, uint64_t query_cap_per_peer, int flags);
void cd_multi_destroy(cd_multi *m);
int cd_multi_set_flags(cd_multi *m, int flags);
int cd_multi_step(cd_multi *m, uint32_t *pairs, uint64_t cap_pairs, uint64_t *n_pairs, cd_multi_info *info);

int cd_find_proximity(cd_ctx *ctx, double dist, uint32_t *pairs, double *dists, uint64_t cap_pairs,
                      uint64_t *n_pairs, uint64_t *n_tested);
int cd_self_proximity(cd_ctx *ctx, double dist, uint32_t *pairs, double *dists, uint64_t cap_pairs,
                      uint64_t *n_pairs, uint64_t *n_tested);
int cd_tri_distance_points(const double *tri, uint64_t n, double *dist);

typedef struct cd_ccd_info { uint64_t n_candidates, n_tested, n_evals, n_unresolved; } cd_ccd_info;
int cd_find_ccd(cd_ctx *ctx, const double *verts_end, double dist, uint32_t *pairs, double *toi, double *dists,
                uint64_t cap_pairs, uint64_t *n_pairs, cd_ccd_info *info);
int cd_self_ccd(cd_ctx *ctx, const double *verts_end, double dist, uint32_t *pairs, double *toi, double *dists,
                uint64_t cap_pairs, uint64_t *n_pairs, cd_ccd_info *info);
int cd_ccd_points(const double *tri, uint64_t n, double dist, double *toi, double *dists, uint32_t *evals);

int cd_find_collisions_between(cd_ctx *a, cd_ctx *b, uint32_t *pairs, uint64_t cap_pairs,
                               uint64_t *n_pairs, uint64_t *n_tested);
int cd_find_proximity_between(cd_ctx *a, cd_ctx *b, double dist, uint32_t *pairs, double *dists,
                              uint64_t cap_pairs, uint64_t *n_pairs, uint64_t *n_tested);
int cd_find_ccd_between(cd_ctx *a, const double *verts_end_a, cd_ctx *b, const double *verts_end_b, double dist,
                        uint32_t *pairs, double *toi, double *dists, uint64_t cap_pairs, uint64_t *n_pairs,
                        cd_ccd_info *info);

typedef struct cd_ray_info { uint64_t n_hits, node_visits, tri_tests; } cd_ray_info;
enum { CD_RAY_ANY = 1 };
int cd_cast_rays(cd_ctx *ctx, const double *rays, uint64_t n, int flags, uint32_t *face, uint32_t *ids, double *t,
                 double *uv, uint8_t *side, cd_ray_info *info);
int cd_ray_tri_points(const double *ray, const double *tri, uint64_t n, uint8_t *hit, double *t, double *uv, uint8_t *side);

typedef struct cd_point_info { uint64_t n_found, node_visits, tri_tests; } cd_point_info;
enum { CD_POINT_ANY = 1 };
int cd_closest_points(cd_ctx *ctx, const double *points, uint64_t n, int flags, uint32_t *face, uint32_t *ids, double *dist,
                      double *closest, double *uv, uint8_t *feature, uint8_t *side, cd_point_info *info);
int cd_pt_tri_points(const double *points, const double *tri, uint64_t n, double *dist, double *closest, double *uv,
                     uint8_t *feature, uint8_t *side);

const char *cd_version(void);

#ifdef __cplusplus
}
#endif
#endif
```

Baseline: 10.70 billion.

## Resolve cross-block LBVH ranges via per-block/group min-delta index instead of key search

The block build kernel now records per-64-leaf-group and per-block minimum delta bytes, plus per-crossing-node info (direction, threshold, in-block min delta and offset). The cross-fused kernel uses these to find the range end and split of nodes spanning blocks. It scans block minima with SWAR byte compares and narrows to group and quad level with DPP row reductions, replacing the exponential/binary search over 64-bit Morton keys. This adds global index buffers and doubles the cross list, in exchange for less key traffic and fewer dependent search steps on the critical path of the hierarchy build.

```diff
diff --git a/gpu-computing-course_amd/csrc/cd_build.h b/gpu-computing-course_amd/csrc/cd_build.h
--- a/gpu-computing-course_amd/csrc/cd_build.h
+++ b/gpu-computing-course_amd/csrc/cd_build.h
@@ -82,6 +82,9 @@
     return __longlong_as_double((long long)((k >> 63) ? (k & 0x7fffffffffffffffull) : ~k));
 }
 
+constexpr uint32_t CROSS_NONE = 255u;
+__device__ __forceinline__ uint32_t cross_info(bool right, int thr, uint32_t mval, uint32_t mrel) { return (right ? 1u : 0u) | ((uint32_t)thr << 1) | (mval << 8) | (mrel << 16); }
+
 struct ZeroPlan { uint32_t *w0; uint32_t nw0; uint4 *q; uint32_t nq; uint32_t *w1; uint32_t nw1;
                   uint32_t *flag; };
 
@@ -89,7 +92,9 @@
                                                            const uint64_t *__restrict__ keys, int32_t *__restrict__ split_of,
                                                            double *__restrict__ boxes, NodeRec32 *__restrict__ recs32, LeafBox32 *__restrict__ qbox32,
                                                            int32_t *__restrict__ root_name, double *__restrict__ seg, float *__restrict__ seg32, int nbp2,
-                                                           int32_t *__restrict__ cross_list, uint32_t *__restrict__ cross_count, uint32_t cross_cap, ZeroPlan zp,
+                                                           int32_t *__restrict__ cross_list ,
+                                                           uint32_t *__restrict__ cross_count, uint32_t cross_cap, ZeroPlan zp,
+                                                           uint8_t *__restrict__ gmin, uint8_t *__restrict__ bmin ,
                                                            int seg_min ,
                                                            AmbTable amb, const uint8_t *__restrict__ vamb,
                                                            const uint32_t *__restrict__ hint_perm, const uint8_t *__restrict__ hint_tri, uint32_t *__restrict__ hint_cost ,
@@ -114,7 +119,7 @@
     __shared__ uint8_t lcov[REFIT_BLK];
     __shared__ unsigned long long lexact[REFIT_BLK / 64], lcertain[REFIT_BLK / 64];
     __shared__ unsigned long long acc[6];
-    __shared__ int32_t lcross[64];
+    __shared__ int32_t lcross[64], linfo[64];
     __shared__ uint32_t lcount, lbase;
     const int b = blockIdx.x, b0 = b * REFIT_BLK, tid = threadIdx.x;
     const int j = b0 + tid;
@@ -169,6 +174,8 @@
         }
     }
     __syncthreads();
+    if (tid < 8) gmin[8 * (size_t)b + tid] = (uint8_t)(dt[6][64 * tid + 1] >> DK_SHIFT);
+    if (tid == 8) bmin[b] = (uint8_t)(dt[REFIT_LOG][1] >> DK_SHIFT);
     if (j < n) {
         const B32 tot = b32_load(t[1]);
         if (m32.lx == tot.lx) atomicMin(&acc[0], f64_ordered(mine.x1));
@@ -214,9 +221,21 @@
         }
         lsplit[tid] = have ? (int16_t)(split - b0) : (int16_t)-1;
         if (cross) {
+            const int a = right ? tid + 1 : 1, e = right ? REFIT_BLK : tid;
+            uint32_t mv = CROSS_NONE, mo = 0u;
+            if (e >= a) {
+                const int k = 31 - __clz(e - a + 1);
+                const int a1 = e - (1 << k) + 1;
+                const DKey m0 = dt[k][a], m1 = dt[k][a1];
+                const int omask = (1 << DK_SHIFT) - 1;
+                const bool second = (m1 >> DK_SHIFT) < (m0 >> DK_SHIFT);
+                mv = (uint32_t)((second ? m1 : m0) >> DK_SHIFT);
+                mo = (uint32_t)((second ? a1 + ((int)m1 & omask) : a + ((int)m0 & omask)) - 1);
+            }
+            const uint32_t info = cross_info(right, thr, mv, mo);
             const uint32_t k = atomicAdd(&lcount, 1u);
-            if (k < 64u) lcross[k] = i;
-            else { const uint32_t g = atomicAdd(cross_count, 1u); if (g < cross_cap) cross_list[g] = i; }
+            if (k < 64u) { lcross[k] = i; linfo[k] = (int32_t)info; }
+            else { const uint32_t g = atomicAdd(cross_count, 1u); if (g < cross_cap) { cross_list[g] = i; cross_list[(size_t)cross_cap + g] = (int32_t)info; } }
         }
     }
     __syncthreads();
@@ -252,7 +271,7 @@
     if (cnt == 0) return;
     if (tid == 0) lbase = atomicAdd(cross_count, cnt);
     __syncthreads();
-    if ((uint32_t)tid < cnt && lbase + tid < cross_cap) cross_list[lbase + tid] = lcross[tid];
+    if ((uint32_t)tid < cnt && lbase + tid < cross_cap) { cross_list[lbase + tid] = lcross[tid]; cross_list[(size_t)cross_cap + lbase + tid] = linfo[tid]; }
 }
 
 __global__ __launch_bounds__(256) void k_fill_qbox(const double *__restrict__ verts, const LeafTri *__restrict__ leaf, int n, LeafBox32 *__restrict__ qbox32,
@@ -489,10 +508,24 @@
     if (tid == 0) *top_flag = top_seq;
 }
 
-__global__ __launch_bounds__(256, 2) void k_cross_fused(const uint64_t *__restrict__ keys, int n, const double *__restrict__ seg, const float *__restrict__ seg32,
+constexpr int XCH = 4;
+template <int CTRL>
+__device__ __forceinline__ uint32_t dpp_row_u32(uint32_t v) { return (uint32_t)__builtin_amdgcn_update_dpp((int)v, (int)v, CTRL, 0xf, 0xf, false); }
+__device__ __forceinline__ uint32_t group_min_u32(uint32_t x)
+{
+    static_assert(XG == 16, "a group is a DPP row");
+    uint32_t y;
+    y = dpp_row_u32<0x128>(x); x = y < x ? y : x;
+    y = dpp_row_u32<0x124>(x); x = y < x ? y : x;
+    y = dpp_row_u32<0x122>(x); x = y < x ? y : x;
+    y = dpp_row_u32<0x121>(x); x = y < x ? y : x;
+    return x;
+}
+
+__global__ __launch_bounds__(256, 2) void k_cross_fused(const uint64_t *__restrict__ keys, int n, const uint8_t *__restrict__ gmin, const uint8_t *__restrict__ bmin , const double *__restrict__ seg, const float *__restrict__ seg32,
                                                      int nbp2, int nblocks, const unsigned long long *__restrict__ leaf_side , double *__restrict__ boxes,
                                                      NodeRec32 *__restrict__ recs32, const int32_t *__restrict__ split_of, int32_t *__restrict__ root_name,
-                                                     const int32_t *__restrict__ dense, const uint32_t *__restrict__ dense_total, uint32_t dense_cap,
+                                                     const int32_t *__restrict__ dense , const uint32_t *__restrict__ dense_total, uint32_t dense_cap,
                                                      unsigned long long *top_pub , uint32_t *top_flag, uint32_t top_seq,
                                                      uint32_t nord ,
                                                      uint32_t order_groups, const uint32_t *__restrict__ hint_cost, uint32_t *__restrict__ hint_order)
@@ -531,33 +564,138 @@
         int first = 0, last = 0, split = 0;
         {
             auto delta_v = [](uint64_t ka, int ia, uint64_t kb, int ib) { const uint64_t x = ka ^ kb; return x ? __clzll((long long)x) : 64 + __clz((int)((uint32_t)ia ^ (uint32_t)ib)); };
-            const int i = live ? dense[kq] : 0;
-            const uint64_t ki = keys[i], kprev = keys[i > 0 ? i - 1 : 0], knext = keys[i + 1 < n ? i + 1 : n - 1];
-            const int dnext = i + 1 < n ? delta_v(ki, i, knext, i + 1) : -1, dprev = i > 0 ? delta_v(ki, i, kprev, i - 1) : -1;
-            const int d = (dnext - dprev) >= 0 ? 1 : -1;
-            const int delta_min = d > 0 ? dprev : dnext;
-            int mlen = 0;
-            for (int r = 0; r < 2; ++r) {
-                const bool todo = live && mlen == 0;
-                if (!__builtin_amdgcn_ballot_w64(todo)) break;
-                const int e = r * XG + gl;
-                const long long o = (long long)i + (long long)d * (2ll << (e < 31 ? e : 31));
-                const bool yes = todo && e < 31 && o >= 0 && o < n && delta_k(keys, n, i, ki, (int)o) > delta_min;
-                const uint32_t no = ~group_ballot(yes, g) & ((1u << XG) - 1u);
-                if (todo && no) mlen = 2 << (r * XG + __ffs((int)no) - 1);
-            }
-            const int l = group_last_true(live, mlen >> 1, mlen, g, gl, [&](int x) { return delta_k(keys, n, i, ki, i + x * d) > delta_min; });
-            const int j = i + l * d;
-            first = min(i, j); last = max(i, j);
-            const uint64_t kj = keys[j];
-            const uint64_t kbefore = first > 0 ? keys[first - 1] : 0ull, kafter = last < n - 1 ? keys[last + 1] : 0ull;
-            const uint64_t kf = first == i ? ki : kj, kl = last == i ? ki : kj;
-            const int common = delta_v(kf, first, kl, last);
-            split = group_last_true(live, first, last, g, gl, [&](int x) { return delta_k(keys, n, first, kf, x) > common; });
+            auto group_deltas = [&](int G, int quad, uint32_t (&A)[4]) {
+                const int q0 = 64 * G + 4 * quad;
+                uint64_t k[5];
+#pragma unroll
+                for (int u = 0; u < 5; ++u) k[u] = keys[q0 + u < n ? q0 + u : n - 1];
+#pragma unroll
+                for (int u = 0; u < 4; ++u) A[u] = q0 + u < n - 1 ? (uint32_t)(delta_v(k[u], q0 + u, k[u + 1], q0 + u + 1) + 1) : 0u;
+            };
+            const int i = dense[live ? kq : 0u];
+            const uint32_t info = (uint32_t)dense[(size_t)dense_cap + (live ? kq : 0u)];
+            const bool right = (info & 1u) != 0u;
+            const int thr = (int)((info >> 1) & 127u);
+            const uint32_t sthr = thr > 0 ? (uint32_t)thr : 1u;
+            const int B = i >> REFIT_LOG, nchunks = (nblocks + 15) >> 4, src_base = lane & ~(XG - 1);
+            uint32_t wbest = ~0u;
+            int F = 0; bool found = false;
+            {
+                int cur = right ? B + 1 : B - 1;
+                bool done = !live || cur < 0 || cur >= nblocks;
+                for (int round = 0; ; ++round) {
+                    if (!__builtin_amdgcn_ballot_w64(!done)) break;
+                    const int c0 = cur >> 4;
+                    const int per = round ? XCH : 1;
+                    uint4 w[XCH]; int cc[XCH]; bool cv[XCH];
+#pragma unroll
+                    for (int u = 0; u < XCH; ++u) {
+                        cc[u] = right ? c0 + per * gl + u : c0 - per * gl - u;
+                        cv[u] = !done && u < per && cc[u] >= 0 && cc[u] < nchunks;
+                        w[u] = reinterpret_cast<const uint4 *>(bmin)[cv[u] ? cc[u] : 0];
+                    }
+                    uint32_t lmin = ~0u; int hit = -1;
+#pragma unroll
+                    for (int u = 0; u < XCH; ++u) {
+                        if (u > 0 && !__builtin_amdgcn_ballot_w64(cv[u])) break;
+                        const uint32_t ww[4] = {w[u].x, w[u].y, w[u].z, w[u].w};
+                        const int base = 16 * cc[u];
+                        int lo_o = right ? cur - base : 0, hi_o = right ? nblocks - base : cur - base + 1;
+                        lo_o = lo_o < 0 ? 0 : (lo_o > 16 ? 16 : lo_o); hi_o = hi_o < 0 ? 0 : (hi_o > 16 ? 16 : hi_o);
+                        const uint32_t vm = cv[u] && hi_o > lo_o ? ((1u << hi_o) - 1u) & ~((1u << lo_o) - 1u) : 0u;
+                        uint32_t below = 0u;
+#pragma unroll
+                        for (int q = 0; q < 4; ++q) {
+                            const uint32_t t = (ww[q] | 0x80808080u) - sthr * 0x01010101u;
+                            const uint32_t m = (~t >> 7) & 0x01010101u;
+                            below |= ((m * 0x01020408u) >> 24) << (4 * q);
+                        }
+                        const uint32_t hb = below & vm;
+                        uint32_t before = hit < 0 ? vm : 0u;
+                        if (hit < 0 && hb) {
+                            const int pos = right ? __ffs((int)hb) - 1 : 31 - __clz((int)hb);
+                            hit = base + pos;
+                            before = right ? vm & ((1u << pos) - 1u) : vm & ~((2u << pos) - 1u);
+                        }
+                        while (__builtin_amdgcn_ballot_w64(before != 0u)) {
+                            if (before) {
+                                const int pos = __ffs((int)before) - 1;
+                                before &= before - 1u;
+                                const uint32_t wsel = pos < 8 ? (pos < 4 ? ww[0] : ww[1]) : (pos < 12 ? ww[2] : ww[3]);
+                                const uint32_t key = (((wsel >> (8 * (pos & 3))) & 255u) << 24) | (uint32_t)(base + pos);
+                                lmin = key < lmin ? key : lmin;
+                            }
+                        }
+                    }
+                    const uint32_t hm = group_ballot(hit >= 0, g);
+                    const int hl = hm ? __ffs((int)hm) - 1 : XG;
+                    const uint32_t gk = group_min_u32(gl <= hl ? lmin : ~0u);
+                    const int fb = __shfl(hit, src_base + (hm ? hl : 0));
+                    if (!done) {
+                        wbest = gk < wbest ? gk : wbest;
+                        if (hm) { F = fb; found = true; done = true; }
+                        else { cur = right ? (c0 + XG * per) * 16 : (c0 - XG * per) * 16 + 15; done = cur < 0 || cur >= nblocks; }
+                    }
+                }
+            }
+            const int go = (right ? gl : 7 - gl) & 7;
+            const uint2 gw = reinterpret_cast<const uint2 *>(gmin)[F];
+            const uint32_t gv = ((go < 4 ? gw.x : gw.y) >> (8 * (go & 3))) & 255u;
+            const uint32_t gm = group_ballot(found && gl < 8 && gv < sthr, g);
+            const int ghl = gm ? __ffs((int)gm) - 1 : 0;
+            const bool gfound = gm != 0u;
+            const uint32_t gbest = group_min_u32(gfound && gl < ghl ? (gv << 24) | (uint32_t)(8 * F + go) : ~0u);
+            const int G = gfound ? 8 * F + (right ? ghl : 7 - ghl) : 0;
+            const int qd = right ? gl : 15 - gl;
+            uint32_t A[4];
+            group_deltas(G, qd, A);
+            uint32_t pmin = ~0u, hv = 0u; int hu = -1;
+#pragma unroll
+            for (int e = 0; e < 4; ++e) {
+                const uint32_t v = right ? A[e] : A[3 - e];
+                const int o = right ? e : 3 - e;
+                const bool open = hu < 0;
+                const uint32_t key = (v << 8) | (uint32_t)(4 * qd + o);
+                if (open && v < sthr) { hu = o; hv = v; }
+                else if (open && key < pmin) pmin = key;
+            }
+            const uint32_t pm = group_ballot(gfound && hu >= 0, g);
+            const int phl = pm ? __ffs((int)pm) - 1 : 0;
+            const bool pfound = pm != 0u;
+            const uint32_t pbest = group_min_u32(pfound && gl <= phl ? pmin : ~0u);
+            const int hrel = __shfl(4 * qd + hu, src_base + phl);
+            const int farv = pfound ? __shfl((int)hv, src_base + phl) : 0;
+            const int pf = pfound ? 64 * G + hrel : (right ? n - 1 : -1);
+            first = right ? i : pf + 1; last = right ? pf : i;
+            const uint32_t ev = (info >> 8) & 255u;
+            const uint32_t vb = wbest >> 24, vg = gbest >> 24, vp = pbest == ~0u ? 255u : pbest >> 8;
+            const uint32_t ce = (ev << 2) | (right ? 0u : 3u), cb = (vb << 2) | (right ? 1u : 2u), cg = (vg << 2) | (right ? 2u : 1u), cp = (vp << 2) | (right ? 3u : 0u);
+            uint32_t cm = ce < cb ? ce : cb; cm = cg < cm ? cg : cm; cm = cp < cm ? cp : cm;
+            const uint32_t kind = right ? (cm & 3u) : 3u - (cm & 3u);
+            split = kind == 0u ? (i & ~(REFIT_BLK - 1)) + (int)((info >> 16) & 1023u) : 64 * G + (int)(pbest & 63u);
+            const bool needb = live && kind == 1u, needg = live && (kind == 1u || kind == 2u);
+            int Wg = (int)(gbest & 0xffffffu);
+            if (__builtin_amdgcn_ballot_w64(needb)) {
+                const int Wb = needb ? (int)(wbest & 0xffffffu) : 0;
+                const uint2 ww = reinterpret_cast<const uint2 *>(gmin)[Wb];
+                const uint32_t v = (((gl & 7) < 4 ? ww.x : ww.y) >> (8 * (gl & 3))) & 255u;
+                const uint32_t r = group_min_u32(gl < 8 ? (v << 8) | (uint32_t)gl : ~0u);
+                if (needb) Wg = 8 * Wb + (int)(r & 7u);
+            }
+            if (__builtin_amdgcn_ballot_w64(needg)) {
+                const int Wc = needg ? Wg : 0;
+                uint32_t D[4];
+                group_deltas(Wc, gl, D);
+                uint32_t key = ~0u;
+#pragma unroll
+                for (int e = 0; e < 4; ++e) { const uint32_t kk = (D[e] << 8) | (uint32_t)(4 * gl + e); key = kk < key ? kk : key; }
+                const uint32_t r = group_min_u32(key);
+                if (needg) split = 64 * Wc + (int)(r & 63u);
+            }
             if (live && gl == 0) {
                 if (first == 0 && last == n - 1) *root_name = split;
                 else {
-                    const int dl = first > 0 ? delta_v(kf, first, kbefore, first - 1) : -1, dr = last < n - 1 ? delta_v(kl, last, kafter, last + 1) : -1;
+                    const int dl = (right ? thr : farv) - 1, dr = (right ? farv : thr) - 1;
                     uint32_t *half = reinterpret_cast<uint32_t *>(const_cast<float4 *>(dr > dl ? rec_left(recs32, n, (uint32_t)last) : rec_right(recs32, n, (uint32_t)(first - 1))));
                     half[6] = (uint32_t)split;
                 }
diff --git a/gpu-computing-course_amd/csrc/mi355cd.hip b/gpu-computing-course_amd/csrc/mi355cd.hip
--- a/gpu-computing-course_amd/csrc/mi355cd.hip
+++ b/gpu-computing-course_amd/csrc/mi355cd.hip
@@ -79,6 +79,8 @@
     unsigned long long *d_top_pub = nullptr; uint32_t top_seq = 0;
     LeafTri *d_leaf = nullptr; NodeMeta *d_meta = nullptr; int32_t *d_parent = nullptr; double *d_seg = nullptr; float *d_seg32 = nullptr; uint32_t nbp2 = 1; int32_t *d_cross = nullptr; uint32_t cross_cap = 0;
     double *d_boxes = nullptr; uint32_t *d_bounded = nullptr; NodeRec32 *d_recs32 = nullptr; LeafBox32 *d_qbox = nullptr;
+    uint8_t *d_gmin = nullptr, *d_bmin = nullptr;
+    bool cross_index_valid = false;
     unsigned long long *d_leaf_side = nullptr;
     uint32_t dbg_big_offsets = 0;
     uint32_t dbg_store_qbox = 0;
@@ -173,7 +175,7 @@
     for (int i = 0; i < 2; ++i) { hipFree(c->d_keys[i]); hipFree(c->d_perm[i]); }
     hipFree(c->d_counts); hipFree(c->d_chunk_tot); hipFree(c->d_os); hipFree(c->d_frame); hipFree(c->d_partial);
     hipFree(c->d_top_pub); hipFree(c->d_leaf); hipFree(c->d_meta); hipFree(c->d_parent); hipFree(c->d_seg); hipFree(c->d_seg32); hipFree(c->d_cross); hipFree(c->d_boxes);
-    hipFree(c->d_bounded); hipFree(c->d_recs32); hipFree(c->d_qbox); hipFree(c->d_leaf_side); hipFree(c->d_split_of); hipFree(c->d_cost); hipFree(c->d_order); hipFree(c->d_tri_cost);
+    hipFree(c->d_bounded); hipFree(c->d_recs32); hipFree(c->d_qbox); hipFree(c->d_leaf_side); hipFree(c->d_gmin); hipFree(c->d_bmin); hipFree(c->d_split_of); hipFree(c->d_cost); hipFree(c->d_order); hipFree(c->d_tri_cost);
     hipFree(c->d_amb_keys); hipFree(c->d_amb_flag); hipFree(c->d_vamb);
     for (TravBuf &tb : c->tb) {
         if (tb.d_pairs) hipFree(reinterpret_cast<char *>(tb.d_pairs) - sizeof(Report));
@@ -448,15 +450,17 @@
             hipExtLaunchKernelGGL(k_build_block, dim3(nblocks), dim3(REFIT_BLK), 0u, s, c->ev[EV_BLK0], c->ev[EV_BLK1], 0u,
                                   (const double *)c->d_verts, (const LeafTri *)c->d_leaf, (int)n, (const uint64_t *)c->d_keys[0], c->d_split_of,
                                   c->d_boxes, c->d_recs32, c->d_qbox, c->d_root, c->d_seg, c->d_seg32, (int)c->nbp2,
-                                  cross_list, cross_count, c->cross_cap, zp, seg_min, c->amb, (const uint8_t *)c->vamb, hp, ht, hc, c->d_leaf_side, store_q);
+                                  cross_list, cross_count, c->cross_cap, zp, c->d_gmin, c->d_bmin, seg_min, c->amb, (const uint8_t *)c->vamb, hp, ht, hc, c->d_leaf_side, store_q);
         else
             k_build_block<<<nblocks, REFIT_BLK, 0, s>>>(c->d_verts, c->d_leaf, (int)n, c->d_keys[0], c->d_split_of, c->d_boxes, c->d_recs32, c->d_qbox, c->d_root,
-                                                        c->d_seg, c->d_seg32, (int)c->nbp2, cross_list, cross_count, c->cross_cap, zp, seg_min, c->amb, (const uint8_t *)c->vamb,
+                                                        c->d_seg, c->d_seg32, (int)c->nbp2, cross_list, cross_count, c->cross_cap, zp, c->d_gmin, c->d_bmin, seg_min, c->amb, (const uint8_t *)c->vamb,
                                                         hp, ht, hc, c->d_leaf_side, store_q);
         c->order_pending = hint;
+        c->cross_index_valid = true;
         c->left.scratch_clean = self_cleaning;
     } else {
         c->left.qbox_valid = true;
+        c->cross_index_valid = false;
         k_refit_seg_local<<<nblocks, REFIT_BLK, 0, s>>>(c->d_verts, c->d_leaf, (int)n, c->d_meta, c->d_boxes, c->d_bounded,
                                                        c->d_recs32, c->d_qbox, c->d_root, write_internal ? 1 : 0, c->d_seg, (int)c->nbp2,
                                                        cross_list, cross_count, c->cross_cap, c->amb, (const uint8_t *)c->vamb);
@@ -479,11 +483,11 @@
         }
         if (done)
             hipExtLaunchKernelGGL(k_cross_fused, dim3(nord + xb + 2u ), dim3(256), xlds, s, nullptr, done, 0u,
-                                  (const uint64_t *)c->d_keys[0], (int)n, (const double *)c->d_seg, (const float *)c->d_seg32, (int)c->nbp2, nblocks, (const unsigned long long *)c->d_leaf_side, c->d_boxes,
+                                  (const uint64_t *)c->d_keys[0], (int)n, (const uint8_t *)c->d_gmin, (const uint8_t *)c->d_bmin, (const double *)c->d_seg, (const float *)c->d_seg32, (int)c->nbp2, nblocks, (const unsigned long long *)c->d_leaf_side, c->d_boxes,
                                   c->d_recs32, (const int32_t *)c->d_split_of, c->d_root, (const int32_t *)c->d_cross, (const uint32_t *)cross_count, c->cross_cap,
                                   c->d_top_pub, top_flag, c->top_seq, nord, ogroups, (const uint32_t *)c->d_cost, c->d_order);
         else
-            k_cross_fused<<<nord + xb + 2u, 256, xlds, s>>>(c->d_keys[0], (int)n, c->d_seg, c->d_seg32, (int)c->nbp2, nblocks, c->d_leaf_side, c->d_boxes,
+            k_cross_fused<<<nord + xb + 2u, 256, xlds, s>>>(c->d_keys[0], (int)n, c->d_gmin, c->d_bmin, c->d_seg, c->d_seg32, (int)c->nbp2, nblocks, c->d_leaf_side, c->d_boxes,
                                                             c->d_recs32, c->d_split_of, c->d_root, c->d_cross, cross_count, c->cross_cap, c->d_top_pub, top_flag, c->top_seq,
                                                             nord, ogroups, c->d_cost, c->d_order);
         if (nord) c->order_ready = true;
@@ -1015,7 +1019,8 @@
     if (hipMemset(c->d_top_pub, 0, top_pub_bytes(c)) != hipSuccess) { free_all(c); delete c; return -(int)hipGetLastError(); }
     ALLOC(c->d_seg32, sizeof(float) * 6 * ((size_t)c->nbp2 << (REFIT_LOG - SEG32_MIN_LEVEL + 1)));
     c->cross_cap = nt;
-    ALLOC(c->d_cross, sizeof(int32_t) * (size_t)c->cross_cap);
+    ALLOC(c->d_cross, sizeof(int32_t) * 2 * (size_t)c->cross_cap);
+    ALLOC(c->d_gmin, 8 * (size_t)c->nbp2); ALLOC(c->d_bmin, ((size_t)c->nbp2 + 15) / 16 * 16);
     ALLOC(c->d_boxes, sizeof(double) * 6 * 2 * n);
     ALLOC(c->d_bounded, sizeof(uint32_t) * n);
     ALLOC(c->d_recs32, sizeof(NodeRec32) * n);
@@ -1426,6 +1431,17 @@
     for (uint32_t b = 0; b < groups; ++b) { if (order[b] >= groups || seen[order[b]]) return CD_ERR_ARG; seen[order[b]] = 1; }
     HIPCHK(hipMemcpy(c->d_order, order, sizeof(uint32_t) * groups, hipMemcpyHostToDevice));
     c->order_ready = true;
+    return CD_OK;
+}
+
+int cd_debug_cross_index(cd_ctx *c, uint8_t *gmin, uint8_t *bmin)
+{
+    if (!c) return CD_ERR_ARG;
+    if (c->stage < ST_REFIT || !c->cross_index_valid) return CD_ERR_ORDER;
+    HIPCHK(hipStreamSynchronize(c->stream));
+    const size_t nblocks = cdiv(c->nt, REFIT_BLK);
+    if (gmin) HIPCHK(hipMemcpy(gmin, c->d_gmin, 8 * nblocks, hipMemcpyDeviceToHost));
+    if (bmin) HIPCHK(hipMemcpy(bmin, c->d_bmin, nblocks, hipMemcpyDeviceToHost));
     return CD_OK;
 }
 
diff --git a/gpu-computing-course_amd/pyhost/mi355cd.py b/gpu-computing-course_amd/pyhost/mi355cd.py
--- a/gpu-computing-course_amd/pyhost/mi355cd.py
+++ b/gpu-computing-course_amd/pyhost/mi355cd.py
@@ -76,7 +76,7 @@
     "cd_load_obj", "cd_free_obj", "cd_create", "cd_destroy", "cd_update_vertices", "cd_set_morton_frame", "cd_get_morton_frame", "cd_set_morton_frame_layout", "cd_morton_sort",
     "cd_build_hierarchy", "cd_refit_boxes", "cd_check_internal", "cd_check_leaves",
     "cd_check_triangle_idx", "cd_find_collisions", "cd_build_tree", "cd_self_collide", "cd_sorted_pairs", "cd_collision_triangles", "cd_brute_force",
-    "cd_test_pairs", "cd_export_keys", "cd_export_tree", "cd_get_stats", "cd_debug_counters", "cd_debug_records", "cd_debug_swept", "cd_num_triangles",
+    "cd_test_pairs", "cd_export_keys", "cd_export_tree", "cd_get_stats", "cd_debug_counters", "cd_debug_records", "cd_debug_cross_index", "cd_debug_swept", "cd_num_triangles",
     "cd_set_option", "cd_set_vertex_id_base", "cd_root_box", "cd_pack_queries", "cd_find_collisions_queries", "cd_version",
     "cd_debug_option", "cd_debug_hint", "cd_debug_hint_set", "cd_morton3d_points", "cd_morton3d_points_layout", "cd_expand64_values", "cd_box_pairs", "cd_tri_contact_points", "cd_alloc_host_pairs", "cd_free_host_pairs",
     "cd_multi_unique_id", "cd_multi_create", "cd_multi_create_from_comm", "cd_multi_destroy", "cd_multi_set_flags", "cd_multi_step",
@@ -132,6 +132,7 @@
     lib.cd_get_stats.argtypes = [vp, C.POINTER(CdStats)]
     lib.cd_debug_counters.argtypes = [vp, vp]
     lib.cd_debug_records.argtypes = [vp, vp, vp, vp]
+    lib.cd_debug_cross_index.argtypes = [vp, vp, vp]
     lib.cd_debug_swept.argtypes = [vp, C.c_int, vp, vp, u32p, C.POINTER(C.c_float), u32p]
     lib.cd_debug_hint.argtypes = [vp, vp, vp, vp]
     lib.cd_debug_hint_set.argtypes = [vp, vp]
@@ -500,6 +501,13 @@
         self._chk("cd_debug_records", self.lib.cd_debug_records(self._ctx, recs.ctypes.data, qb.ctypes.data, C.byref(root)))
         return recs[:n], recs[n:], qb, int(root.value)
 
+    def debug_cross_index(self):
+        nb = (self.nt + 511) // 512
+        gmin = np.zeros(8 * nb, dtype=np.uint8)
+        bmin = np.zeros(nb, dtype=np.uint8)
+        self._chk("cd_debug_cross_index", self.lib.cd_debug_cross_index(self._ctx, gmin.ctypes.data, bmin.ctypes.data))
+        return gmin, bmin
+
     def debug_swept(self, other=None):
         which = 0 if other is None else 1
         m, pad, got = C.c_uint32(0), C.c_float(0.0), C.c_uint32(0)
diff --git a/include/mi355cd.h b/include/mi355cd.h
--- a/include/mi355cd.h
+++ b/include/mi355cd.h
@@ -145,6 +145,7 @@
 int cd_debug_hint(cd_ctx *ctx, uint32_t *cost, uint32_t *order, uint8_t *tri);
 int cd_debug_hint_set(cd_ctx *ctx, const uint32_t *order);
 int cd_debug_records(cd_ctx *ctx, void *recs, void *qboxes, int32_t *root);
+int cd_debug_cross_index(cd_ctx *ctx, uint8_t *gmin, uint8_t *bmin);
 int cd_debug_swept(cd_ctx *ctx, int between, void *recs, int32_t *up, uint32_t *m_bits, float *pad, uint32_t *n_leaves);
 int cd_num_triangles(cd_ctx *ctx, uint32_t *nt);
 
```

After: 9.688 billion. 0.906x the previous value.
